# Lakonik/SSDNeRF

Measured on AMD Instinct MI355X. Metric: rays/s (rendered-views/s = rays/s / 16384), SRN Cars 128x128 novel-view render of cached triplanes, higher is better.
Workload: dtype f32

## Files before the change

include/ssdnerf_hip.h:

```cpp
#ifndef SSDNERF_HIP_H
#define SSDNERF_HIP_H

#include <stddef.h>
#include <stdint.h>

#ifdef __cplusplus
extern "C" {
#endif

#define SSDNERF_OK 0
#define SSDNERF_E_INVALID (-1)
#define SSDNERF_E_LAUNCH (-2)
#define SSDNERF_E_WORKSPACE (-3)

#define SSDNERF_DTYPE_F32 0
#define SSDNERF_DTYPE_F16 1

const char* ssdnerf_last_error(void);
int ssdnerf_abi_version(void);


int ssdnerf_near_far_from_aabb(const float* rays_o, const float* rays_d, const float* aabb, uint32_t N, float min_near,
                               float* nears, float* fars, void* stream);

// ... 68 lines not shown
                              const uint8_t* bitfield, uint32_t grid_size, const float* rays_o, const float* rays_d,
                              uint32_t N, float bound, float min_near, float dt_gamma, uint32_t max_steps, float T_thresh,
                              float bg_color, float sigmoid_saturation, float* image, float* depth, float* weights_sum,
                              int32_t* sample_counts, int32_t* overflow_flag, void* stream);

int ssdnerf_render_rays_fused_batch(const void* planes, int planes_dtype, uint32_t Hp, uint32_t Wp, const float* mlp_params,
                                    const uint8_t* bitfield, uint32_t grid_size, const float* rays_o, const float* rays_d,
                                    uint32_t S, uint32_t N, float bound, float min_near, float dt_gamma, const float* dt_gammas,
                                    uint32_t max_steps, float T_thresh, float bg_color, float sigmoid_saturation, float* image,
                                    float* depth, float* weights_sum, int32_t* sample_counts, int32_t* overflow_flag,
                                    void* stream);

size_t ssdnerf_render_queue_workspace(uint32_t S, uint32_t N, uint32_t grid_size);
int ssdnerf_render_first_hit(const uint8_t* bitfield, uint32_t grid_size, const float* rays_o, const float* rays_d, uint32_t S,
                             uint32_t N, float bound, float min_near, float dt_gamma, const float* dt_gammas, uint32_t max_steps,
                             float bg_color, float* image, float* depth, float* weights_sum, int32_t* sample_counts,
                             void* workspace, size_t workspace_bytes, void* stream);
int ssdnerf_render_shade_queue(const void* planes, int planes_dtype, uint32_t Hp, uint32_t Wp, const float* mlp_params,
                               uint32_t grid_size, const float* rays_o, const float* rays_d, uint32_t S, uint32_t N, float bound,
                               float min_near, float dt_gamma, const float* dt_gammas, uint32_t max_steps, float T_thresh,
                               float bg_color, float sigmoid_saturation, float* image, float* depth, float* weights_sum,
                               int32_t* sample_counts, int32_t* overflow_flag, void* workspace, size_t workspace_bytes,
                               void* stream);

#define SSDNERF_SHADE_FULL_DIR_PRODUCTS 0x100
int ssdnerf_render_shade_queue_mfma(const void* planes, int planes_dtype, uint32_t Hp, uint32_t Wp, const float* mlp_params,
                                    uint32_t grid_size, const float* rays_o, const float* rays_d, uint32_t S, uint32_t N,
                                    float bound, float min_near, float dt_gamma, const float* dt_gammas, uint32_t max_steps,
                                    float T_thresh, float bg_color, float sigmoid_saturation, float* image, float* depth,
                                    float* weights_sum, int32_t* sample_counts, int32_t* overflow_flag, void* workspace,
                                    size_t workspace_bytes, void* stream);

#define SSDNERF_FIRST_HIT_SMALL_BLOCKS 0x10000u
int ssdnerf_render_first_hit_cams(const uint8_t* bitfield, uint32_t grid_size, const float* c2w, const float* intrinsics, uint32_t S,
                                  uint32_t V, uint32_t h, uint32_t w, float bound, float min_near, float dt_gamma,
                                  const float* dt_gammas, uint32_t max_steps, float bg_color, float* image, float* depth,
                                  float* weights_sum, int32_t* sample_counts, uint8_t* image_u8, void* workspace, size_t workspace_bytes,
                                  void* stream);
int ssdnerf_render_shade_queue_mfma_cams(const void* planes, int planes_dtype, uint32_t Hp, uint32_t Wp, const float* mlp_params,
                                         uint32_t grid_size, const float* c2w, const float* intrinsics, uint32_t S, uint32_t V,
                                         uint32_t h, uint32_t w, float bound, float min_near, float dt_gamma, const float* dt_gammas,
                                         uint32_t max_steps, float T_thresh, float bg_color, float sigmoid_saturation, float* image,
                                         float* depth, float* weights_sum, int32_t* sample_counts, int32_t* overflow_flag,
                                         uint8_t* image_u8, void* workspace, size_t workspace_bytes, void* stream);

int ssdnerf_density_grid_update(const void* planes, int planes_dtype, uint32_t Hp, uint32_t Wp, const float* mlp_params,
                                uint32_t S, uint32_t grid_size, float bound, const float* jitter, float decay,
                                void* density_grid, int grid_dtype, float* mean_out, void* stream);

int ssdnerf_packbits_dev_thresh(const void* grid, int grid_dtype, uint32_t N, const float* mean, float density_thresh,
                                uint8_t* bitfield, void* stream);


int ssdnerf_ddim_step_v(const float* x_t, const float* v, uint64_t n, float sqrt_ab, float sqrt_1mab, float sqrt_ab_prev,
                        float dir_coef, float clip_lo, float clip_hi, float* x0_out, float* xprev_out, void* stream);

int ssdnerf_dpmpp_step_v(const float* x_t, const float* v, const float* x0_prev, uint64_t n, float sqrt_ab, float sqrt_1mab, float c,
                         float d, float e, float clip_lo, float clip_hi, float* x0_out, float* xnext_out, void* stream);
uint32_t ssdnerf_dpmpp_block_cap(void);

int ssdnerf_philox_normal_fill(float* out, uint64_t n, uint64_t seed, uint32_t draw, void* stream);

int ssdnerf_sde_step_v(const float* x_t, const float* v, const float* x0_prev, uint64_t n, int form, float sqrt_ab, float sqrt_1mab, float c,
                       float d, float e, float nz, float clip_lo, float clip_hi, uint64_t seed, uint32_t draw, float* x0_out, float* xnext_out,
                       void* stream);
uint32_t ssdnerf_sde_block_cap(void);

int ssdnerf_prior_q_sample(const float* x0, const float* a, const float* b, uint32_t B, uint64_t n_per, uint64_t seed, uint32_t draw,
                           float* x_t_out, void* stream);
int ssdnerf_prior_loss_v(const void* pred, int pred_dtype, const float* x0, const float* a, const float* b, uint32_t B, uint64_t n_per,
                         uint64_t seed, uint32_t draw, float* partials, float* msd_out, float* x0sq_out, void* stream);
int ssdnerf_prior_loss_v_backward(const void* pred, int pred_dtype, const float* x0, const float* a, const float* b, const float* k, uint32_t B,
                                  uint64_t n_per, uint64_t seed, uint32_t draw, void* grad_pred_out, float* grad_x0_out, void* stream);
uint32_t ssdnerf_prior_block_cap(void);
uint32_t ssdnerf_prior_blocks_per_sample(uint64_t n_per);
uint64_t ssdnerf_prior_loss_partials(uint32_t B, uint64_t n_per);

int ssdnerf_cam_rays(const float* c2w, const float* intrinsics, uint32_t n_views, uint32_t h, uint32_t w, float* rays_o,
                     float* rays_d, void* stream);

int ssdnerf_quantize_u8(const float* x, uint64_t n, uint8_t* y, void* stream);

int ssdnerf_image_metrics(const float* a, const float* b, uint32_t n, uint32_t h, uint32_t w, float* mse, float* ssim, void* stream);

int ssdnerf_tv_loss_forward(const float* x, uint32_t n, uint32_t h, uint32_t w, float power, float* slice_mean, void* stream);
int ssdnerf_tv_loss_backward(const float* x, const float* g, uint32_t n, uint32_t h, uint32_t w, float power, float* dx_out, void* stream);

#define SSDNERF_ADAM_MAX_TENSORS 32
typedef struct ssdnerf_adam_tensor {
    float* param;
    const float* grad;
    float* exp_avg;
    float* exp_avg_sq;
    uint64_t numel;
    float step_size, bc2_sqrt, weight_decay;
    uint32_t reserved;
} ssdnerf_adam_tensor;
uint32_t ssdnerf_adam_max_tensors(void);
int ssdnerf_adam_step_multi(const ssdnerf_adam_tensor* tensors, uint32_t T, double beta1, double beta2, double eps, void* stream);

#define SSDNERF_EMA_MAX_ROWS (1u << 20)
typedef struct ssdnerf_ema_row {
    const float* src;
    float* dst;
    uint64_t numel;
    uint32_t trainable;
    uint32_t first_block;
} ssdnerf_ema_row;
uint32_t ssdnerf_ema_chunk(void);
int ssdnerf_ema_plan_build(ssdnerf_ema_row* rows, uint32_t T, uint32_t* blocks_out);
int ssdnerf_ema_update_multi(const ssdnerf_ema_row* plan, uint32_t T, uint32_t blocks, float momentum, float momentum_nontrainable, void* stream);

int ssdnerf_gather_views_u8(const uint8_t* store, uint64_t image_bytes, uint64_t num_images, const int32_t* index, uint64_t count, float* out,
                            void* stream);

int ssdnerf_sample_rays_u8(const uint8_t* store, uint64_t num_images, uint32_t h, uint32_t w, const int32_t* view_image, const float* c2w,
                           const float* intr, uint32_t S, uint32_t V, const int64_t* inds, uint32_t R, float* rays_o, float* rays_d, float* target,
                           void* stream);

int ssdnerf_perm_indices(int64_t* out, uint32_t S, uint64_t P, uint64_t start, uint32_t R, uint64_t seed, uint32_t draw, void* stream);
int ssdnerf_sample_rays_perm_u8(const uint8_t* store, uint64_t num_images, uint32_t h, uint32_t w, const int32_t* view_image, const float* c2w,
                                const float* intr, uint32_t S, uint32_t V, uint64_t seed, uint32_t draw, uint64_t start, uint32_t R, float* rays_o,
                                float* rays_d, float* target, void* stream);

#define SSDNERF_CACHE_MAX_SCENES 32
typedef struct ssdnerf_cache_store {
    void* code;
    void* exp_avg;
    void* exp_avg_sq;
    void* density_grid;
    void* density_bitfield;
    uint64_t slots, numel, grid_bytes, bits_bytes;
    int32_t code_dtype, moment_dtype;
} ssdnerf_cache_store;
typedef struct ssdnerf_cache_row {
    uint32_t slot;
    uint32_t row;
    uint32_t has_state;
    uint32_t reserved;
} ssdnerf_cache_row;
uint32_t ssdnerf_cache_max_scenes(void);
int ssdnerf_cache_load_multi(const ssdnerf_cache_store* store, const ssdnerf_cache_row* rows, uint32_t S, float* leaves, float* m, float* v,
                             void* grid, void* bits, void* stream);
int ssdnerf_cache_store_multi(const ssdnerf_cache_store* store, const ssdnerf_cache_row* rows, uint32_t S, const float* leaves, const float* m,
                              const float* v, const void* grid, const void* bits, void* stream);

size_t ssdnerf_group_norm_workspace(uint32_t B, uint32_t G);
int ssdnerf_group_norm_nhwc(const void* x, const void* x2, uint32_t C1, int dtype, uint32_t B, uint32_t HW, uint32_t C, uint32_t G, const float* pre_bias,
                            const float* gamma, const float* beta, const float* scale_shift, uint32_t scale_shift_stride,
                            float eps, int act, void* workspace, int workspace_state, void* y, void* stream);
int ssdnerf_group_norm_nhwc_runs(const void* x, const void* x2, uint32_t C1, int dtype, uint32_t B, uint32_t HW, uint32_t C, uint32_t G, const float* gamma,
                                 const float* beta, const float* scale_shift, uint32_t scale_shift_stride, float eps, int act, const void* runs1,
                                 const void* runs2, void* y, void* stream);

size_t ssdnerf_group_norm_backward_workspace(uint32_t B, uint32_t G);

int ssdnerf_group_norm_nhwc_backward_cat(const void* x, const void* x2, uint32_t C1, const void* dy, int dtype, uint32_t B, uint32_t HW, uint32_t C, uint32_t G,
                                         const float* gamma, const float* beta, const float* scale_shift, uint32_t scale_shift_stride, float eps, int act,
                                         const void* fwd_sums, const void* fwd_sums2, void* bwd_workspace, int bwd_workspace_is_zero, void* dx, void* dx2,
                                         void* stream);
int ssdnerf_group_norm_nhwc_backward(const void* x, const void* dy, int dtype, uint32_t B, uint32_t HW, uint32_t C, uint32_t G,
                                     const float* gamma, const float* beta, const float* scale_shift, uint32_t scale_shift_stride,
                                     float eps, int act, const void* fwd_sums, void* bwd_workspace, int bwd_workspace_is_zero,
                                     void* dx, void* stream);

int ssdnerf_bias_residual_nhwc(const void* x, int dtype, uint32_t B, uint32_t HW, uint32_t C, const float* bias,
                               const void* residual, void* y, void* gn_sums, uint32_t gn_groups, void* stream);

int ssdnerf_conv2d_nhwc_bf16_supported(uint32_t Cin, uint32_t Cout, uint32_t ksize, uint32_t stride, uint32_t upsample);
int ssdnerf_conv2d_nhwc_bf16_plan(uint32_t M, uint32_t Cin, uint32_t Cout, uint32_t ksize, int tile_hint, int may_split,
                                  int splits_hint);
int ssdnerf_conv2d_nhwc_bf16(const void* x, const void* x2, uint32_t Cin1, const void* w, const float* bias,
                             const void* residual, void* y, uint32_t B, uint32_t H, uint32_t W, uint32_t Cin,
                             uint32_t Cout, uint32_t ksize, uint32_t stride,
                             uint32_t upsample, void* gn_sums, uint32_t gn_groups, int tile_hint, void* splitk_ws,
                             size_t splitk_ws_bytes, int splits_hint, void* stream);

int ssdnerf_conv2d_nhwc_f32x2_plan(uint32_t M, uint32_t Cin, uint32_t Cout, uint32_t ksize, int tile_hint, int splits_hint);
int ssdnerf_conv2d_nhwc_f32x2(const void* x, const void* x2, uint32_t Cin1, const void* w_hi, const void* w_lo, const float* bias,
                              const void* residual, void* y, uint32_t B, uint32_t H, uint32_t W, uint32_t Cin, uint32_t Cout,
                              uint32_t ksize, uint32_t stride, uint32_t upsample, void* gn_sums, uint32_t gn_groups, int tile_hint,
                              int splits_hint, int y_is_zero, void* splitk_ws, size_t splitk_ws_bytes, void* stream);

int ssdnerf_conv2d_nhwc_f32x2_presplit_supported(uint32_t B, uint32_t H, uint32_t W, uint32_t Cin, uint32_t Cout, uint32_t ksize, int with_gn_sums);
int ssdnerf_split_f32_nhwc(const void* x, void* y, uint64_t pixels, uint32_t C, uint64_t x_stride, void* stream);
int ssdnerf_conv2d_nhwc_f32x2_presplit(const void* x_split, const void* w_hi, const void* w_lo, const float* bias, const void* residual, void* y, uint32_t B,
                                       uint32_t H, uint32_t W, uint32_t Cin, uint32_t Cout, uint32_t ksize, void* gn_sums, uint32_t gn_groups,
                                       int tile_hint, int splits_hint, void* splitk_ws, size_t splitk_ws_bytes, void* stream);

int ssdnerf_attention_qkv_bf16(const void* qkv, void* out, uint32_t B, uint32_t T, uint32_t heads, uint32_t ch, void* stream);
int ssdnerf_attention_qkv_f32(const void* qkv, void* out, uint32_t B, uint32_t T, uint32_t heads, uint32_t ch, void* stream);
int ssdnerf_attention_qkv_f32_lse(const void* qkv, void* out, void* lse2, uint32_t B, uint32_t T, uint32_t heads, uint32_t ch, void* stream);
int ssdnerf_attention_qkv_f32_backward(const void* qkv, const void* out, const void* dout, const void* lse2, void* dqkv, void* workspace, uint32_t B,
                                       uint32_t T, uint32_t heads, uint32_t ch, void* stream);

int ssdnerf_marching_cubes_count(const float* volume, uint32_t nx, uint32_t ny, uint32_t nz, float iso, const uint8_t* tri_count,
                                 int32_t* cell_tris, int32_t* point_verts, uint8_t* point_mask, void* stream);
int ssdnerf_marching_cubes_emit(const float* volume, uint32_t nx, uint32_t ny, uint32_t nz, float iso, const uint8_t* tri_count,
                                const int8_t* tri_edges, const int32_t* tri_offsets, const int32_t* vert_offsets, const uint8_t* point_mask,
                                float* vertices, int32_t* triangles, void* stream);
int ssdnerf_mesh_vertex_attributes(const void* planes, int planes_dtype, uint32_t Hp, uint32_t Wp, const float* mlp_params, const float* verts_idx,
                                   uint32_t V, const float* b_min, const float* scale, float sigmoid_saturation, float* xyz, float* sigma,
                                   float* grad_sigma, float* normals, float* colors, uint8_t* colors_u8, void* stream);

int ssdnerf_lpips_input(const float* pred, const float* target, uint32_t n, uint32_t h, uint32_t w, float* out, void* stream);
int ssdnerf_relu_pool_nhwc(const float* x, uint32_t N, uint32_t H, uint32_t W, uint32_t C, int pool, int split_out, void* y, void* stream);
size_t ssdnerf_lpips_layer_workspace(uint32_t n);
int ssdnerf_lpips_layer(const float* x, uint32_t n, uint32_t H, uint32_t W, uint32_t C, const float* lin_w, float* acc, void* y_pool, int split_out,
                        void* workspace, void* stream);

int ssdnerf_feature_moments_accumulate(const float* x, uint32_t n, uint32_t D, double* sum, double* outer, void* stream);
size_t ssdnerf_kid_subset_sums_workspace(uint32_t num_subsets, uint32_t m);
int ssdnerf_kid_subset_sums(const float* fake, const float* real, const int64_t* idx_fake, const int64_t* idx_real, uint32_t num_subsets, uint32_t m,
                            uint32_t D, double* out, void* workspace, size_t workspace_bytes, void* stream);

int ssdnerf_png_filter_rows(const void* pred, int pred_is_u8, const void* target, int target_is_u8, uint32_t n, uint32_t h, uint32_t w, uint8_t* out,
                            void* stream);
int ssdnerf_code_plane_rgb(const float* code, const uint8_t* table, uint32_t S, uint32_t C, uint32_t h, uint32_t w, float vmin, float vmax, int flip_z,
                           uint8_t* out, void* stream);

#ifdef __cplusplus
}
#endif
#endif
```

ssdnerf_amd/_cabi.py:

```python
from __future__ import annotations

import ctypes
import os
from typing import Optional

import torch

_LIB_PATH = os.environ.get("SSDNERF_HIP_LIB") or os.path.join(os.path.dirname(os.path.abspath(__file__)), "lib", "libssdnerf_hip.so")
_lib: Optional[ctypes.CDLL] = None

ABI_VERSION = 3
F32, F16 = 0, 1
BF16 = 2

EXPORTS = [
    "ssdnerf_last_error", "ssdnerf_abi_version", "ssdnerf_near_far_from_aabb", "ssdnerf_sph_from_ray", "ssdnerf_morton3D",
    "ssdnerf_morton3D_invert", "ssdnerf_packbits", "ssdnerf_march_rays_train_workspace", "ssdnerf_march_rays_train",
    "ssdnerf_march_rays_train_batch_workspace", "ssdnerf_march_rays_train_batch_count", "ssdnerf_march_rays_train_batch_write",
    "ssdnerf_composite_rays_train_forward", "ssdnerf_composite_rays_train_backward", "ssdnerf_march_rays", "ssdnerf_composite_rays",
    "ssdnerf_sh_encode_forward", "ssdnerf_sh_encode_backward", "ssdnerf_triplane_pack", "ssdnerf_point_decode", "ssdnerf_point_decode_backward_workspace",
    "ssdnerf_point_decode_backward", "ssdnerf_point_decode_backward_layout",
    "ssdnerf_render_rays_fused", "ssdnerf_render_rays_fused_batch", "ssdnerf_render_queue_workspace", "ssdnerf_render_first_hit",
    "ssdnerf_render_shade_queue", "ssdnerf_render_shade_queue_mfma", "ssdnerf_render_first_hit_cams", "ssdnerf_render_shade_queue_mfma_cams", "ssdnerf_density_grid_update", "ssdnerf_packbits_dev_thresh", "ssdnerf_ddim_step_v",
    "ssdnerf_group_norm_workspace", "ssdnerf_group_norm_backward_workspace", "ssdnerf_group_norm_nhwc", "ssdnerf_group_norm_nhwc_runs", "ssdnerf_group_norm_nhwc_backward", "ssdnerf_group_norm_nhwc_backward_cat", "ssdnerf_bias_residual_nhwc",
    "ssdnerf_conv2d_nhwc_bf16_supported", "ssdnerf_conv2d_nhwc_bf16_plan", "ssdnerf_conv2d_nhwc_bf16", "ssdnerf_conv2d_nhwc_f32x2", "ssdnerf_conv2d_nhwc_f32x2_plan", "ssdnerf_attention_qkv_bf16", "ssdnerf_attention_qkv_f32", "ssdnerf_attention_qkv_f32_lse", "ssdnerf_attention_qkv_f32_backward", "ssdnerf_cam_rays", "ssdnerf_quantize_u8",
    "ssdnerf_marching_cubes_count", "ssdnerf_marching_cubes_emit", "ssdnerf_conv2d_nhwc_f32x2_presplit_supported", "ssdnerf_conv2d_nhwc_f32x2_presplit", "ssdnerf_split_f32_nhwc",
    "ssdnerf_image_metrics", "ssdnerf_tv_loss_forward", "ssdnerf_tv_loss_backward", "ssdnerf_mesh_vertex_attributes",
    "ssdnerf_lpips_input", "ssdnerf_relu_pool_nhwc", "ssdnerf_lpips_layer_workspace", "ssdnerf_lpips_layer",
    "ssdnerf_feature_moments_accumulate", "ssdnerf_kid_subset_sums_workspace", "ssdnerf_kid_subset_sums",
    "ssdnerf_adam_max_tensors", "ssdnerf_adam_step_multi",
    "ssdnerf_gather_views_u8", "ssdnerf_sample_rays_u8", "ssdnerf_perm_indices", "ssdnerf_sample_rays_perm_u8",
    "ssdnerf_ema_chunk", "ssdnerf_ema_plan_build", "ssdnerf_ema_update_multi",
    "ssdnerf_cache_max_scenes", "ssdnerf_cache_load_multi", "ssdnerf_cache_store_multi",
    "ssdnerf_dpmpp_step_v", "ssdnerf_dpmpp_block_cap",
    "ssdnerf_png_filter_rows", "ssdnerf_code_plane_rgb",
    "ssdnerf_philox_normal_fill", "ssdnerf_sde_step_v", "ssdnerf_sde_block_cap",
    "ssdnerf_prior_q_sample", "ssdnerf_prior_loss_v", "ssdnerf_prior_loss_v_backward", "ssdnerf_prior_block_cap", "ssdnerf_prior_blocks_per_sample",
    "ssdnerf_prior_loss_partials",
]


class AdamTensor(ctypes.Structure):
    _fields_ = [("param", ctypes.c_void_p), ("grad", ctypes.c_void_p), ("exp_avg", ctypes.c_void_p), ("exp_avg_sq", ctypes.c_void_p),
                ("numel", ctypes.c_uint64), ("step_size", ctypes.c_float), ("bc2_sqrt", ctypes.c_float), ("weight_decay", ctypes.c_float),
                ("reserved", ctypes.c_uint32)]


class EmaRow(ctypes.Structure):
    _fields_ = [("src", ctypes.c_void_p), ("dst", ctypes.c_void_p), ("numel", ctypes.c_uint64), ("trainable", ctypes.c_uint32),
                ("first_block", ctypes.c_uint32)]


class CacheStore(ctypes.Structure):
    _fields_ = [("code", ctypes.c_void_p), ("exp_avg", ctypes.c_void_p), ("exp_avg_sq", ctypes.c_void_p), ("density_grid", ctypes.c_void_p),
                ("density_bitfield", ctypes.c_void_p), ("slots", ctypes.c_uint64), ("numel", ctypes.c_uint64), ("grid_bytes", ctypes.c_uint64),
                ("bits_bytes", ctypes.c_uint64), ("code_dtype", ctypes.c_int32), ("moment_dtype", ctypes.c_int32)]


class CacheRow(ctypes.Structure):
    _fields_ = [("slot", ctypes.c_uint32), ("row", ctypes.c_uint32), ("has_state", ctypes.c_uint32), ("reserved", ctypes.c_uint32)]


def lib_path() -> str:
    return _LIB_PATH


def lib() -> ctypes.CDLL:
    global _lib
    if _lib is None:
        if not os.path.exists(_LIB_PATH):
            raise RuntimeError(
                f"libssdnerf_hip.so not found at {_LIB_PATH}: build it with `python -m ssdnerf_amd.build` "
                "(there is no CPU fallback for the product path)")
        l = ctypes.CDLL(_LIB_PATH)
        l.ssdnerf_last_error.restype = ctypes.c_char_p
        l.ssdnerf_abi_version.restype = ctypes.c_int
        l.ssdnerf_march_rays_train_workspace.restype = ctypes.c_size_t
        l.ssdnerf_march_rays_train_workspace.argtypes = [ctypes.c_uint32]
        l.ssdnerf_render_queue_workspace.restype = ctypes.c_size_t
        l.ssdnerf_render_queue_workspace.argtypes = [ctypes.c_uint32, ctypes.c_uint32, ctypes.c_uint32]
        l.ssdnerf_march_rays_train_batch_workspace.restype = ctypes.c_size_t
        l.ssdnerf_march_rays_train_batch_workspace.argtypes = [ctypes.c_uint32, ctypes.c_uint32]
        l.ssdnerf_point_decode_backward_workspace.restype = ctypes.c_size_t
        l.ssdnerf_point_decode_backward_workspace.argtypes = [ctypes.c_uint32] * 4
        l.ssdnerf_point_decode_backward_layout.restype = None
        l.ssdnerf_point_decode_backward_layout.argtypes = [ctypes.c_uint32] * 4 + [ctypes.POINTER(ctypes.c_uint64)]
        l.ssdnerf_group_norm_workspace.restype = ctypes.c_size_t
        l.ssdnerf_group_norm_workspace.argtypes = [ctypes.c_uint32, ctypes.c_uint32]
        l.ssdnerf_group_norm_backward_workspace.restype = ctypes.c_size_t
        l.ssdnerf_group_norm_backward_workspace.argtypes = [ctypes.c_uint32, ctypes.c_uint32]
        l.ssdnerf_image_metrics.argtypes = [ctypes.c_void_p, ctypes.c_void_p, ctypes.c_uint32, ctypes.c_uint32, ctypes.c_uint32, ctypes.c_void_p,
                                             ctypes.c_void_p, ctypes.c_void_p]
        l.ssdnerf_tv_loss_forward.argtypes = [ctypes.c_void_p, ctypes.c_uint32, ctypes.c_uint32, ctypes.c_uint32, ctypes.c_float, ctypes.c_void_p,
                                              ctypes.c_void_p]
        l.ssdnerf_tv_loss_backward.argtypes = [ctypes.c_void_p, ctypes.c_void_p, ctypes.c_uint32, ctypes.c_uint32, ctypes.c_uint32, ctypes.c_float,
                                               ctypes.c_void_p, ctypes.c_void_p]
        l.ssdnerf_mesh_vertex_attributes.argtypes = [ctypes.c_void_p, ctypes.c_int, ctypes.c_uint32, ctypes.c_uint32, ctypes.c_void_p, ctypes.c_void_p,
                                                     ctypes.c_uint32, ctypes.POINTER(ctypes.c_float), ctypes.POINTER(ctypes.c_float), ctypes.c_float] + [ctypes.c_void_p] * 7
        l.ssdnerf_lpips_input.argtypes = [ctypes.c_void_p, ctypes.c_void_p, ctypes.c_uint32, ctypes.c_uint32, ctypes.c_uint32, ctypes.c_void_p, ctypes.c_void_p]
        l.ssdnerf_relu_pool_nhwc.argtypes = [ctypes.c_void_p] + [ctypes.c_uint32] * 4 + [ctypes.c_int, ctypes.c_int, ctypes.c_void_p, ctypes.c_void_p]
        l.ssdnerf_lpips_layer_workspace.restype = ctypes.c_size_t
        l.ssdnerf_lpips_layer_workspace.argtypes = [ctypes.c_uint32]
        l.ssdnerf_lpips_layer.argtypes = [ctypes.c_void_p] + [ctypes.c_uint32] * 4 + [ctypes.c_void_p, ctypes.c_void_p, ctypes.c_void_p, ctypes.c_int, ctypes.c_void_p,
                                          ctypes.c_void_p]
        l.ssdnerf_feature_moments_accumulate.argtypes = [ctypes.c_void_p, ctypes.c_uint32, ctypes.c_uint32, ctypes.c_void_p, ctypes.c_void_p, ctypes.c_void_p]
        l.ssdnerf_kid_subset_sums_workspace.restype = ctypes.c_size_t
        l.ssdnerf_kid_subset_sums_workspace.argtypes = [ctypes.c_uint32, ctypes.c_uint32]
        l.ssdnerf_kid_subset_sums.argtypes = [ctypes.c_void_p] * 4 + [ctypes.c_uint32] * 3 + [ctypes.c_void_p, ctypes.c_void_p, ctypes.c_size_t, ctypes.c_void_p]
        l.ssdnerf_adam_max_tensors.restype = ctypes.c_uint32
        l.ssdnerf_adam_max_tensors.argtypes = []
        l.ssdnerf_adam_step_multi.argtypes = [ctypes.POINTER(AdamTensor), ctypes.c_uint32, ctypes.c_double, ctypes.c_double, ctypes.c_double, ctypes.c_void_p]
        l.ssdnerf_gather_views_u8.argtypes = [ctypes.c_void_p, ctypes.c_uint64, ctypes.c_uint64, ctypes.c_void_p, ctypes.c_uint64, ctypes.c_void_p, ctypes.c_void_p]
        l.ssdnerf_sample_rays_u8.argtypes = [ctypes.c_void_p, ctypes.c_uint64, ctypes.c_uint32, ctypes.c_uint32] + [ctypes.c_void_p] * 3 + \
                                            [ctypes.c_uint32, ctypes.c_uint32, ctypes.c_void_p, ctypes.c_uint32] + [ctypes.c_void_p] * 4
        l.ssdnerf_perm_indices.argtypes = [ctypes.c_void_p, ctypes.c_uint32, ctypes.c_uint64, ctypes.c_uint64, ctypes.c_uint32, ctypes.c_uint64,
                                           ctypes.c_uint32, ctypes.c_void_p]
        l.ssdnerf_sample_rays_perm_u8.argtypes = [ctypes.c_void_p, ctypes.c_uint64, ctypes.c_uint32, ctypes.c_uint32] + [ctypes.c_void_p] * 3 + \
                                                 [ctypes.c_uint32, ctypes.c_uint32, ctypes.c_uint64, ctypes.c_uint32, ctypes.c_uint64, ctypes.c_uint32] + \
                                                 [ctypes.c_void_p] * 4
        l.ssdnerf_ema_chunk.restype = ctypes.c_uint32
        l.ssdnerf_ema_chunk.argtypes = []
        l.ssdnerf_ema_plan_build.argtypes = [ctypes.POINTER(EmaRow), ctypes.c_uint32, ctypes.POINTER(ctypes.c_uint32)]
        l.ssdnerf_ema_update_multi.argtypes = [ctypes.c_void_p, ctypes.c_uint32, ctypes.c_uint32, ctypes.c_float, ctypes.c_float, ctypes.c_void_p]
        l.ssdnerf_cache_max_scenes.restype = ctypes.c_uint32
        l.ssdnerf_cache_max_scenes.argtypes = []
        for fn in (l.ssdnerf_cache_load_multi, l.ssdnerf_cache_store_multi):
            fn.argtypes = [ctypes.POINTER(CacheStore), ctypes.POINTER(CacheRow), ctypes.c_uint32] + [ctypes.c_void_p] * 6
        l.ssdnerf_dpmpp_block_cap.restype = ctypes.c_uint32
        l.ssdnerf_dpmpp_block_cap.argtypes = []
        l.ssdnerf_dpmpp_step_v.argtypes = [ctypes.c_void_p] * 3 + [ctypes.c_uint64] + [ctypes.c_float] * 7 + [ctypes.c_void_p] * 3
        l.ssdnerf_sde_block_cap.restype = ctypes.c_uint32
        l.ssdnerf_sde_block_cap.argtypes = []
        l.ssdnerf_philox_normal_fill.argtypes = [ctypes.c_void_p, ctypes.c_uint64, ctypes.c_uint64, ctypes.c_uint32, ctypes.c_void_p]
        l.ssdnerf_sde_step_v.argtypes = [ctypes.c_void_p] * 3 + [ctypes.c_uint64, ctypes.c_int] + [ctypes.c_float] * 8 + \
                                        [ctypes.c_uint64, ctypes.c_uint32] + [ctypes.c_void_p] * 3
        l.ssdnerf_prior_block_cap.restype = l.ssdnerf_prior_blocks_per_sample.restype = ctypes.c_uint32
        l.ssdnerf_prior_block_cap.argtypes = []
        l.ssdnerf_prior_blocks_per_sample.argtypes = [ctypes.c_uint64]
        l.ssdnerf_prior_loss_partials.restype = ctypes.c_uint64
        l.ssdnerf_prior_loss_partials.argtypes = [ctypes.c_uint32, ctypes.c_uint64]
        l.ssdnerf_prior_q_sample.argtypes = [ctypes.c_void_p] * 3 + [ctypes.c_uint32, ctypes.c_uint64, ctypes.c_uint64, ctypes.c_uint32] + [ctypes.c_void_p] * 2
        l.ssdnerf_prior_loss_v.argtypes = [ctypes.c_void_p, ctypes.c_int] + [ctypes.c_void_p] * 3 + \
                                          [ctypes.c_uint32, ctypes.c_uint64, ctypes.c_uint64, ctypes.c_uint32] + [ctypes.c_void_p] * 4
        l.ssdnerf_prior_loss_v_backward.argtypes = [ctypes.c_void_p, ctypes.c_int] + [ctypes.c_void_p] * 4 + \
                                                   [ctypes.c_uint32, ctypes.c_uint64, ctypes.c_uint64, ctypes.c_uint32] + [ctypes.c_void_p] * 3
        l.ssdnerf_png_filter_rows.argtypes =[ctypes.c_void_p, ctypes.c_int, ctypes.c_void_p, ctypes.c_int] + [ctypes.c_uint32] * 3 + [ctypes.c_void_p] * 2
        l.ssdnerf_code_plane_rgb.argtypes = [ctypes.c_void_p] * 2 + [ctypes.c_uint32] * 4 + [ctypes.c_float] * 2 + [ctypes.c_int] + [ctypes.c_void_p] * 2
        if l.ssdnerf_abi_version() != ABI_VERSION:
            raise RuntimeError(f"libssdnerf_hip.so ABI {l.ssdnerf_abi_version()} != expected {ABI_VERSION}: rebuild")
        _lib = l
    return _lib


_SYNC_CHECK = os.environ.get("SSDNERF_SYNC_CHECK", "0") == "1"


def check(status: int, what: str) -> None:
    if status != 0:
        raise RuntimeError(f"{what} failed ({status}): {lib().ssdnerf_last_error().decode()}")
    if _SYNC_CHECK and not torch.cuda.is_current_stream_capturing():
        import sys
        print(f"[ssdnerf sync-check] {what}", file=sys.stderr, flush=True)
        torch.cuda.synchronize()


def ptr(t: Optional[torch.Tensor]) -> ctypes.c_void_p:
    return ctypes.c_void_p(0 if t is None else t.data_ptr())


def stream() -> ctypes.c_void_p:
    return ctypes.c_void_p(torch.cuda.current_stream().cuda_stream)


def u32(v) -> ctypes.c_uint32:
    return ctypes.c_uint32(int(v))


def f32(v) -> ctypes.c_float:
    return ctypes.c_float(float(v))


def dtype_code(t: torch.Tensor) -> int:
    if t.dtype == torch.float32:
        return F32
    if t.dtype == torch.float16:
        return F16
    raise RuntimeError(f"unsupported dtype {t.dtype} (fp32 / fp16 only)")


def require_cuda(*tensors: torch.Tensor) -> None:
    for t in tensors:
# ... 3 lines not shown
```

ssdnerf_amd/csrc/conv_igemm.hip:

```cpp
#include "common.h"
#include <type_traits>

namespace {

typedef __attribute__((ext_vector_type(8))) __bf16 bf16x8;
typedef __attribute__((ext_vector_type(16))) float f32x16;

__device__ __attribute__((aligned(16))) const uint32_t g_conv_zero_page[4] = {0, 0, 0, 0};

struct ConvArgs {
    const unsigned char* x;
    const unsigned char* x2;
    uint32_t Cin1;
    const unsigned char* w;
    const float* bias;
    const unsigned char* res;
    unsigned char* y;
    double* gn_sums;
    float* splitk_ws;
    uint32_t splits;
    uint32_t B, H, W, Cin, Cout;
    uint32_t Ho, Wo, M;
    uint32_t ksize, stride, pad, upsample;
    uint32_t G;
    uint32_t m_tiles, n_tiles;
};

constexpr int CV_BK = 64;
constexpr int CV_ROWB = CV_BK * 2;

SSD_DEV void cv_glds16(const void* gptr, unsigned char* lds_wave_base) {
    __builtin_amdgcn_global_load_lds((const __attribute__((address_space(1))) void*)gptr, (__attribute__((address_space(3))) void*)lds_wave_base, 16, 0, 0);
}

SSD_DEV uint32_t cv_pack_bf16(float lo, float hi) {
    typedef float f2 __attribute__((ext_vector_type(2)));
    typedef __bf16 b2 __attribute__((ext_vector_type(2)));
    const b2 r = __builtin_convertvector(f2{lo, hi}, b2);
    return *reinterpret_cast<const uint32_t*>(&r);
}

template <int CTRL, int RM, int BM, bool BC> SSD_DEV double cv_dpp_f64(double v) {
    const unsigned long long u = (unsigned long long)__double_as_longlong(v);
    const uint32_t lo = (uint32_t)__builtin_amdgcn_update_dpp(0, (int)(uint32_t)u, CTRL, RM, BM, BC);
    const uint32_t hi = (uint32_t)__builtin_amdgcn_update_dpp(0, (int)(uint32_t)(u >> 32), CTRL, RM, BM, BC);
    return __longlong_as_double((long long)(((unsigned long long)hi << 32) | lo));
}
SSD_DEV double cv_half_wave_sum(double v) {
    v += cv_dpp_f64<0xB1, 0xf, 0xf, true>(v);
    v += cv_dpp_f64<0x4E, 0xf, 0xf, true>(v);
    v += cv_dpp_f64<0x141, 0xf, 0xf, true>(v);
    v += cv_dpp_f64<0x140, 0xf, 0xf, true>(v);
    v += cv_dpp_f64<0x142, 0xa, 0xf, false>(v);
    return v;
}

template <int TM, int TN, bool F32 = false>
SSD_DEV void cv_epilogue_direct(const ConvArgs& a, f32x16 (&acc)[TN][TM], unsigned char* lds, uint32_t m0, uint32_t n0, uint32_t wm, uint32_t wn) {
    constexpr int BN = 128;
    const uint32_t tid = threadIdx.x, lane = tid & 63, half = lane >> 5;
    using S = double;
    S* red = reinterpret_cast<S*>(lds);
    if (a.gn_sums) {
        if (tid < BN / 4 * 2) red[tid] = S(0);
        __syncthreads();
    }
#pragma unroll
    for (int j = 0; j < TN; ++j) {
        const uint32_t cb = n0 + wn * 32 * TN + j * 32;
        float4 bv[4];
#pragma unroll
        for (int q = 0; q < 4; ++q) bv[q] = a.bias ? *reinterpret_cast<const float4*>(a.bias + cb + 8 * q + 4 * half) : make_float4(0.f, 0.f, 0.f, 0.f);
        S gs[4] = {S(0), S(0), S(0), S(0)}, gq[4] = {S(0), S(0), S(0), S(0)};
#pragma unroll
        for (int i = 0; i < TM; ++i) {
            const uint32_t m = m0 + wm * 32 * TM + i * 32 + (lane & 31);
            const bool ok = m < a.M;
            const size_t row = (size_t)(ok ? m : 0) * a.Cout;
            uint2 pk[4];
#pragma unroll
            for (int q = 0; q < 4; ++q) {
                float f[4] = {acc[j][i][4 * q] + bv[q].x, acc[j][i][4 * q + 1] + bv[q].y, acc[j][i][4 * q + 2] + bv[q].z, acc[j][i][4 * q + 3] + bv[q].w};
                if (F32) {
                    const size_t o = row + cb + 8 * q + 4 * half;
                    if (a.res) {
                        const float4 rv = *reinterpret_cast<const float4*>(reinterpret_cast<const float*>(a.res) + o);
                        f[0] += rv.x; f[1] += rv.y; f[2] += rv.z; f[3] += rv.w;
                    }
                    if (ok) *reinterpret_cast<float4*>(reinterpret_cast<float*>(a.y) + o) = make_float4(f[0], f[1], f[2], f[3]);
                    if (a.gn_sums && ok) {
#pragma unroll
                        for (int k = 0; k < 4; ++k) { const double v = f[k]; gs[q] += v; gq[q] = __builtin_fma(v, v, gq[q]); }
                    }
                    continue;
                }
                if (a.res) {
                    const uint2 rv = *reinterpret_cast<const uint2*>(a.res + (row + cb + 8 * q + 4 * half) * 2);
                    f[0] += __uint_as_float(rv.x << 16); f[1] += __uint_as_float(rv.x & 0xffff0000u);
                    f[2] += __uint_as_float(rv.y << 16); f[3] += __uint_as_float(rv.y & 0xffff0000u);
                }
                pk[q] = make_uint2(cv_pack_bf16(f[0], f[1]), cv_pack_bf16(f[2], f[3]));
                if (a.gn_sums && ok) {
                    const double r[4] = {__uint_as_float(pk[q].x << 16), __uint_as_float(pk[q].x & 0xffff0000u), __uint_as_float(pk[q].y << 16),
                                         __uint_as_float(pk[q].y & 0xffff0000u)};
#pragma unroll
                    for (int k = 0; k < 4; ++k) { gs[q] += r[k]; gq[q] = __builtin_fma(r[k], r[k], gq[q]); }
                }
            }
#pragma unroll
            for (int qp = 0; qp < (F32 ? 0 : 2); ++qp) {
                auto sx = __builtin_amdgcn_permlane32_swap(pk[2 * qp].x, pk[2 * qp + 1].x, false, false);
                auto sy = __builtin_amdgcn_permlane32_swap(pk[2 * qp].y, pk[2 * qp + 1].y, false, false);
                if (ok) *reinterpret_cast<uint4*>(a.y + (row + cb + 16 * qp + 8 * half) * 2) = make_uint4(sx[0], sy[0], sx[1], sy[1]);
            }
        }
        if (a.gn_sums) {
#pragma unroll
            for (int q = 0; q < 4; ++q) {
                const S s1 = cv_half_wave_sum(gs[q]), s2 = cv_half_wave_sum(gq[q]);
                if ((lane & 31) == 31) {
                    const uint32_t run = (cb - n0 + 8 * q + 4 * half) / 4;
                    atomicAdd(&red[run * 2], s1);
                    atomicAdd(&red[run * 2 + 1], s2);
                }
            }
        }
    }
    if (a.gn_sums) {
        __syncthreads();
        const uint32_t cpg = a.Cout / a.G, hpg = cpg / 4, g0 = n0 / cpg, ng = (n0 + BN - 1) / cpg - g0 + 1;
        if (tid < ng && m0 < a.M) {
            const uint32_t lo = max((g0 + tid) * hpg, n0 / 4) - n0 / 4, hi = min((g0 + tid + 1) * hpg, (n0 + BN) / 4) - n0 / 4;
            S ss = S(0), qq = S(0);
            for (uint32_t i = lo; i < hi; ++i) { ss += red[i * 2]; qq += red[i * 2 + 1]; }
            double* dst = a.gn_sums + ((size_t)(m0 / (a.Ho * a.Wo)) * a.G + g0 + tid) * 2;
            atomicAdd(dst, (double)ss);
            atomicAdd(dst + 1, (double)qq);
        }
    }
}

typedef __attribute__((address_space(3))) void* cv_lds_ptr;
SSD_DEV __amdgpu_buffer_rsrc_t cv_rsrc(const void* base, uint64_t bytes) {
    return __builtin_amdgcn_make_buffer_rsrc(const_cast<void*>(base), 0, (uint32_t)bytes, 0x00020000);
}
SSD_DEV void cv_dma16(__amdgpu_buffer_rsrc_t r, unsigned char* dst, uint32_t voff, uint32_t soff) {
    __builtin_amdgcn_raw_ptr_buffer_load_lds(r, (cv_lds_ptr)dst, 16, voff, soff, 0, 0);
}
static constexpr uint32_t CV_OOB = 0x80000000u;


template <int N> SSD_DEV void cv_wait_tiles_and_barrier() {
    asm volatile("s_waitcnt vmcnt(%0) lgkmcnt(0)\n\ts_barrier" ::"n"(N) : "memory");
}

template <int TM, int TN, int WM, int WN, bool PT = false>
SSD_DEV void cv_epilogue_bf16(const ConvArgs& a, f32x16 (&acc)[TM][TN], unsigned char* lds, uint32_t m0, uint32_t n0) {
    constexpr int NT = 64 * WM * WN, BM = 32 * TM * WM, BN = 32 * TN * WN;
    constexpr int EP_ROWS = BM < 128 ? BM : 128, EPI = EP_ROWS * BN * 4;
    const uint32_t tid = threadIdx.x, lane = tid & 63, wave = tid >> 6, wm = wave / WN, wn = wave % WN;
    float* tile_f = reinterpret_cast<float*>(lds);
    constexpr int CPR = BN / 8;
    double* red = reinterpret_cast<double*>(lds + EPI);
    if (a.gn_sums && tid < CPR * 4) red[tid] = 0.0;
    const uint32_t cc = tid % CPR, co = n0 + cc * 8;
    const bool c_ok = !PT || co < a.Cout;
    float bias_v[8];
#pragma unroll
    for (int k = 0; k < 8; ++k) bias_v[k] = (a.bias && c_ok) ? a.bias[co + k] : 0.f;
    double gs[2] = {0.0, 0.0}, gq[2] = {0.0, 0.0};
#pragma unroll
    for (int pass = 0; pass < BM / EP_ROWS; ++pass) {
        if (pass) __syncthreads();
        if ((wm * 32 * TM) / EP_ROWS == (uint32_t)pass) {
#pragma unroll
            for (int i = 0; i < TM; ++i)
#pragma unroll
                for (int j = 0; j < TN; ++j)
#pragma unroll
                    for (int e = 0; e < 16; ++e) {
                        const uint32_t row = (wm * 32 * TM) % EP_ROWS + i * 32 + (e & 3) + 8 * (e >> 2) + 4 * (lane >> 5);
                        const uint32_t col = wn * 32 * TN + j * 32 + (lane & 31);
                        tile_f[row * BN + col] = acc[i][j][e];
                    }
        }
        __syncthreads();
#pragma unroll 2
        for (uint32_t row = tid / CPR; row < (uint32_t)EP_ROWS; row += NT / CPR) {
            const uint32_t m = m0 + pass * EP_ROWS + row;
            if (m >= a.M || !c_ok) break;
            const float4 v0 = *reinterpret_cast<const float4*>(tile_f + row * BN + cc * 8);
            const float4 v1 = *reinterpret_cast<const float4*>(tile_f + row * BN + cc * 8 + 4);
            float f[8] = {v0.x, v0.y, v0.z, v0.w, v1.x, v1.y, v1.z, v1.w};
#pragma unroll
            for (int k = 0; k < 8; ++k) f[k] += bias_v[k];
            const size_t o = ((size_t)m * a.Cout + co) * 2;
            if (a.res) {
                const uint4 rv = *reinterpret_cast<const uint4*>(a.res + o);
                const uint32_t rw[4] = {rv.x, rv.y, rv.z, rv.w};
#pragma unroll
                for (int k = 0; k < 4; ++k) { f[2 * k] += __uint_as_float(rw[k] << 16); f[2 * k + 1] += __uint_as_float(rw[k] & 0xffff0000u); }
            }
            uint32_t pk[4];
#pragma unroll
            for (int k = 0; k < 4; ++k) pk[k] = cv_pack_bf16(f[2 * k], f[2 * k + 1]);
            *reinterpret_cast<uint4*>(a.y + o) = make_uint4(pk[0], pk[1], pk[2], pk[3]);
            if (a.gn_sums) {
#pragma unroll
                for (int k = 0; k < 4; ++k) {
                    const double lo = __uint_as_float(pk[k] << 16), hi = __uint_as_float(pk[k] & 0xffff0000u);
                    gs[k >> 1] += lo + hi;
                    gq[k >> 1] = __builtin_fma(lo, lo, gq[k >> 1]);
                    gq[k >> 1] = __builtin_fma(hi, hi, gq[k >> 1]);
                }
            }
        }
    }
    if (a.gn_sums) {
#pragma unroll
        for (int h = 0; h < 2; ++h) { atomicAdd(&red[(cc * 2 + h) * 2], gs[h]); atomicAdd(&red[(cc * 2 + h) * 2 + 1], gq[h]); }
        __syncthreads();
        const uint32_t n1 = PT ? min(n0 + BN, a.Cout) : n0 + BN;
        const uint32_t cpg = a.Cout / a.G, hpg = cpg / 4, g0 = n0 / cpg, ng = (n1 - 1) / cpg - g0 + 1;
        if (tid < ng && m0 < a.M) {
            const uint32_t lo = max((g0 + tid) * hpg, n0 / 4) - n0 / 4, hi = min((g0 + tid + 1) * hpg, n1 / 4) - n0 / 4;
            double ss = 0.0, qq = 0.0;
            for (uint32_t i = lo; i < hi; ++i) { ss += red[i * 2]; qq += red[i * 2 + 1]; }
            double* dst = a.gn_sums + ((size_t)(m0 / (a.Ho * a.Wo)) * a.G + g0 + tid) * 2;
            atomicAdd(dst, ss);
            atomicAdd(dst + 1, qq);
        }
    }
}

template <int TM, int TN, bool PT = false> SSD_DEV void cv_epilogue_f32(const ConvArgs& a, f32x16 (&acc)[TM][TN], unsigned char* lds, uint32_t m0, uint32_t n0);

template <int TM, int TN, int WM, int WN, int NS, bool PT, bool PS = false>
__global__ __launch_bounds__(64 * WM * WN) void k_conv_igemm_bf16(const ConvArgs a) {
    static_assert(!PS || (WM == 2 && WN == 2 && !PT), "the pre-split form shares cv_epilogue_f32's 2 x 2 wave grid and takes whole tiles only");
    constexpr int KCH = PS ? 32 : CV_BK;
    constexpr int XB = PS ? 4 : 2;
    constexpr int NW = WM * WN, NT = 64 * NW;
    constexpr int BM = 32 * TM * WM, BN = 32 * TN * WN;
    constexpr int A_INST = BM / 8 / NW, B_INST = BN / 8 / NW;
    constexpr int STAGE = (BM + BN) * CV_ROWB;
    constexpr int EP_ROWS = BM < 128 ? BM : 128;
    constexpr int EPI = EP_ROWS * BN * 4;
    constexpr int LPT = A_INST + B_INST;
    constexpr int LDS_BYTES = ((NS * STAGE > EPI) ? NS * STAGE : EPI) + 512;
    static_assert((BM / 8) % NW == 0 && (BN / 8) % NW == 0 && EP_ROWS % (32 * TM) == 0, "tile / wave grid mismatch");
    __shared__ __attribute__((aligned(1024))) unsigned char lds[LDS_BYTES];

    const uint32_t tid = threadIdx.x, lane = tid & 63, wave = __builtin_amdgcn_readfirstlane(tid >> 6);
    const uint32_t wm = wave / WN, wn = wave % WN;

    const uint32_t n_blocks = a.m_tiles * a.n_tiles * a.splits;
    uint32_t tile, split;
    {
        const uint32_t xcd = blockIdx.x & 7, idx = blockIdx.x >> 3, q = n_blocks >> 3, r = n_blocks & 7;
        const uint32_t lin = (xcd < r ? xcd * (q + 1) : r * (q + 1) + (xcd - r) * q) + idx;
        tile = lin / a.splits; split = lin % a.splits;
    }
    const uint32_t m0 = (tile / a.n_tiles) * BM, n0 = (tile % a.n_tiles) * BN;

    const uint32_t taps = a.ksize * a.ksize;
    const uint32_t Hv = a.upsample ? a.H * 2 : a.H, Wv = a.upsample ? a.W * 2 : a.W;
    int32_t a_y0[A_INST], a_x0[A_INST];
    uint32_t a_img[A_INST], a_sc[A_INST];
    bool a_ok[A_INST];
#pragma unroll
    for (int i = 0; i < A_INST; ++i) {
        const uint32_t r = (wave * A_INST + i) * 8 + (lane >> 3);
        const uint32_t m = m0 + r;
        a_ok[i] = m < a.M;
        const uint32_t mm = a_ok[i] ? m : 0;
        const uint32_t b = mm / (a.Ho * a.Wo), rem = mm % (a.Ho * a.Wo);
        a_y0[i] = (int32_t)((rem / a.Wo) * a.stride) - (int32_t)a.pad;
        a_x0[i] = (int32_t)((rem % a.Wo) * a.stride) - (int32_t)a.pad;
        a_img[i] = b * a.H * a.W;
        a_sc[i] = (lane & 7) ^ ((r >> 1) & 7);
    }
    uint32_t b_off[B_INST], b_sc[B_INST];
#pragma unroll
    for (int i = 0; i < B_INST; ++i) {
        const uint32_t r = (wave * B_INST + i) * 8 + (lane >> 3);
        b_sc[i] = (lane & 7) ^ ((r >> 1) & 7);
        if (PS) b_off[i] = ((n0 + r) * taps * a.Cin) * 2 + (b_sc[i] & 3) * 16 + (b_sc[i] >> 2) * (a.Cout * taps * a.Cin * 2);
        else b_off[i] = (!PT || n0 + r < a.Cout) ? ((n0 + r) * taps * a.Cin) * 2 + b_sc[i] * 16 : CV_OOB;
    }

    const __amdgpu_buffer_rsrc_t rs_x = cv_rsrc(a.x, (uint64_t)a.B * a.H * a.W * a.Cin1 * XB);
    const __amdgpu_buffer_rsrc_t rs_x2 = cv_rsrc(a.x2 ? a.x2 : a.x, a.x2 ? (uint64_t)a.B * a.H * a.W * (a.Cin - a.Cin1) * 2 : 0);
    const __amdgpu_buffer_rsrc_t rs_w = cv_rsrc(a.w, (uint64_t)a.Cout * taps * a.Cin * 2 * (PS ? 2 : 1));
    uint32_t a_voff[A_INST], a_voff2[A_INST];
    const uint32_t Cin2 = a.Cin - a.Cin1;
    auto set_tap = [&](uint32_t tap) {
        const int32_t kh = (int32_t)(tap / a.ksize), kw = (int32_t)(tap % a.ksize);
#pragma unroll
        for (int i = 0; i < A_INST; ++i) {
            const int32_t yv = a_y0[i] + kh, xv = a_x0[i] + kw;
            const bool ok = a_ok[i] && yv >= 0 && xv >= 0 && yv < (int32_t)Hv && xv < (int32_t)Wv;
            const uint32_t yi = a.upsample ? (uint32_t)yv >> 1 : (uint32_t)yv, xi = a.upsample ? (uint32_t)xv >> 1 : (uint32_t)xv;
            const uint32_t pix = a_img[i] + yi * a.W + xi;
            a_voff[i] = ok ? pix * a.Cin1 * XB + a_sc[i] * 16 : CV_OOB;
            a_voff2[i] = ok ? pix * Cin2 * 2 + a_sc[i] * 16 : CV_OOB;
        }
    };

    const uint32_t kc1 = (a.Cin1 + KCH - 1) / KCH, kc = kc1 + (Cin2 + CV_BK - 1) / CV_BK;
    auto tile_channels = [&](uint32_t ci) {
        if (!PT) return (uint32_t)CV_BK;
        const uint32_t left = ci >= kc1 ? Cin2 - (ci - kc1) * CV_BK : a.Cin1 - ci * CV_BK;
        return left < (uint32_t)CV_BK ? left : (uint32_t)CV_BK;
    };
    auto issue = [&](uint32_t tap, uint32_t ci, uint32_t buf) {
        unsigned char* sa = lds + buf * STAGE;
        unsigned char* sb = sa + BM * CV_ROWB;
        const bool second = ci >= kc1;
        const uint32_t cb = (second ? ci - kc1 : ci) * KCH, coff = cb * XB, nchunk = tile_channels(ci) >> 3;
#pragma unroll
        for (int i = 0; i < A_INST; ++i) {
            unsigned char* dst = sa + (wave * A_INST + i) * 1024;
            if (second) cv_dma16(rs_x2, dst, (!PT || a_sc[i] < nchunk) ? a_voff2[i] : CV_OOB, coff);
            else cv_dma16(rs_x, dst, (!PT || a_sc[i] < nchunk) ? a_voff[i] : CV_OOB, coff);
        }
#pragma unroll
        for (int i = 0; i < B_INST; ++i)
            cv_dma16(rs_w, sb + (wave * B_INST + i) * 1024, (!PT || b_sc[i] < nchunk) ? b_off[i] : CV_OOB, (tap * a.Cin + (second ? a.Cin1 : 0u) + cb) * 2);
    };

    const uint32_t rd_row = lane & 31;
    const uint32_t rd_c0 = ((lane >> 5) ^ ((lane >> 1) & 7)) * 16;
    const uint32_t a_rd = (wm * 32 * TM + rd_row) * CV_ROWB + rd_c0;
    const uint32_t b_rd = BM * CV_ROWB + (wn * 32 * TN + rd_row) * CV_ROWB + rd_c0;

    f32x16 acc[TM][TN];
#pragma unroll
    for (int i = 0; i < TM; ++i)
#pragma unroll
        for (int j = 0; j < TN; ++j)
#pragma unroll
            for (int e = 0; e < 16; ++e) acc[i][j][e] = 0.f;

    const uint32_t KT_all = taps * kc;
    const uint32_t kt_begin = (uint32_t)((uint64_t)split * KT_all / a.splits), KT = (uint32_t)((uint64_t)(split + 1) * KT_all / a.splits) - kt_begin;
    uint32_t tap = kt_begin / kc, ci = kt_begin % kc, issued = 0;
    uint32_t ci_mul = ci;
    set_tap(tap);
    auto issue_next = [&]() {
        if (issued) { if (++ci == kc) { ci = 0; ++tap; set_tap(tap); } }
        issue(tap, ci, issued % NS);
        ++issued;
    };
#pragma unroll
    for (int p = 0; p < NS - 1; ++p)
        if (issued < KT) issue_next();
    for (uint32_t kt = 0; kt < KT; ++kt) {
        const uint32_t in_flight = issued - (kt + 1);
        if (NS >= 4 && in_flight >= 2) cv_wait_tiles_and_barrier<2 * LPT>();
        else if (NS >= 3 && in_flight == 1) cv_wait_tiles_and_barrier<1 * LPT>();
        else cv_wait_tiles_and_barrier<0>();
        if (issued < KT) issue_next();
        const unsigned char* st = lds + (kt % NS) * STAGE;
        const uint32_t ksteps = (tile_channels(ci_mul) + 15) >> 4;
        if (PT && ++ci_mul == kc) ci_mul = 0;
        if (!PT || ksteps == 4) {
            bf16x8 fa[4][TM], fb[4][TN];
#pragma unroll
            for (int s = 0; s < 4; ++s) {
#pragma unroll
                for (int i = 0; i < TM; ++i) fa[s][i] = *reinterpret_cast<const bf16x8*>(st + ((a_rd + i * 32 * CV_ROWB) ^ (s * 32)));
#pragma unroll
                for (int j = 0; j < TN; ++j) fb[s][j] = *reinterpret_cast<const bf16x8*>(st + ((b_rd + j * 32 * CV_ROWB) ^ (s * 32)));
            }
            __builtin_amdgcn_sched_barrier(0);
            if (PS) {
#pragma unroll
                for (int s = 0; s < 2; ++s)
#pragma unroll
                    for (int i = 0; i < TM; ++i)
#pragma unroll
                        for (int j = 0; j < TN; ++j) {
                            acc[i][j] = __builtin_amdgcn_mfma_f32_32x32x16_bf16(fa[2 + s][i], fb[s][j], acc[i][j], 0, 0, 0);
                            acc[i][j] = __builtin_amdgcn_mfma_f32_32x32x16_bf16(fa[s][i], fb[2 + s][j], acc[i][j], 0, 0, 0);
                            acc[i][j] = __builtin_amdgcn_mfma_f32_32x32x16_bf16(fa[s][i], fb[s][j], acc[i][j], 0, 0, 0);
                        }
            } else {
#pragma unroll
            for (int s = 0; s < 4; ++s)
#pragma unroll
                for (int i = 0; i < TM; ++i)
#pragma unroll
                    for (int j = 0; j < TN; ++j) acc[i][j] = __builtin_amdgcn_mfma_f32_32x32x16_bf16(fa[s][i], fb[s][j], acc[i][j], 0, 0, 0);
            }
        } else {
            for (uint32_t s = 0; s < ksteps; ++s) {
                bf16x8 fa[TM], fb[TN];
#pragma unroll
                for (int i = 0; i < TM; ++i) fa[i] = *reinterpret_cast<const bf16x8*>(st + ((a_rd + i * 32 * CV_ROWB) ^ (s * 32)));
#pragma unroll
                for (int j = 0; j < TN; ++j) fb[j] = *reinterpret_cast<const bf16x8*>(st + ((b_rd + j * 32 * CV_ROWB) ^ (s * 32)));
#pragma unroll
                for (int i = 0; i < TM; ++i)
#pragma unroll
                    for (int j = 0; j < TN; ++j) acc[i][j] = __builtin_amdgcn_mfma_f32_32x32x16_bf16(fa[i], fb[j], acc[i][j], 0, 0, 0);
            }
        }
    }
    __syncthreads();

    if (a.splits > 1) {
#pragma unroll
        for (int i = 0; i < TM; ++i)
#pragma unroll
            for (int j = 0; j < TN; ++j)
#pragma unroll
                for (int e = 0; e < 16; ++e) {
                    const uint32_t m = m0 + wm * 32 * TM + i * 32 + (e & 3) + 8 * (e >> 2) + 4 * (lane >> 5);
                    const uint32_t col = n0 + wn * 32 * TN + j * 32 + (lane & 31);
                    if (m < a.M && (!PT || col < a.Cout)) unsafeAtomicAdd(a.splitk_ws + (size_t)m * a.Cout + col, acc[i][j][e]);
                }
        return;
    }

    if constexpr (PS) cv_epilogue_f32<TM, TN, false>(a, acc, lds, m0, n0);
    else cv_epilogue_bf16<TM, TN, WM, WN, PT>(a, acc, lds, m0, n0);
}

template <int TM, int TN, bool PT>
SSD_DEV void cv_epilogue_f32(const ConvArgs& a, f32x16 (&acc)[TM][TN], unsigned char* lds, uint32_t m0, uint32_t n0) {
    constexpr int BM = 64 * TM, BN = 64 * TN, EPI = BM * BN * 4;
    const uint32_t tid = threadIdx.x, lane = tid & 63, wave = tid >> 6, wm = wave >> 1, wn = wave & 1;
    float* tile_f = reinterpret_cast<float*>(lds);
#pragma unroll
    for (int i = 0; i < TM; ++i)
#pragma unroll
        for (int j = 0; j < TN; ++j)
#pragma unroll
            for (int e = 0; e < 16; ++e)
                tile_f[(wm * 32 * TM + i * 32 + (e & 3) + 8 * (e >> 2) + 4 * (lane >> 5)) * BN + wn * 32 * TN + j * 32 + (lane & 31)] = acc[i][j][e];
    constexpr int CPR = BN / 8;
    double* red = reinterpret_cast<double*>(lds + EPI);
    if (a.gn_sums && tid < CPR * 4) red[tid] = 0.0;
    __syncthreads();
    const uint32_t cc = tid % CPR, co = n0 + cc * 8;
    const bool c_ok = !PT || co < a.Cout;
    float bias_v[8];
#pragma unroll
    for (int k = 0; k < 8; ++k) bias_v[k] = (a.bias && c_ok) ? a.bias[co + k] : 0.f;
    double gs[2] = {0.0, 0.0}, gq[2] = {0.0, 0.0};
    float* yo = reinterpret_cast<float*>(a.y);
    const float* ro = reinterpret_cast<const float*>(a.res);
#pragma unroll 2
    for (uint32_t row = tid / CPR; row < (uint32_t)BM; row += 256 / CPR) {
        const uint32_t m = m0 + row;
        if (m >= a.M || !c_ok) break;
        const float4 v0 = *reinterpret_cast<const float4*>(tile_f + row * BN + cc * 8), v1 = *reinterpret_cast<const float4*>(tile_f + row * BN + cc * 8 + 4);
        float f[8] = {v0.x, v0.y, v0.z, v0.w, v1.x, v1.y, v1.z, v1.w};
#pragma unroll
        for (int k = 0; k < 8; ++k) f[k] += bias_v[k];
        const size_t o = (size_t)m * a.Cout + co;
        if (ro) {
            const float4 r0 = *reinterpret_cast<const float4*>(ro + o), r1 = *reinterpret_cast<const float4*>(ro + o + 4);
            f[0] += r0.x; f[1] += r0.y; f[2] += r0.z; f[3] += r0.w; f[4] += r1.x; f[5] += r1.y; f[6] += r1.z; f[7] += r1.w;
        }
        *reinterpret_cast<float4*>(yo + o) = make_float4(f[0], f[1], f[2], f[3]);
        *reinterpret_cast<float4*>(yo + o + 4) = make_float4(f[4], f[5], f[6], f[7]);
        if (a.gn_sums) {
#pragma unroll
            for (int k = 0; k < 8; ++k) { const double v = f[k]; gs[k >> 2] += v; gq[k >> 2] = __builtin_fma(v, v, gq[k >> 2]); }
        }
    }
    if (a.gn_sums) {
#pragma unroll
        for (int h = 0; h < 2; ++h) { atomicAdd(&red[(cc * 2 + h) * 2], gs[h]); atomicAdd(&red[(cc * 2 + h) * 2 + 1], gq[h]); }
        __syncthreads();
        const uint32_t n1 = PT ? min(n0 + BN, a.Cout) : n0 + BN;
        const uint32_t cpg = a.Cout / a.G, hpg = cpg / 4, g0 = n0 / cpg, ng = (n1 - 1) / cpg - g0 + 1;
        if (tid < ng && m0 < a.M) {
            const uint32_t lo = max((g0 + tid) * hpg, n0 / 4) - n0 / 4, hi = min((g0 + tid + 1) * hpg, n1 / 4) - n0 / 4;
            double ss = 0.0, qq = 0.0;
            for (uint32_t i = lo; i < hi; ++i) { ss += red[i * 2]; qq += red[i * 2 + 1]; }
            double* dst = a.gn_sums + ((size_t)(m0 / (a.Ho * a.Wo)) * a.G + g0 + tid) * 2;
            atomicAdd(dst, ss);
            atomicAdd(dst + 1, qq);
        }
    }
}

__global__ __launch_bounds__(256) void k_conv3x3_bf16_rows(const ConvArgs a) {
    constexpr int TM = 2, TN = 2, BM = 128, BN = 128;
    constexpr int A_INST = BM / 32, B_INST = BN / 32;
    constexpr int A_ROWS = BM + 4 + 1, A_BUF = A_ROWS * CV_ROWB, B_BUF = BN * CV_ROWB;
    constexpr int EPI = BM * BN * 4;
    constexpr int LDS_BYTES = ((2 * A_BUF + 2 * B_BUF > EPI) ? 2 * A_BUF + 2 * B_BUF : EPI) + 512;
    __shared__ __attribute__((aligned(1024))) unsigned char lds[LDS_BYTES];
    const uint32_t tid = threadIdx.x, lane = tid & 63, wave = tid >> 6, wm = wave >> 1, wn = wave & 1;
    unsigned char* const abuf = lds;
    unsigned char* const bbuf = lds + 2 * A_BUF;

    const uint32_t n_blocks = a.m_tiles * a.n_tiles;
    uint32_t tile;
    {
        const uint32_t xcd = blockIdx.x & 7, idx = blockIdx.x >> 3, q = n_blocks >> 3, r = n_blocks & 7;
// ... 812 lines not shown
                if (P == 1) { advance_l(); if (l_kt < KT && l_ci == 0) set_tap(l_tap); }
            }
        }
        __builtin_amdgcn_sched_barrier(0);
        if (F32 && PS) {
            if (P == 0) pp_wait_vm_lgkm_barrier(issued);
            else pp_wait_lgkm_barrier();
        } else if (F32) {
            asm volatile("s_waitcnt lgkmcnt(0)" ::: "memory");
#pragma unroll
            for (int i = 0; i < TM; ++i) {
                const float v[8] = {xa[F32 ? i : 0][0].x, xa[F32 ? i : 0][0].y, xa[F32 ? i : 0][0].z, xa[F32 ? i : 0][0].w,
                                    xa[F32 ? i : 0][1].x, xa[F32 ? i : 0][1].y, xa[F32 ? i : 0][1].z, xa[F32 ? i : 0][1].w};
                uint32_t hw[4], lw[4];
#pragma unroll
                for (int k = 0; k < 4; ++k) {
                    const float r0 = v[2 * k] - __uint_as_float(__float_as_uint(v[2 * k]) & 0xffff0000u);
                    const float r1 = v[2 * k + 1] - __uint_as_float(__float_as_uint(v[2 * k + 1]) & 0xffff0000u);
                    hw[k] = __builtin_amdgcn_perm(__float_as_uint(v[2 * k + 1]), __float_as_uint(v[2 * k]), 0x07060302u);
                    lw[k] = __builtin_amdgcn_perm(__float_as_uint(r1), __float_as_uint(r0), 0x07060302u);
                }
                const uint4 uh = make_uint4(hw[0], hw[1], hw[2], hw[3]), ul = make_uint4(lw[0], lw[1], lw[2], lw[3]);
                fa[P][0][i] = *reinterpret_cast<const bf16x8*>(&uh);
                fa[P][1][i] = *reinterpret_cast<const bf16x8*>(&ul);
            }
            __builtin_amdgcn_sched_barrier(0);
            if (P == 0) pp_wait_vm_barrier(issued);
            else pp_barrier();
        } else if (P == 0) pp_wait_vm_lgkm_barrier(issued);
        else pp_wait_lgkm_barrier();
        __builtin_amdgcn_sched_barrier(0);
        __builtin_amdgcn_s_setprio(1);
        if (has_next) {
            if (P == 0) load_frags(P1{}, kwc, sa_n, sb_n);
            else load_frags(P0{}, kwnc, sa_n, sb_n);
        }
        __builtin_amdgcn_sched_barrier(0);
        if (F32) {
#pragma unroll
            for (int i = 0; i < TM; ++i)
#pragma unroll
                for (int j = 0; j < TN; ++j) {
                    acc[j][i] = __builtin_amdgcn_mfma_f32_32x32x16_bf16(fb[P][1][j], fa[P][0][i], acc[j][i], 0, 0, 0);
                    acc[j][i] = __builtin_amdgcn_mfma_f32_32x32x16_bf16(fb[P][0][j], fa[P][1][i], acc[j][i], 0, 0, 0);
                    acc[j][i] = __builtin_amdgcn_mfma_f32_32x32x16_bf16(fb[P][0][j], fa[P][0][i], acc[j][i], 0, 0, 0);
                }
        } else {
#pragma unroll
            for (int s = 0; s < 2; ++s)
#pragma unroll
                for (int i = 0; i < TM; ++i)
#pragma unroll
                    for (int j = 0; j < TN; ++j) acc[j][i] = __builtin_amdgcn_mfma_f32_32x32x16_bf16(fb[P][s][j], fa[P][s][i], acc[j][i], 0, 0, 0);
        }
        __builtin_amdgcn_s_setprio(0);
        __builtin_amdgcn_sched_barrier(0);
        pp_barrier();
        __builtin_amdgcn_sched_barrier(0);
    };
    if (ROWS) {
        const uint32_t G = 3 * kc;
        for (uint32_t g = 0, t = 0; g < G; ++g, t += 3) {
            const unsigned char* sa = abuf + (g & 1) * A_BUF;
            const unsigned char* sb0 = bbuf + (t % NB) * B_BUF;
            const unsigned char* sb1 = bbuf + ((t + 1) % NB) * B_BUF;
            const unsigned char* sb2 = bbuf + ((t + 2) % NB) * B_BUF;
            phase(P0{}, K0{}, K0{}, sa, sb0, true);
            phase(P1{}, K0{}, K1{}, sa, sb1, true);
            phase(P0{}, K1{}, K1{}, sa, sb1, true);
            phase(P1{}, K1{}, K2{}, sa, sb2, true);
            phase(P0{}, K2{}, K2{}, sa, sb2, true);
            phase(P1{}, K2{}, K0{}, abuf + ((g + 1) & 1) * A_BUF, bbuf + ((t + 3) % NB) * B_BUF, g + 1 < G);
        }
    } else {
        for (uint32_t t = 0; t < KT; ++t) {
            const unsigned char* sa = abuf + (t % NA) * A_BUF;
            const unsigned char* sb = bbuf + (t % NB) * B_BUF;
            phase(P0{}, K0{}, K0{}, sa, sb, true);
            phase(P1{}, K0{}, K0{}, abuf + ((t + 1) % NA) * A_BUF, bbuf + ((t + 1) % NB) * B_BUF, t + 1 < KT);
        }
    }
    if (group == 0) pp_barrier();
    __syncthreads();
#ifdef CV_PP_TIMING
    if (tid == 0) stamps[2] = __builtin_amdgcn_s_memtime();
#endif
    cv_epilogue_direct<TM, TN, F32>(a, acc, lds + RING, m0, n0, wm, wn);
#ifdef CV_PP_TIMING
    asm volatile("s_waitcnt vmcnt(0)" ::: "memory");
    if (tid == 0) stamps[3] = __builtin_amdgcn_s_memtime();
#endif
    if (a.gn_sums) __syncthreads();
  }
}

#ifndef CV_NS_SMALL
#define CV_NS_SMALL 4
#endif
template <int TM, int TN, int WM, int WN, int NS>
int cv_launch(ConvArgs& a, hipStream_t st) {
    constexpr int BM = 32 * TM * WM, BN = 32 * TN * WN;
    a.m_tiles = (a.M + BM - 1) / BM;
    a.n_tiles = (a.Cout + BN - 1) / BN;
    const bool partial = a.Cin1 % CV_BK != 0 || (a.Cin - a.Cin1) % CV_BK != 0 || a.Cout % BN != 0;
    if (partial) hipLaunchKernelGGL((k_conv_igemm_bf16<TM, TN, WM, WN, NS, true>), dim3(a.m_tiles * a.n_tiles * a.splits), dim3(64 * WM * WN), 0, st, a);
    else hipLaunchKernelGGL((k_conv_igemm_bf16<TM, TN, WM, WN, NS, false>), dim3(a.m_tiles * a.n_tiles * a.splits), dim3(64 * WM * WN), 0, st, a);
    return 0;
}

uint32_t cv_cu_count() {
    static const uint32_t n = [] {
        int dev = 0, n_cu = 0;
        hipDeviceProp_t prop;
        if (hipGetDevice(&dev) == hipSuccess && hipGetDeviceProperties(&prop, dev) == hipSuccess) n_cu = prop.multiProcessorCount;
        if (n_cu < 8) n_cu = 256;
        return (uint32_t)(n_cu & ~7);
    }();
    return n;
}

template <bool ROWS, bool F32 = false, bool PS = false>
void cv_launch_pp(ConvArgs& a, hipStream_t st) {
    a.m_tiles = (a.M + 255) / 256;
    a.n_tiles = a.Cout / 128;
    const uint32_t tiles = a.m_tiles * a.n_tiles, n_cu = cv_cu_count();
    hipLaunchKernelGGL((k_conv_pp_bf16<ROWS, F32, PS>), dim3(tiles < n_cu ? tiles : n_cu), dim3(512), 0, st, a);
}

void cv_launch_finish(const ConvArgs& a, bool f32_out, float* ws, hipStream_t st) {
    const uint32_t HWo = a.Ho * a.Wo, cpr = a.Cout / 8, rstep = 256 / cpr ? 256 / cpr : 1;
    uint32_t rows = HWo;
    while (rows > rstep && rows % 2 == 0 && (uint64_t)a.B * (HWo / rows) < 1024) rows /= 2;
    const dim3 grid((HWo + rows - 1) / rows, a.B);
    if (f32_out) hipLaunchKernelGGL(k_conv_f32_finish, grid, dim3(256), 0, st, (float*)a.y, ws, a.bias, (const float*)a.res, HWo, cpr, rows, a.gn_sums, a.G);
    else hipLaunchKernelGGL(k_conv_splitk_finish, grid, dim3(256), 0, st, ws, a.bias, a.res, a.y, HWo, cpr, rows, a.gn_sums, a.G);
}

ConvArgs cv_args(const void* x, const void* x2, uint32_t Cin1, const void* w, const float* bias, const void* residual, void* y, uint32_t B, uint32_t H,
                 uint32_t W, uint32_t Cin, uint32_t Cout, uint32_t ksize, uint32_t stride, uint32_t upsample, void* gn_sums, uint32_t gn_groups,
                 void* splitk_ws, size_t splitk_ws_bytes) {
    ConvArgs a;
    a.x = (const unsigned char*)x; a.x2 = (const unsigned char*)x2; a.Cin1 = x2 ? Cin1 : Cin;
    a.w = (const unsigned char*)w; a.bias = bias; a.res = (const unsigned char*)residual; a.y = (unsigned char*)y;
    a.gn_sums = (double*)gn_sums; a.G = gn_groups ? gn_groups : 1;
    a.B = B; a.H = H; a.W = W; a.Cin = Cin; a.Cout = Cout;
    a.ksize = ksize; a.stride = stride; a.pad = ksize / 2; a.upsample = upsample;
    const uint32_t Hv = upsample ? 2 * H : H, Wv = upsample ? 2 * W : W;
    a.Ho = (Hv + 2 * a.pad - ksize) / stride + 1;
    a.Wo = (Wv + 2 * a.pad - ksize) / stride + 1;
    a.M = B * a.Ho * a.Wo;
    a.splitk_ws = (splitk_ws && splitk_ws_bytes >= (size_t)a.M * Cout * 4) ? (float*)splitk_ws : nullptr;
    a.splits = 1;
    a.m_tiles = a.n_tiles = 0;
    return a;
}

int cv_check_layer(const char* fn, const void* x2, uint32_t Cin1, uint32_t Cin, uint32_t Cout, uint32_t ksize, uint32_t stride, uint32_t upsample) {
    SSD_REQUIRE(ssdnerf_conv2d_nhwc_bf16_supported(Cin, Cout, ksize, stride, upsample),
                "%s: needs Cin %% 8 == 0, Cout %% 8 == 0, ksize 1|3, stride 1|2 (no stride with upsample)", fn);
    SSD_REQUIRE(!x2 || (Cin1 <= Cin && Cin1 % 8 == 0), "%s: the first input's channel count must be a multiple of 8 and <= Cin", fn);
    SSD_REQUIRE((uint64_t)Cout * ksize * ksize * Cin * 2 < (1ull << 31), "%s: weight tensor too large", fn);
    return SSDNERF_OK;
}

int cv_check_gn(const char* fn, const void* gn_sums, uint32_t gn_groups, uint32_t Cout) {
    SSD_REQUIRE(!gn_sums || (gn_groups > 0 && Cout % gn_groups == 0 && (Cout / gn_groups) % 4 == 0), "%s: fused GroupNorm statistics need groups of a multiple of 4 channels", fn);
    return SSDNERF_OK;
}

}

static void cv_plan(uint32_t M, uint32_t Cin, uint32_t Cout, uint32_t ksize, int tile_hint, bool may_split, int splits_hint, int* choice_out, uint32_t* splits_out) {
    int choice = tile_hint;
    if (choice < 1 || choice > 4) {
        const uint64_t t128 = (uint64_t)((M + 127) / 128) * (Cout / 128);
        const uint64_t t64 = (uint64_t)((M + 63) / 64) * (Cout / 128);
        choice = (Cout % 128 != 0) ? 3 : (t128 >= 384) ? 1 : (t64 >= 512) ? 2 : 3;
    }
    const uint32_t bm = choice == 4 ? 256 : choice == 1 ? 128 : 64, bn = choice == 3 ? 64 : 128;
    const uint32_t tiles = ((M + bm - 1) / bm) * ((Cout + bn - 1) / bn);
    const uint32_t KT = ksize * ksize * ((Cin + 63) / 64);
    uint32_t splits = 1;
    if (may_split) {
        if (splits_hint > 0) splits = (uint32_t)splits_hint;
        else if (tiles < 384 && (uint64_t)M * Cout <= (1u << 20)) {
            splits = (384 + tiles / 2) / tiles;
            if (splits > KT / 12) splits = KT / 12;
            if (splits == 2 && KT < 64) splits = 1;
            if (splits < 1) splits = 1;
        }
        if (splits > 16) splits = 16;
        if (splits > KT / 2) splits = KT / 2 ? KT / 2 : 1;
    }
    *choice_out = choice; *splits_out = splits;
}

extern "C" int ssdnerf_conv2d_nhwc_bf16_plan(uint32_t M, uint32_t Cin, uint32_t Cout, uint32_t ksize, int tile_hint, int may_split, int splits_hint) {
    int choice; uint32_t splits;
    cv_plan(M, Cin, Cout, ksize, tile_hint, may_split != 0, splits_hint, &choice, &splits);
    return choice | (int)(splits << 8);
}

extern "C" int ssdnerf_conv2d_nhwc_f32x2_plan(uint32_t M, uint32_t Cin, uint32_t Cout, uint32_t ksize, int tile_hint, int splits_hint) {
    int choice = tile_hint;
    if (choice != 1 && choice != 3) choice = (Cout % 128 == 0 && (uint64_t)((M + 127) / 128) * (Cout / 128) >= 384) ? 1 : 3;
    const uint32_t bm = choice == 1 ? 128 : 64, tiles = ((M + bm - 1) / bm) * ((Cout + bm - 1) / bm), KT = ksize * ksize * ((Cin + 31) / 32);
    uint32_t splits = 1;
    if (splits_hint > 0) splits = (uint32_t)splits_hint;
    else if (tiles < 512 && (uint64_t)M * Cout <= (1u << 21) && Cout <= 1024) splits = (1024 + tiles - 1) / tiles;
    if (splits > 16) splits = 16;
    if (splits > KT / 2) splits = KT / 2 ? KT / 2 : 1;
    return choice | (int)(splits << 8);
}

extern "C" int ssdnerf_conv2d_nhwc_f32x2(const void* x, const void* x2, uint32_t Cin1, const void* w_hi, const void* w_lo, const float* bias, const void* residual,
                                         void* y, uint32_t B, uint32_t H, uint32_t W, uint32_t Cin, uint32_t Cout, uint32_t ksize, uint32_t stride, uint32_t upsample,
                                         void* gn_sums, uint32_t gn_groups, int tile_hint, int splits_hint, int y_is_zero, void* splitk_ws, size_t splitk_ws_bytes,
                                         void* stream) {
    if (B == 0 || H == 0 || W == 0) return SSDNERF_OK;
    SSD_REQUIRE(x && w_hi && w_lo && y, "conv2d_nhwc_f32x2: null pointer");
    if (const int e = cv_check_layer("conv2d_nhwc_f32x2", x2, Cin1, Cin, Cout, ksize, stride, upsample)) return e;
    if (const int e = cv_check_gn("conv2d_nhwc_f32x2", gn_sums, gn_groups, Cout)) return e;
    ConvArgs a = cv_args(x, x2, Cin1, w_hi, bias, residual, y, B, H, W, Cin, Cout, ksize, stride, upsample, gn_sums, gn_groups, splitk_ws, splitk_ws_bytes);
    SSD_REQUIRE((uint64_t)B * a.Ho * a.Wo < (1ull << 31), "conv2d_nhwc_f32x2: tensor too large");
    const int plan = ssdnerf_conv2d_nhwc_f32x2_plan(a.M, Cin, Cout, ksize, tile_hint, splits_hint);
    const int choice = plan & 0xff;
    const uint32_t splits = (uint32_t)plan >> 8, bm = choice == 1 ? 128 : 64;
    if (choice == 1) SSD_REQUIRE(Cout % 128 == 0, "conv2d_nhwc_f32x2: 128-wide tiles need Cout %% 128 == 0");
    SSD_REQUIRE(!gn_sums || splits > 1 || (a.Ho * a.Wo) % bm == 0, "conv2d_nhwc_f32x2: fused GroupNorm statistics need Ho*Wo to be a multiple of the M tile");
    hipStream_t st = (hipStream_t)stream;
    const bool pp_ok = Cin % 32 == 0 && a.Cin1 % 32 == 0 && Cout % 128 == 0 && (const unsigned char*)w_lo == (const unsigned char*)w_hi + (size_t)Cout * ksize * ksize * Cin * 2
                       && (uint64_t)B * H * W * Cin * 4 < (1ull << 31) && (!gn_sums || (a.Ho * a.Wo) % 256 == 0);
    if (tile_hint == 0 && pp_ok && splits == 1 && ksize == 3 && stride == 1 && a.M >= 32768 && !upsample && (W == 128 || W == 64) && (H * W) % 256 == 0)
        tile_hint = 6;
    if (tile_hint == 5 || tile_hint == 6) {
        SSD_REQUIRE(pp_ok, "conv2d_nhwc_f32x2: the 256 x 128 kernel needs Cin %% 32 == 0, Cout %% 128 == 0 and w_lo directly behind w_hi");
        const bool pp_rows = tile_hint == 6 && ksize == 3 && stride == 1 && !upsample && (W == 128 || W == 64 || W == 32) && (H * W) % 256 == 0;
        if (pp_rows) cv_launch_pp<true, true>(a, st); else cv_launch_pp<false, true>(a, st);
        SSD_CHECK_LAUNCH("conv2d_nhwc_f32x2");
        return SSDNERF_OK;
    }
    a.splits = splits;
    if (splits > 1 && !a.splitk_ws && !y_is_zero && hipMemsetAsync(y, 0, (size_t)a.M * Cout * 4, st) != hipSuccess)
        return ssdnerf_fail(SSDNERF_E_LAUNCH, "conv2d_nhwc_f32x2: memset failed");
    a.m_tiles = (a.M + bm - 1) / bm; a.n_tiles = (Cout + bm - 1) / bm;
    const bool rows = Cin % 64 == 0 && a.Cin1 % 64 == 0 && choice == 1 && splits == 1 && ksize == 3 && stride == 1 && !upsample && (W == 128 || W == 64 || W == 32) && (H * W) % 128 == 0;
    if (rows) hipLaunchKernelGGL(k_conv3x3_f32x2_rows, dim3(a.m_tiles * a.n_tiles), dim3(256), 0, st, a, (const unsigned char*)w_lo);
    else {
        const bool partial = a.Cin1 % 32 != 0 || (Cin - a.Cin1) % 32 != 0 || Cout % bm != 0;
        const dim3 grid(a.m_tiles * a.n_tiles * splits);
        if (choice == 1 && partial) hipLaunchKernelGGL((k_conv_igemm_f32x2<2, 2, true>), grid, dim3(256), 0, st, a, (const unsigned char*)w_lo);
        else if (choice == 1) hipLaunchKernelGGL((k_conv_igemm_f32x2<2, 2, false>), grid, dim3(256), 0, st, a, (const unsigned char*)w_lo);
        else if (partial) hipLaunchKernelGGL((k_conv_igemm_f32x2<1, 1, true>), grid, dim3(256), 0, st, a, (const unsigned char*)w_lo);
        else hipLaunchKernelGGL((k_conv_igemm_f32x2<1, 1, false>), grid, dim3(256), 0, st, a, (const unsigned char*)w_lo);
    }
    if (splits > 1) cv_launch_finish(a, true, a.splitk_ws, st);
    SSD_CHECK_LAUNCH("conv2d_nhwc_f32x2");
    return SSDNERF_OK;
}

static int cv_ps_plan(uint32_t M, uint32_t Cin, uint32_t Cout, uint32_t ksize, int tile_hint, int splits_hint) {
    int choice = tile_hint;
    if (choice < 1 || choice > 3) choice = (Cout % 128 == 0 && (uint64_t)((M + 127) / 128) * (Cout / 128) >= 384) ? 1 : 3;
    const uint32_t bm = choice == 1 ? 128 : 64, bn = choice == 3 ? 64 : 128, tiles = ((M + bm - 1) / bm) * ((Cout + bn - 1) / bn), KT = ksize * ksize * (Cin / 32);
    uint32_t splits = 1;
    if (splits_hint > 0) splits = (uint32_t)splits_hint;
    else if (tiles < 384 && KT >= 64 && (uint64_t)M * Cout <= (1u << 21) && Cout <= 1024) {
        splits = (512 + tiles / 2) / tiles;
        if (splits > 8) splits = 8;
        while (splits > 1 && KT / splits < 16) --splits;
    }
    if (splits > 16) splits = 16;
    if (splits > KT / 2) splits = KT / 2 ? KT / 2 : 1;
    return choice | (int)(splits << 8);
}

extern "C" int ssdnerf_conv2d_nhwc_f32x2_presplit_supported(uint32_t B, uint32_t H, uint32_t W, uint32_t Cin, uint32_t Cout, uint32_t ksize, int with_gn_sums) {
    const uint64_t M = (uint64_t)B * H * W;
    if (B == 0 || H == 0 || W == 0 || (ksize != 1 && ksize != 3) || Cin % 32 != 0 || M >= (1ull << 31) || M * Cin * 4 >= (1ull << 31)
        || (uint64_t)Cout * ksize * ksize * Cin * 4 >= (1ull << 31)) return 0;
    if (ksize == 3 && Cout % 128 == 0 && (W == 128 || W == 64) && (H * W) % 256 == 0 && M >= 32768) return 1;
    if (Cout % 64 != 0 || M * Cout * 4 >= (1ull << 31)) return 0;
    const int plan = cv_ps_plan((uint32_t)M, Cin, Cout, ksize, 0, 0);
    const uint32_t bm = (plan & 0xff) == 1 ? 128 : 64, splits = (uint32_t)plan >> 8;
    if (with_gn_sums && splits == 1 && (H * W) % bm != 0) return 0;
    return 2;
}

extern "C" int ssdnerf_conv2d_nhwc_f32x2_presplit(const void* x_split, const void* w_hi, const void* w_lo, const float* bias, const void* residual, void* y, uint32_t B,
                                                  uint32_t H, uint32_t W, uint32_t Cin, uint32_t Cout, uint32_t ksize, void* gn_sums, uint32_t gn_groups,
                                                  int tile_hint, int splits_hint, void* splitk_ws, size_t splitk_ws_bytes, void* stream) {
    if (B == 0 || H == 0 || W == 0) return SSDNERF_OK;
    SSD_REQUIRE(x_split && w_hi && w_lo && y, "conv2d_nhwc_f32x2_presplit: null pointer");
    int kind = ssdnerf_conv2d_nhwc_f32x2_presplit_supported(B, H, W, Cin, Cout, ksize, gn_sums != nullptr);
    if (tile_hint >= 1 && tile_hint <= 3 && ssdnerf_conv2d_nhwc_f32x2_presplit_supported(B, H, W, Cin, tile_hint == 3 ? 64 : 128, ksize, 0) && Cout % (tile_hint == 3 ? 64 : 128) == 0)
        kind = 2;
    SSD_REQUIRE(kind != 0, "conv2d_nhwc_f32x2_presplit: layer not taken by a pre-split kernel (ask ssdnerf_conv2d_nhwc_f32x2_presplit_supported first)");
    SSD_REQUIRE((const unsigned char*)w_lo == (const unsigned char*)w_hi + (size_t)Cout * ksize * ksize * Cin * 2, "conv2d_nhwc_f32x2_presplit: w_lo must lie directly behind w_hi");
    if (const int e = cv_check_gn("conv2d_nhwc_f32x2_presplit", gn_sums, gn_groups, Cout)) return e;
    hipStream_t st = (hipStream_t)stream;
    ConvArgs a = cv_args(x_split, nullptr, Cin, w_hi, bias, residual, y, B, H, W, Cin, Cout, ksize, 1, 0, gn_sums, gn_groups, splitk_ws, splitk_ws_bytes);
    if (kind == 1) {
        cv_launch_pp<true, true, true>(a, st);
        SSD_CHECK_LAUNCH("conv2d_nhwc_f32x2_presplit");
        return SSDNERF_OK;
    }
    const int plan = cv_ps_plan(a.M, Cin, Cout, ksize, tile_hint, splits_hint);
    const int choice = plan & 0xff;
    const uint32_t bm = choice == 1 ? 128 : 64, bn = choice == 3 ? 64 : 128;
    a.splits = (uint32_t)plan >> 8;
    SSD_REQUIRE(!gn_sums || a.splits > 1 || (H * W) % bm == 0, "conv2d_nhwc_f32x2_presplit: fused GroupNorm statistics need H*W to be a multiple of the M tile");
    a.m_tiles = (a.M + bm - 1) / bm; a.n_tiles = Cout / bn;
    float* const ws = a.splitk_ws;
    if (a.splits > 1 && !ws) {
        if (hipMemsetAsync(y, 0, (size_t)a.M * Cout * 4, st) != hipSuccess) return ssdnerf_fail(SSDNERF_E_LAUNCH, "conv2d_nhwc_f32x2_presplit: memset failed");
        a.splitk_ws = (float*)y;
    }
    const dim3 grid(a.m_tiles * a.n_tiles * a.splits);
    if (choice == 1) hipLaunchKernelGGL((k_conv_igemm_bf16<2, 2, 2, 2, 2, false, true>), grid, dim3(256), 0, st, a);
    else if (choice == 2) hipLaunchKernelGGL((k_conv_igemm_bf16<1, 2, 2, 2, 3, false, true>), grid, dim3(256), 0, st, a);
    else hipLaunchKernelGGL((k_conv_igemm_bf16<1, 1, 2, 2, CV_NS_SMALL, false, true>), grid, dim3(256), 0, st, a);
    if (a.splits > 1) cv_launch_finish(a, true, ws, st);
    SSD_CHECK_LAUNCH("conv2d_nhwc_f32x2_presplit");
    return SSDNERF_OK;
}

extern "C" int ssdnerf_conv2d_nhwc_bf16_supported(uint32_t Cin, uint32_t Cout, uint32_t ksize, uint32_t stride, uint32_t upsample) {
    return Cin > 0 && Cout > 0 && (Cin % 8 == 0) && (Cout % 8 == 0) && (ksize == 1 || ksize == 3) && (stride == 1 || stride == 2) && !(upsample && stride != 1);
}

extern "C" int ssdnerf_conv2d_nhwc_bf16(const void* x, const void* x2, uint32_t Cin1, const void* w, const float* bias, const void* residual, void* y, uint32_t B,
                                        uint32_t H, uint32_t W, uint32_t Cin, uint32_t Cout, uint32_t ksize, uint32_t stride, uint32_t upsample, void* gn_sums, uint32_t gn_groups,
                                        int tile_hint, void* splitk_ws, size_t splitk_ws_bytes, int splits_hint, void* stream) {
    if (B == 0 || H == 0 || W == 0) return SSDNERF_OK;
    SSD_REQUIRE(x && w && y, "conv2d_nhwc_bf16: null pointer");
    if (const int e = cv_check_layer("conv2d_nhwc_bf16", x2, Cin1, Cin, Cout, ksize, stride, upsample)) return e;
    if (const int e = cv_check_gn("conv2d_nhwc_bf16", gn_sums, gn_groups, Cout)) return e;
    ConvArgs a = cv_args(x, x2, Cin1, w, bias, residual, y, B, H, W, Cin, Cout, ksize, stride, upsample, gn_sums, gn_groups, splitk_ws, splitk_ws_bytes);
    SSD_REQUIRE((uint64_t)B * a.Ho * a.Wo < (1ull << 31) && (uint64_t)B * H * W * Cin * 2 < (1ull << 31), "conv2d_nhwc_bf16: tensor too large (32-bit buffer offsets)");
    const bool c64 = Cin % 64 == 0 && a.Cin1 % 64 == 0;
    hipStream_t st = (hipStream_t)stream;
    if (tile_hint == 0 && c64 && Cout % 128 == 0 && ksize == 3 && stride == 1 && a.M >= 32768 && (!gn_sums || (a.Ho * a.Wo) % 256 == 0)
        && ((!upsample && (W == 128 || W == 64) && (H * W) % 256 == 0) || (upsample && a.M >= 131072)))
        tile_hint = 6;
    if (tile_hint == 5 || tile_hint == 6) {
        SSD_REQUIRE(c64 && Cout % 128 == 0, "conv2d_nhwc_bf16: the 256 x 128 kernel needs Cin %% 64 == 0 and Cout %% 128 == 0");
        SSD_REQUIRE(!gn_sums || (a.Ho * a.Wo) % 256 == 0, "conv2d_nhwc_bf16: fused GroupNorm statistics need Ho*Wo to be a multiple of the M tile");
#ifdef CV_PP_TIMING
        a.splitk_ws = (float*)splitk_ws;
#endif
        const bool pp_rows = tile_hint == 6 && ksize == 3 && stride == 1 && !upsample && (W == 128 || W == 64 || W == 32) && (H * W) % 256 == 0;
        if (pp_rows) cv_launch_pp<true>(a, st); else cv_launch_pp<false>(a, st);
        SSD_CHECK_LAUNCH("conv2d_nhwc_bf16");
        return SSDNERF_OK;
    }
    int choice; uint32_t splits;
    cv_plan(a.M, Cin, Cout, ksize, tile_hint, a.splitk_ws && Cout <= 1024, splits_hint, &choice, &splits);
    if (choice != 3) SSD_REQUIRE(Cout % 128 == 0, "conv2d_nhwc_bf16: 128-wide tiles need Cout %% 128 == 0");
    SSD_REQUIRE(!gn_sums || splits > 1 || (a.Ho * a.Wo) % (choice == 4 ? 256 : choice == 1 ? 128 : 64) == 0, "conv2d_nhwc_bf16: fused GroupNorm statistics need Ho*Wo to be a multiple of the M tile");
    a.splits = splits;
    const bool rows = c64 && choice == 1 && splits == 1 && ksize == 3 && stride == 1 && !upsample && (W == 128 || W == 64 || W == 32) && (H * W) % 128 == 0;
    if (rows) {
        a.m_tiles = (a.M + 127) / 128; a.n_tiles = Cout / 128;
        hipLaunchKernelGGL(k_conv3x3_bf16_rows, dim3(a.m_tiles * a.n_tiles), dim3(256), 0, st, a);
    } else if (choice == 4) cv_launch<2, 2, 4, 2, 3>(a, st); else if (choice == 1) cv_launch<2, 2, 2, 2, 2>(a, st); else if (choice == 2) cv_launch<1, 2, 2, 2, 3>(a, st); else cv_launch<1, 1, 2, 2, CV_NS_SMALL>(a, st);
    if (splits > 1) cv_launch_finish(a, false, a.splitk_ws, st);
    SSD_CHECK_LAUNCH("conv2d_nhwc_bf16");
    return SSDNERF_OK;
}
```

ssdnerf_amd/csrc/groupnorm.hip:

```cpp
#include "common.h"
#include "gn_bwd_math.h"

#include <hip/hip_fp16.h>

namespace {

enum { GN_F32 = 0, GN_F16 = 1, GN_BF16 = 2 };

template <int DT> struct GnVec;
template <> struct GnVec<GN_F32> {
    static constexpr int V = 4;
    __device__ static void load(const void* p, size_t idx, float* f) {
        const float4 v = reinterpret_cast<const float4*>(p)[idx];
        f[0] = v.x; f[1] = v.y; f[2] = v.z; f[3] = v.w;
    }
    __device__ static uint4 raw(const void* p, size_t idx) { return reinterpret_cast<const uint4*>(p)[idx]; }
    __device__ static void cvt(const uint4& v, float* f) { f[0] = __uint_as_float(v.x); f[1] = __uint_as_float(v.y); f[2] = __uint_as_float(v.z); f[3] = __uint_as_float(v.w); }
    __device__ static void store(void* p, size_t idx, const float* f) { reinterpret_cast<float4*>(p)[idx] = make_float4(f[0], f[1], f[2], f[3]); }
    __device__ static float round(float x) { return x; }
    __device__ static void store_split(void* p, size_t idx, const float* f) {
        uint32_t hi[4], lo[4];
#pragma unroll
        for (int i = 0; i < 4; ++i) {
            hi[i] = __float_as_uint(f[i]) & 0xffff0000u;
            lo[i] = __float_as_uint(f[i] - __uint_as_float(hi[i]));
        }
        unsigned char* base = reinterpret_cast<unsigned char*>(p) + (idx >> 3) * 128 + (idx & 7) * 8;
        *reinterpret_cast<uint2*>(base) = make_uint2(__builtin_amdgcn_perm(hi[1], hi[0], 0x07060302u), __builtin_amdgcn_perm(hi[3], hi[2], 0x07060302u));
        *reinterpret_cast<uint2*>(base + 64) = make_uint2(__builtin_amdgcn_perm(lo[1], lo[0], 0x07060302u), __builtin_amdgcn_perm(lo[3], lo[2], 0x07060302u));
    }
};
template <> struct GnVec<GN_BF16> {
    static constexpr int V = 8;
    __device__ static void load(const void* p, size_t idx, float* f) {
        const uint4 v = reinterpret_cast<const uint4*>(p)[idx];
        const uint32_t w[4] = {v.x, v.y, v.z, v.w};
#pragma unroll
        for (int i = 0; i < 4; ++i) {
            f[2 * i] = __uint_as_float(w[i] << 16);
            f[2 * i + 1] = __uint_as_float(w[i] & 0xffff0000u);
        }
    }
    __device__ static uint4 raw(const void* p, size_t idx) { return reinterpret_cast<const uint4*>(p)[idx]; }
    __device__ static void cvt(const uint4& v, float* f) {
        const uint32_t w[4] = {v.x, v.y, v.z, v.w};
#pragma unroll
        for (int i = 0; i < 4; ++i) {
            f[2 * i] = __uint_as_float(w[i] << 16);
            f[2 * i + 1] = __uint_as_float(w[i] & 0xffff0000u);
        }
    }
    typedef float f2 __attribute__((ext_vector_type(2)));
    typedef __bf16 b2 __attribute__((ext_vector_type(2)));
    __device__ static uint32_t pack2(float lo, float hi) {
        const b2 r = __builtin_convertvector(f2{lo, hi}, b2);
        return *reinterpret_cast<const uint32_t*>(&r);
    }
    __device__ static void store(void* p, size_t idx, const float* f) {
        reinterpret_cast<uint4*>(p)[idx] = make_uint4(pack2(f[0], f[1]), pack2(f[2], f[3]), pack2(f[4], f[5]), pack2(f[6], f[7]));
    }
    __device__ static float round(float x) { return __uint_as_float(pack2(x, 0.f) << 16); }
};
template <> struct GnVec<GN_F16> {
    static constexpr int V = 8;
    __device__ static void load(const void* p, size_t idx, float* f) {
        union { uint4 u; _Float16 h[8]; } v;
        v.u = reinterpret_cast<const uint4*>(p)[idx];
#pragma unroll
        for (int i = 0; i < 8; ++i) f[i] = (float)v.h[i];
    }
    __device__ static uint4 raw(const void* p, size_t idx) { return reinterpret_cast<const uint4*>(p)[idx]; }
    __device__ static void cvt(const uint4& r, float* f) {
        union { uint4 u; _Float16 h[8]; } v;
        v.u = r;
#pragma unroll
        for (int i = 0; i < 8; ++i) f[i] = (float)v.h[i];
    }
    __device__ static void store(void* p, size_t idx, const float* f) {
        union { uint4 u; _Float16 h[8]; } v;
#pragma unroll
        for (int i = 0; i < 8; ++i) v.h[i] = (_Float16)f[i];
        reinterpret_cast<uint4*>(p)[idx] = v.u;
    }
    __device__ static float round(float x) { return (float)(_Float16)x; }
};

constexpr int GN_TPB = 256;
constexpr int GN_MAX_C = 2048;

template <int V>
__device__ __forceinline__ void gn_fold_to_groups(double* part, const double (&v)[V], bool active, uint32_t lane_row, uint32_t cv, uint32_t rif, uint32_t C,
                                                  uint32_t G, double* __restrict__ dst) {
    if (active) {
#pragma unroll
        for (int i = 0; i < V; ++i) part[lane_row * C + cv * V + i] = v[i];
    }
    __syncthreads();
    for (uint32_t c = threadIdx.x; c < C; c += GN_TPB) {
        double t = 0.0;
        for (uint32_t r = 0; r < rif; ++r) t += part[r * C + c];
        part[c] = t;
    }
    __syncthreads();
    const uint32_t cpg = C / G;
    for (uint32_t g = threadIdx.x; g < G; g += GN_TPB) {
        double t = 0.0;
        for (uint32_t i = 0; i < cpg; ++i) t += part[g * cpg + i];
        atomicAdd(&dst[(size_t)g * 2], t);
    }
    __syncthreads();
}

template <int DT>
__global__ __launch_bounds__(GN_TPB) void k_gn_stats(const void* __restrict__ x, const void* __restrict__ x2, uint32_t C1, const float* __restrict__ pre_bias,
                                                      uint32_t HW, uint32_t C, uint32_t G, uint32_t rows_per_block, double* __restrict__ sums) {
    constexpr int V = GnVec<DT>::V;
    __shared__ double part[GN_TPB * V];
    const uint32_t tpr = C / V, rif = GN_TPB / tpr;
    const uint32_t lane_row = threadIdx.x / tpr, cv = threadIdx.x % tpr;
    const uint32_t b = blockIdx.y, row0 = blockIdx.x * rows_per_block;
    const uint32_t tpr1 = C1 / V;
    const bool second = cv >= tpr1;
    const void* src = second ? x2 : x;
    const uint32_t stpr = second ? tpr - tpr1 : tpr1, scv = second ? cv - tpr1 : cv;
    double s[V], q[V];
#pragma unroll
    for (int i = 0; i < V; ++i) { s[i] = 0.0; q[i] = 0.0; }
    if (lane_row < rif) {
        const size_t base = ((size_t)b * HW + row0) * stpr + scv;
        for (uint32_t r = lane_row; r < rows_per_block; r += rif) {
            float f[V];
            GnVec<DT>::load(src, base + (size_t)r * stpr, f);
#pragma unroll
            for (int i = 0; i < V; ++i) { const double v = f[i]; s[i] += v; q[i] = __builtin_fma(v, v, q[i]); }
        }
        if (pre_bias) {
            const double n = (double)((rows_per_block - lane_row + rif - 1) / rif);
#pragma unroll
            for (int i = 0; i < V; ++i) { const double pb = pre_bias[cv * V + i]; q[i] += pb * (2.0 * s[i] + n * pb); s[i] += n * pb; }
        }
    }
    gn_fold_to_groups<V>(part, s, lane_row < rif, lane_row, cv, rif, C, G, sums + (size_t)b * G * 2);
    gn_fold_to_groups<V>(part, q, lane_row < rif, lane_row, cv, rif, C, G, sums + (size_t)b * G * 2 + 1);
}

template <int DT, bool RUNS = false>
__global__ __launch_bounds__(GN_TPB) void k_gn_apply(const void* __restrict__ x, const void* __restrict__ x2, uint32_t C1, const float* __restrict__ pre_bias,
                                                      uint32_t HW, uint32_t C, uint32_t G, uint32_t rows_per_block, const double* __restrict__ sums, const float* __restrict__ gamma,
                                                      const float* __restrict__ beta, const float* __restrict__ scale_shift, uint32_t ss_stride, float eps,
                                                      int act, void* __restrict__ y, const double* __restrict__ sums2 = nullptr) {
    constexpr int V = GnVec<DT>::V;
    __shared__ float fa[GN_MAX_C], fb[GN_MAX_C];
    const uint32_t tpr = C / V, rif = GN_TPB / tpr;
    const uint32_t lane_row = threadIdx.x / tpr, cv = threadIdx.x % tpr;
    const uint32_t b = blockIdx.y, row0 = blockIdx.x * rows_per_block;
    const uint32_t cpg = C / G;
    const double inv_n = 1.0 / ((double)HW * (double)cpg);
    __shared__ double grp[RUNS ? 2 * GN_TPB : 2];
    if (RUNS) {
        const uint32_t R1 = C1 / 4, R2 = C / 4 - R1, rpg = cpg / 4;
        for (uint32_t g = threadIdx.x; g < G; g += GN_TPB) {
            double gs = 0.0, gq = 0.0;
            for (uint32_t r0 = g * rpg; r0 < (g + 1) * rpg; r0 += 8) {
                double2 v[8];
#pragma unroll
                for (uint32_t k = 0; k < 8; ++k) {
                    const uint32_t r = r0 + k;
                    const double* p = r < R1 ? sums + ((size_t)b * R1 + r) * 2 : sums2 + ((size_t)b * R2 + (r - R1)) * 2;
                    v[k] = r < (g + 1) * rpg ? *reinterpret_cast<const double2*>(p) : make_double2(0.0, 0.0);
                }
#pragma unroll
                for (uint32_t k = 0; k < 8; ++k) { gs += v[k].x; gq += v[k].y; }
            }
            grp[2 * g] = gs; grp[2 * g + 1] = gq;
        }
        __syncthreads();
    }
    for (uint32_t c = threadIdx.x; c < C; c += GN_TPB) {
        const uint32_t g = c / cpg;
        const double gs = RUNS ? grp[2 * g] : sums[((size_t)b * G + g) * 2 + 0], gq = RUNS ? grp[2 * g + 1] : sums[((size_t)b * G + g) * 2 + 1];
        const double mean = gs * inv_n;
        double var = gq * inv_n - mean * mean;
        var = var > 0.0 ? var : 0.0;
        const float rstd = (float)(1.0 / sqrt(var + (double)eps));
        float a = rstd * gamma[c];
        float o = __builtin_fmaf((pre_bias ? pre_bias[c] : 0.f) - (float)mean, a, beta[c]);
        if (scale_shift) {
            const float sc = 1.0f + scale_shift[(size_t)b * ss_stride + c], sh = scale_shift[(size_t)b * ss_stride + C + c];
            a *= sc;
            o = __builtin_fmaf(o, sc, sh);
        }
        fa[c] = a; fb[c] = o;
    }
    __syncthreads();
    if (lane_row >= rif) return;
    float a[V], o[V];
#pragma unroll
    for (int i = 0; i < V; ++i) { a[i] = fa[cv * V + i]; o[i] = fb[cv * V + i]; }
    const uint32_t tpr1 = C1 / V;
    const bool second = cv >= tpr1;
    const void* src = second ? x2 : x;
    const uint32_t stpr = second ? tpr - tpr1 : tpr1, scv = second ? cv - tpr1 : cv;
    const size_t sbase = ((size_t)b * HW + row0) * stpr + scv;
    const size_t base = ((size_t)b * HW + row0) * tpr + cv;
#ifndef GN_APPLY_UNROLL
#define GN_APPLY_UNROLL 2
#endif
    constexpr int UR = GN_APPLY_UNROLL;
    for (uint32_t r0 = lane_row; r0 < rows_per_block; r0 += rif * UR) {
        float f[UR][V];
#pragma unroll
        for (int k = 0; k < UR; ++k)
            if (r0 + k * rif < rows_per_block) GnVec<DT>::load(src, sbase + (size_t)(r0 + k * rif) * stpr, f[k]);
        typedef float f2 __attribute__((ext_vector_type(2)));
#pragma unroll
        for (int k = 0; k < UR; ++k) {
            if (r0 + k * rif >= rows_per_block) break;
#pragma unroll
            for (int i = 0; i < V; i += 2) {
                f2 v = __builtin_elementwise_fma(f2{f[k][i], f[k][i + 1]}, f2{a[i], a[i + 1]}, f2{o[i], o[i + 1]});
                if (act & 1) {
                    const f2 u = v * f2{-1.4426950408889634f, -1.4426950408889634f};
                    const f2 d = f2{__builtin_amdgcn_exp2f(u.x), __builtin_amdgcn_exp2f(u.y)} + f2{1.0f, 1.0f};
                    v = v * f2{__builtin_amdgcn_rcpf(d.x), __builtin_amdgcn_rcpf(d.y)};
                }
                f[k][i] = v.x; f[k][i + 1] = v.y;
            }
            if constexpr (DT == GN_F32) {
                if (act & 2) { GnVec<DT>::store_split(y, base + (size_t)(r0 + k * rif) * tpr, f[k]); continue; }
            }
            GnVec<DT>::store(y, base + (size_t)(r0 + k * rif) * tpr, f[k]);
        }
    }
}

template <int DT>
__global__ __launch_bounds__(GN_TPB) void k_bias_residual(const void* __restrict__ x, const float* __restrict__ bias, const void* __restrict__ residual,
                                                           uint32_t HW, uint32_t C, uint32_t rows_per_block, void* __restrict__ y, double* __restrict__ sums,
                                                           uint32_t G) {
    constexpr int V = GnVec<DT>::V;
    __shared__ double part[GN_TPB * V];
    const uint32_t tpr = C / V, rif = GN_TPB / tpr;
    const uint32_t lane_row = threadIdx.x / tpr, cv = threadIdx.x % tpr;
    const uint32_t b = blockIdx.y, row0 = blockIdx.x * rows_per_block;
    double s[V], q[V];
#pragma unroll
    for (int i = 0; i < V; ++i) { s[i] = 0.0; q[i] = 0.0; }
    if (lane_row < rif) {
        float bv[V];
#pragma unroll
        for (int i = 0; i < V; ++i) bv[i] = bias ? bias[cv * V + i] : 0.f;
        const size_t base = ((size_t)b * HW + row0) * tpr + cv;
        for (uint32_t r = lane_row; r < rows_per_block; r += rif) {
            float f[V], rr[V];
            GnVec<DT>::load(x, base + (size_t)r * tpr, f);
#pragma unroll
            for (int i = 0; i < V; ++i) f[i] += bv[i];
            if (residual) {
                GnVec<DT>::load(residual, base + (size_t)r * tpr, rr);
#pragma unroll
                for (int i = 0; i < V; ++i) f[i] += rr[i];
            }
            GnVec<DT>::store(y, base + (size_t)r * tpr, f);
            if (sums) {
#pragma unroll
                for (int i = 0; i < V; ++i) { const double v = GnVec<DT>::round(f[i]); s[i] += v; q[i] = __builtin_fma(v, v, q[i]); }
            }
        }
    }
    if (!sums) return;
    gn_fold_to_groups<V>(part, s, lane_row < rif, lane_row, cv, rif, C, G, sums + (size_t)b * G * 2);
    gn_fold_to_groups<V>(part, q, lane_row < rif, lane_row, cv, rif, C, G, sums + (size_t)b * G * 2 + 1);
}

__device__ __forceinline__ void gn_bwd_group_table(uint32_t b, uint32_t HW, uint32_t C, uint32_t G, const double* __restrict__ fsums, float eps, int act,
                                                   float* __restrict__ g_mean, float* __restrict__ g_rstd, const double* __restrict__ fsums2 = nullptr, uint32_t C1 = 0) {
    const uint32_t cpg = C / G;
    const double inv_n = 1.0 / ((double)HW * (double)cpg);
    for (uint32_t g = threadIdx.x; g < G; g += GN_TPB) {
        double gs, gq;
        if (act & 4) {
            gs = 0.0; gq = 0.0;
            const uint32_t rpg = cpg / 4, R1 = fsums2 ? C1 / 4 : C / 4, R2 = C / 4 - R1;
            for (uint32_t r = g * rpg; r < (g + 1) * rpg; ++r) {
                const double2 v = *reinterpret_cast<const double2*>(r < R1 ? fsums + ((size_t)b * R1 + r) * 2 : fsums2 + ((size_t)b * R2 + (r - R1)) * 2);
                gs += v.x; gq += v.y;
            }
        } else {
            gs = fsums[((size_t)b * G + g) * 2 + 0]; gq = fsums[((size_t)b * G + g) * 2 + 1];
        }
        const double mean = gs * inv_n;
        double var = gq * inv_n - mean * mean;
        var = var > 0.0 ? var : 0.0;
        g_mean[g] = (float)mean;
        g_rstd[g] = (float)(1.0 / sqrt(var + (double)eps));
    }
}

#ifndef GN_BWD_UNROLL
#define GN_BWD_UNROLL 4
#endif
#ifndef GN_BWD_REPLICAS
#define GN_BWD_REPLICAS 8
#endif
__device__ __forceinline__ void gn_bwd_channel_table(uint32_t b, uint32_t C, uint32_t G, const float* __restrict__ g_mean, const float* __restrict__ g_rstd,
                                                     const float* __restrict__ gamma, const float* __restrict__ beta, const float* __restrict__ scale_shift,
                                                     uint32_t ss_stride, float* __restrict__ tab) {
    const uint32_t cpg = C / G;
    for (uint32_t c = threadIdx.x; c < C; c += GN_TPB) {
        const uint32_t g = c / cpg;
        float A, O, K, M, R;
        ssdg_coeffs_from(g_mean[g], g_rstd[g], gamma[c], beta[c], scale_shift != nullptr,
                         scale_shift ? scale_shift[(size_t)b * ss_stride + c] : 0.f, scale_shift ? scale_shift[(size_t)b * ss_stride + C + c] : 0.f, &A, &O, &K, &M, &R);
        tab[c] = A; tab[C + c] = O; tab[2 * C + c] = K;
    }
}
template <int V>
__device__ __forceinline__ void gn_bwd_coeffs(uint32_t cv, uint32_t C, uint32_t G, const float* __restrict__ g_mean, const float* __restrict__ g_rstd,
                                              const float* __restrict__ tab, float* A, float* O, float* K, float* M, float* R) {
    const uint32_t cpg = C / G;
#pragma unroll
    for (int i = 0; i < V; i += 4) {
        const float4 a = *reinterpret_cast<const float4*>(tab + cv * V + i), o = *reinterpret_cast<const float4*>(tab + C + cv * V + i),
                     k = *reinterpret_cast<const float4*>(tab + 2 * C + cv * V + i);
        A[i] = a.x; A[i + 1] = a.y; A[i + 2] = a.z; A[i + 3] = a.w;
        O[i] = o.x; O[i + 1] = o.y; O[i + 2] = o.z; O[i + 3] = o.w;
        K[i] = k.x; K[i + 1] = k.y; K[i + 2] = k.z; K[i + 3] = k.w;
    }
#pragma unroll
    for (int i = 0; i < V; ++i) {
        const uint32_t g = (cv * V + i) / cpg;
        M[i] = g_mean[g]; R[i] = g_rstd[g];
    }
}

template <int DT>
__global__ __launch_bounds__(GN_TPB) void k_gn_bwd_stats(const void* __restrict__ x, const void* __restrict__ dy, uint32_t HW, uint32_t C, uint32_t G,
                                                          uint32_t rows_per_block, const double* __restrict__ fsums, const float* __restrict__ gamma,
                                                          const float* __restrict__ beta, const float* __restrict__ scale_shift, uint32_t ss_stride, float eps,
                                                          int act, double* __restrict__ bsums, const void* __restrict__ x2, uint32_t C1, const double* __restrict__ fsums2) {
    constexpr int V = GnVec<DT>::V;
    __shared__ float part_s[GN_TPB * V], part_q[GN_TPB * V];
    const uint32_t tpr = C / V, rif = GN_TPB / tpr;
    const uint32_t lane_row = threadIdx.x / tpr, cv = threadIdx.x % tpr;
    const uint32_t b = blockIdx.y, row0 = blockIdx.x * rows_per_block;
    constexpr int UR = GN_BWD_UNROLL;
    const size_t base = ((size_t)b * HW + row0) * tpr + cv;
    const uint32_t tpr1 = (x2 ? C1 : C) / V;
    const bool second = cv >= tpr1;
    const void* const xs = second ? x2 : x;
    const uint32_t stpr = second ? tpr - tpr1 : tpr1;
    const size_t sbase = ((size_t)b * HW + row0) * stpr + (second ? cv - tpr1 : cv);
    uint4 rx[UR], rd[UR];
    auto issue = [&](uint32_t r0) {
#pragma unroll
        for (int k = 0; k < UR; ++k)
            if (r0 + k * rif < rows_per_block) {
                rx[k] = GnVec<DT>::raw(xs, sbase + (size_t)(r0 + k * rif) * stpr);
                rd[k] = GnVec<DT>::raw(dy, base + (size_t)(r0 + k * rif) * tpr);
            }
    };
    if (lane_row < rif) issue(lane_row);
    extern __shared__ __attribute__((aligned(16))) float ctab[];
    float* const gtab = ctab + 3 * C;
    gn_bwd_group_table(b, HW, C, G, fsums, eps, act, gtab, gtab + G, fsums2, C1);
    __syncthreads();
    gn_bwd_channel_table(b, C, G, gtab, gtab + G, gamma, beta, scale_shift, ss_stride, ctab);
    __syncthreads();
    float A[V], O[V], K[V], M[V], R[V];
    if (lane_row < rif) gn_bwd_coeffs<V>(cv, C, G, gtab, gtab + G, ctab, A, O, K, M, R);
// ... 35 lines not shown
        double* rep = bsums + (size_t)(blockIdx.x % GN_BWD_REPLICAS) * gridDim.y * G * 2;
        atomicAdd(&rep[((size_t)b * G + g) * 2 + 0], ds);
        atomicAdd(&rep[((size_t)b * G + g) * 2 + 1], dq);
    }
}

template <int DT>
__global__ __launch_bounds__(GN_TPB) void k_gn_bwd_apply(const void* __restrict__ x, const void* __restrict__ dy, uint32_t HW, uint32_t C, uint32_t G,
                                                          uint32_t rows_per_block, const double* __restrict__ fsums, const double* __restrict__ bsums,
                                                          const float* __restrict__ gamma, const float* __restrict__ beta, const float* __restrict__ scale_shift,
                                                          uint32_t ss_stride, float eps, int act, void* __restrict__ dx, const void* __restrict__ x2, uint32_t C1,
                                                          const double* __restrict__ fsums2, void* __restrict__ dx2) {
    constexpr int V = GnVec<DT>::V;
    const uint32_t tpr = C / V, rif = GN_TPB / tpr;
    const uint32_t lane_row = threadIdx.x / tpr, cv = threadIdx.x % tpr;
    const uint32_t b = blockIdx.y, row0 = blockIdx.x * rows_per_block;
    extern __shared__ __attribute__((aligned(16))) float ctab[];
    float* const gtab = ctab + 3 * C;
    const uint32_t cpg = C / G;
    constexpr int UR = GN_BWD_UNROLL;
    const size_t base = ((size_t)b * HW + row0) * tpr + cv;
    const uint32_t tpr1 = (x2 ? C1 : C) / V;
    const bool second = cv >= tpr1;
    const void* const xs = second ? x2 : x;
    void* const dxs = second ? dx2 : dx;
    const uint32_t stpr = second ? tpr - tpr1 : tpr1;
    const size_t sbase = ((size_t)b * HW + row0) * stpr + (second ? cv - tpr1 : cv);
    uint4 rx[UR], rd[UR];
    auto issue = [&](uint32_t r0) {
#pragma unroll
        for (int k = 0; k < UR; ++k)
            if (r0 + k * rif < rows_per_block) {
                rx[k] = GnVec<DT>::raw(xs, sbase + (size_t)(r0 + k * rif) * stpr);
                rd[k] = GnVec<DT>::raw(dy, base + (size_t)(r0 + k * rif) * tpr);
            }
    };
    if (lane_row < rif) issue(lane_row);
    gn_bwd_group_table(b, HW, C, G, fsums, eps, act, gtab, gtab + G, fsums2, C1);
    {
        const double inv_n = 1.0 / ((double)HW * (double)cpg);
        for (uint32_t g = threadIdx.x; g < G; g += GN_TPB) {
            double s0 = 0.0, s1 = 0.0;
#pragma unroll
            for (uint32_t r = 0; r < GN_BWD_REPLICAS; ++r) {
                const double2 v = *reinterpret_cast<const double2*>(bsums + ((size_t)r * gridDim.y * G + (size_t)b * G + g) * 2);
                s0 += v.x; s1 += v.y;
            }
            gtab[2 * G + g] = (float)(s0 * inv_n);
            gtab[3 * G + g] = (float)(s1 * inv_n);
        }
    }
    __syncthreads();
    gn_bwd_channel_table(b, C, G, gtab, gtab + G, gamma, beta, scale_shift, ss_stride, ctab);
    __syncthreads();
    if (lane_row >= rif) return;
    float A[V], O[V], K[V], M[V], R[V], m1[V], m2[V];
    gn_bwd_coeffs<V>(cv, C, G, gtab, gtab + G, ctab, A, O, K, M, R);
#pragma unroll
    for (int i = 0; i < V; ++i) {
        const uint32_t g = (cv * V + i) / cpg;
        m1[i] = gtab[2 * G + g];
        m2[i] = gtab[3 * G + g];
    }
    for (uint32_t r0 = lane_row; r0 < rows_per_block; r0 += rif * UR) {
        if (r0 != lane_row) issue(r0);
#pragma unroll
        for (int k = 0; k < UR; ++k) {
            if (r0 + k * rif >= rows_per_block) break;
            float f[V], d[V];
            GnVec<DT>::cvt(rx[k], f);
            GnVec<DT>::cvt(rd[k], d);
#pragma unroll
            for (int i = 0; i < V; ++i) {
                float p, xh;
                ssdg_elem(f[i], d[i], A[i], O[i], K[i], M[i], R[i], act & 1, &p, &xh);
                f[i] = ssdg_dx(p, xh, R[i], m1[i], m2[i]);
            }
            if constexpr (DT == GN_F32) {
                if (act & 2) { GnVec<DT>::store_split(dx, base + (size_t)(r0 + k * rif) * tpr, f); continue; }
            }
            GnVec<DT>::store(dxs, sbase + (size_t)(r0 + k * rif) * stpr, f);
        }
    }
}

__global__ __launch_bounds__(256) void k_split_f32(const float* __restrict__ x, void* __restrict__ y, size_t n_vec, uint32_t vpp, size_t x_stride) {
    for (size_t i = (size_t)blockIdx.x * 256 + threadIdx.x; i < n_vec; i += (size_t)gridDim.x * 256) {
        const size_t pix = i / vpp;
        const float4 v = *reinterpret_cast<const float4*>(x + pix * x_stride + (i - pix * vpp) * 4);
        const float f[4] = {v.x, v.y, v.z, v.w};
        GnVec<GN_F32>::store_split(y, i, f);
    }
}

#ifndef GN_FWD_STATS_BLOCKS
#define GN_FWD_STATS_BLOCKS 1024
#define GN_FWD_STATS_ROWS 64
#endif
#ifndef GN_FWD_APPLY_BLOCKS
#define GN_FWD_APPLY_BLOCKS 2048
#define GN_FWD_APPLY_ROWS 16
#endif
#ifndef GN_BWD_STATS_BLOCKS
#define GN_BWD_STATS_BLOCKS 1024
#endif
#ifndef GN_BWD_MIN_TRIPS
#define GN_BWD_MIN_TRIPS 1
#endif
#ifndef GN_BWD_APPLY_BLOCKS
#define GN_BWD_APPLY_BLOCKS 1024
#endif
uint32_t gn_rows_per_block(uint32_t B, uint32_t HW, uint32_t min_blocks, uint32_t min_rows) {
    uint32_t rows = HW;
    while (rows > min_rows && (rows % 2 == 0) && (uint64_t)B * (HW / rows) < min_blocks) rows /= 2;
    return rows;
}

}

extern "C" size_t ssdnerf_group_norm_workspace(uint32_t B, uint32_t G) { return (size_t)B * G * 2 * sizeof(double); }
extern "C" size_t ssdnerf_group_norm_backward_workspace(uint32_t B, uint32_t G) { return (size_t)GN_BWD_REPLICAS * B * G * 2 * sizeof(double); }

extern "C" int ssdnerf_group_norm_nhwc(const void* x, const void* x2, uint32_t C1, int dtype, uint32_t B, uint32_t HW, uint32_t C, uint32_t G, const float* pre_bias, const float* gamma,
                                       const float* beta, const float* scale_shift, uint32_t scale_shift_stride, float eps, int act, void* workspace,
                                       int workspace_state, void* y, void* stream) {
    if (B == 0 || HW == 0 || C == 0) return SSDNERF_OK;
    SSD_REQUIRE(x && y && gamma && beta && workspace, "group_norm_nhwc: null pointer");
    SSD_REQUIRE(dtype == GN_F32 || dtype == GN_F16 || dtype == GN_BF16, "group_norm_nhwc: dtype must be 0 (f32), 1 (f16) or 2 (bf16)");
    const uint32_t V = dtype == GN_F32 ? 4 : 8;
    SSD_REQUIRE(G > 0 && C % G == 0, "group_norm_nhwc: channels must be divisible by groups");
    SSD_REQUIRE(!scale_shift || scale_shift_stride >= 2 * C, "group_norm_nhwc: scale_shift_stride must be >= 2*C");
    SSD_REQUIRE(C % V == 0 && C / V <= GN_TPB && C <= GN_MAX_C, "group_norm_nhwc: channel count must be a multiple of the 16-byte vector and <= 1024 (f32) / 2048 (16-bit)");
    if (!x2) C1 = C;
    SSD_REQUIRE(C1 <= C && C1 % V == 0 && (x2 || C1 == C), "group_norm_nhwc: the first tensor's channel count must be a multiple of the 16-byte vector and <= C");
    SSD_REQUIRE(!(act & 2) || (dtype == GN_F32 && C % 32 == 0), "group_norm_nhwc: the pre-split output (act & 2) needs fp32 and C % 32 == 0");
    hipStream_t st = (hipStream_t)stream;
    const uint32_t rows_s = gn_rows_per_block(B, HW, GN_FWD_STATS_BLOCKS, GN_FWD_STATS_ROWS), rows_a = gn_rows_per_block(B, HW, GN_FWD_APPLY_BLOCKS, GN_FWD_APPLY_ROWS);
    const dim3 grid_s(HW / rows_s, B), grid_a(HW / rows_a, B), block(GN_TPB);
    SSD_REQUIRE(workspace_state >= 0 && workspace_state <= 2 && !(workspace_state == 2 && pre_bias), "group_norm_nhwc: bad workspace_state");
    const bool stats_ready = workspace_state == 2;
    if (workspace_state == 0 && hipMemsetAsync(workspace, 0, ssdnerf_group_norm_workspace(B, G), st) != hipSuccess)
        return ssdnerf_fail(SSDNERF_E_LAUNCH, "group_norm_nhwc: memset failed");
    double* sums = (double*)workspace;
#define SSD_GN_LAUNCH(DT)                                                                                                                    \
    if (!stats_ready) hipLaunchKernelGGL(k_gn_stats<DT>, grid_s, block, 0, st, x, x2, C1, pre_bias, HW, C, G, rows_s, sums);                                            \
    hipLaunchKernelGGL(k_gn_apply<DT>, grid_a, block, 0, st, x, x2, C1, pre_bias, HW, C, G, rows_a, (const double*)sums, gamma, beta, scale_shift,    \
                       scale_shift_stride, eps, act, y);
    if (dtype == GN_F32) { SSD_GN_LAUNCH(GN_F32) } else if (dtype == GN_F16) { SSD_GN_LAUNCH(GN_F16) } else { SSD_GN_LAUNCH(GN_BF16) }
#undef SSD_GN_LAUNCH
    SSD_CHECK_LAUNCH("group_norm_nhwc");
    return SSDNERF_OK;
}

extern "C" int ssdnerf_group_norm_nhwc_runs(const void* x, const void* x2, uint32_t C1, int dtype, uint32_t B, uint32_t HW, uint32_t C, uint32_t G, const float* gamma,
                                            const float* beta, const float* scale_shift, uint32_t scale_shift_stride, float eps, int act, const void* runs1,
                                            const void* runs2, void* y, void* stream) {
    if (B == 0 || HW == 0 || C == 0) return SSDNERF_OK;
    SSD_REQUIRE(x && y && gamma && beta && runs1 && (!x2 || runs2), "group_norm_nhwc_runs: null pointer");
    SSD_REQUIRE(dtype == GN_F32 || dtype == GN_F16 || dtype == GN_BF16, "group_norm_nhwc_runs: dtype must be 0 (f32), 1 (f16) or 2 (bf16)");
    const uint32_t V = dtype == GN_F32 ? 4 : 8;
    SSD_REQUIRE(G > 0 && G <= GN_TPB && C % G == 0 && (C / G) % 4 == 0, "group_norm_nhwc_runs: groups must be multiples of 4 channels (and at most 256 groups)");
    SSD_REQUIRE(!scale_shift || scale_shift_stride >= 2 * C, "group_norm_nhwc_runs: scale_shift_stride must be >= 2*C");
    SSD_REQUIRE(C % V == 0 && C / V <= GN_TPB && C <= GN_MAX_C, "group_norm_nhwc_runs: channel count must be a multiple of the 16-byte vector and <= 1024 (f32) / 2048 (16-bit)");
    if (!x2) C1 = C;
    SSD_REQUIRE(C1 <= C && C1 % V == 0 && (x2 || C1 == C), "group_norm_nhwc_runs: the first tensor's channel count must be a multiple of the 16-byte vector and <= C");
    SSD_REQUIRE(!(act & 2) || (dtype == GN_F32 && C % 32 == 0), "group_norm_nhwc_runs: the pre-split output (act & 2) needs fp32 and C % 32 == 0");
    hipStream_t st = (hipStream_t)stream;
    const uint32_t rows_a = gn_rows_per_block(B, HW, GN_FWD_APPLY_BLOCKS, GN_FWD_APPLY_ROWS);
    const dim3 grid_a(HW / rows_a, B), block(GN_TPB);
#define SSD_GN_LAUNCH(DT)                                                                                                                    \
    hipLaunchKernelGGL((k_gn_apply<DT, true>), grid_a, block, 0, st, x, x2, C1, (const float*)nullptr, HW, C, G, rows_a, (const double*)runs1, gamma, beta, scale_shift,    \
                       scale_shift_stride, eps, act, y, (const double*)runs2);
    if (dtype == GN_F32) { SSD_GN_LAUNCH(GN_F32) } else if (dtype == GN_F16) { SSD_GN_LAUNCH(GN_F16) } else { SSD_GN_LAUNCH(GN_BF16) }
#undef SSD_GN_LAUNCH
    SSD_CHECK_LAUNCH("group_norm_nhwc_runs");
    return SSDNERF_OK;
}

extern "C" int ssdnerf_group_norm_nhwc_backward_cat(const void* x, const void* x2, uint32_t C1, const void* dy, int dtype, uint32_t B, uint32_t HW, uint32_t C, uint32_t G,
                                                    const float* gamma, const float* beta, const float* scale_shift, uint32_t scale_shift_stride, float eps, int act,
                                                    const void* fwd_sums, const void* fwd_sums2, void* bwd_workspace, int bwd_workspace_is_zero, void* dx, void* dx2,
                                                    void* stream) {
    if (B == 0 || HW == 0 || C == 0) return SSDNERF_OK;
    SSD_REQUIRE(x && dy && dx && gamma && beta && fwd_sums && bwd_workspace, "group_norm_nhwc_backward: null pointer");
    SSD_REQUIRE(dtype == GN_F32 || dtype == GN_F16 || dtype == GN_BF16, "group_norm_nhwc_backward: dtype must be 0 (f32), 1 (f16) or 2 (bf16)");
    const uint32_t V = dtype == GN_F32 ? 4 : 8;
    SSD_REQUIRE(G > 0 && C % G == 0, "group_norm_nhwc_backward: channels must be divisible by groups");
    SSD_REQUIRE(!scale_shift || scale_shift_stride >= 2 * C, "group_norm_nhwc_backward: scale_shift_stride must be >= 2*C");
    SSD_REQUIRE(C % V == 0 && C / V <= GN_TPB && C <= GN_MAX_C, "group_norm_nhwc_backward: channel count must be a multiple of the 16-byte vector and <= 1024 (f32) / 2048 (16-bit)");
    SSD_REQUIRE(!(act & 2) || (dtype == GN_F32 && C % 32 == 0), "group_norm_nhwc_backward: the pre-split dx (act & 2) needs fp32 and C % 32 == 0");
    SSD_REQUIRE(!(act & 4) || (C / G) % 4 == 0, "group_norm_nhwc_backward: run-level forward sums (act & 4) need groups of a multiple of 4 channels");
    if (x2) {
        SSD_REQUIRE(dx2 && C1 > 0 && C1 < C && C1 % V == 0, "group_norm_nhwc_backward_cat: needs dx2 and 0 < C1 < C, C1 a multiple of the 16-byte vector");
        SSD_REQUIRE(!(act & 2), "group_norm_nhwc_backward_cat: no pre-split dx for two sources");
        SSD_REQUIRE(!(act & 4) || (fwd_sums2 && C1 % 4 == 0), "group_norm_nhwc_backward_cat: run-level sums need fwd_sums2 and C1 % 4 == 0");
    } else {
        C1 = C; fwd_sums2 = nullptr; dx2 = nullptr;
    }
    hipStream_t st = (hipStream_t)stream;
    const uint32_t rif = GN_TPB / (C / V) ? GN_TPB / (C / V) : 1;
    const uint32_t rows_s = gn_rows_per_block(B, HW, GN_BWD_STATS_BLOCKS, rif * GN_BWD_MIN_TRIPS), rows_a = gn_rows_per_block(B, HW, GN_BWD_APPLY_BLOCKS, rif * GN_BWD_MIN_TRIPS);
    const dim3 grid_s(HW / rows_s, B), grid_a(HW / rows_a, B), block(GN_TPB);
    if (!bwd_workspace_is_zero && hipMemsetAsync(bwd_workspace, 0, ssdnerf_group_norm_backward_workspace(B, G), st) != hipSuccess)
        return ssdnerf_fail(SSDNERF_E_LAUNCH, "group_norm_nhwc_backward: memset failed");
#define SSD_GNB_LAUNCH(DT)                                                                                                                              \
    hipLaunchKernelGGL(k_gn_bwd_stats<DT>, grid_s, block, ((size_t)2 * G + 3 * C) * 4, st, x, dy, HW, C, G, rows_s, (const double*)fwd_sums, gamma, beta, scale_shift, scale_shift_stride, \
                       eps, act, (double*)bwd_workspace, x2, C1, (const double*)fwd_sums2);                                                            \
    hipLaunchKernelGGL(k_gn_bwd_apply<DT>, grid_a, block, ((size_t)4 * G + 3 * C) * 4, st, x, dy, HW, C, G, rows_a, (const double*)fwd_sums, (const double*)bwd_workspace, gamma, beta,   \
                       scale_shift, scale_shift_stride, eps, act, dx, x2, C1, (const double*)fwd_sums2, dx2);
    if (dtype == GN_F32) { SSD_GNB_LAUNCH(GN_F32) } else if (dtype == GN_F16) { SSD_GNB_LAUNCH(GN_F16) } else { SSD_GNB_LAUNCH(GN_BF16) }
#undef SSD_GNB_LAUNCH
    SSD_CHECK_LAUNCH("group_norm_nhwc_backward");
    return SSDNERF_OK;
}

extern "C" int ssdnerf_group_norm_nhwc_backward(const void* x, const void* dy, int dtype, uint32_t B, uint32_t HW, uint32_t C, uint32_t G, const float* gamma,
                                                const float* beta, const float* scale_shift, uint32_t scale_shift_stride, float eps, int act,
                                                const void* fwd_sums, void* bwd_workspace, int bwd_workspace_is_zero, void* dx, void* stream) {
    return ssdnerf_group_norm_nhwc_backward_cat(x, nullptr, C, dy, dtype, B, HW, C, G, gamma, beta, scale_shift, scale_shift_stride, eps, act, fwd_sums, nullptr, bwd_workspace,
                                                bwd_workspace_is_zero, dx, nullptr, stream);
}

extern "C" int ssdnerf_bias_residual_nhwc(const void* x, int dtype, uint32_t B, uint32_t HW, uint32_t C, const float* bias, const void* residual, void* y,
                                          void* gn_sums, uint32_t gn_groups, void* stream) {
    if (B == 0 || HW == 0 || C == 0) return SSDNERF_OK;
    SSD_REQUIRE(x && y, "bias_residual_nhwc: null pointer");
    SSD_REQUIRE(dtype == GN_F32 || dtype == GN_F16 || dtype == GN_BF16, "bias_residual_nhwc: dtype must be 0 (f32), 1 (f16) or 2 (bf16)");
    const uint32_t V = dtype == GN_F32 ? 4 : 8;
    SSD_REQUIRE(C % V == 0 && C / V <= GN_TPB && C <= GN_MAX_C, "bias_residual_nhwc: channel count must be a multiple of the 16-byte vector and <= 1024 (f32) / 2048 (16-bit)");
    SSD_REQUIRE(!gn_sums || (gn_groups > 0 && C % gn_groups == 0), "bias_residual_nhwc: channels must be divisible by groups");
    const uint32_t rows = gn_rows_per_block(B, HW, GN_FWD_APPLY_BLOCKS, GN_FWD_APPLY_ROWS);
    hipStream_t st = (hipStream_t)stream;
    const dim3 grid(HW / rows, B), block(GN_TPB);
#define SSD_BR_LAUNCH(DT) hipLaunchKernelGGL(k_bias_residual<DT>, grid, block, 0, st, x, bias, residual, HW, C, rows, y, (double*)gn_sums, gn_groups ? gn_groups : 1u);
    if (dtype == GN_F32) { SSD_BR_LAUNCH(GN_F32) } else if (dtype == GN_F16) { SSD_BR_LAUNCH(GN_F16) } else { SSD_BR_LAUNCH(GN_BF16) }
#undef SSD_BR_LAUNCH
    SSD_CHECK_LAUNCH("bias_residual_nhwc");
    return SSDNERF_OK;
}

extern "C" int ssdnerf_split_f32_nhwc(const void* x, void* y, uint64_t pixels, uint32_t C, uint64_t x_stride, void* stream) {
    if (pixels == 0 || C == 0) return SSDNERF_OK;
    SSD_REQUIRE(x && y && x != y, "split_f32_nhwc: null pointer / in place");
    SSD_REQUIRE(C % 32 == 0, "split_f32_nhwc: C %% 32 == 0");
    if (x_stride == 0) x_stride = C;
    SSD_REQUIRE(x_stride >= C && x_stride % 4 == 0 && ((uintptr_t)x & 15) == 0, "split_f32_nhwc: the source's pixel stride must be >= C and, like its base, a multiple of 16 bytes");
    const size_t n_vec = (size_t)pixels * (C / 4);
    const size_t blocks = (n_vec + 255) / 256;
    hipLaunchKernelGGL(k_split_f32, dim3((unsigned)(blocks < 8192 ? blocks : 8192)), dim3(256), 0, (hipStream_t)stream, (const float*)x, y, n_vec, C / 4, (size_t)x_stride);
    SSD_CHECK_LAUNCH("split_f32_nhwc");
    return SSDNERF_OK;
}
```

ssdnerf_amd/unet_fast.py:

```python
from __future__ import annotations

import ctypes
import math
import os
from typing import Dict, List, Optional, Tuple

import torch
import torch.nn.functional as F

from . import _cabi as C

_GN_DTYPE = {torch.float32: 0, torch.float16: 1, torch.bfloat16: 2}

_FALLBACK_LOG: Optional[list] = None


def _lib_call(what: str):
    if _FALLBACK_LOG is not None:
        _FALLBACK_LOG.append(what)


def group_norm_nhwc(x: torch.Tensor, groups: int, gamma: torch.Tensor, beta: torch.Tensor, scale_shift: Optional[torch.Tensor], eps: float,
                    act: bool, workspace: torch.Tensor, out: Optional[torch.Tensor] = None, pre_bias: Optional[torch.Tensor] = None,
                    workspace_is_zero: bool = False, stats_ready: bool = False, x2: Optional[torch.Tensor] = None,
                    runs: Optional[Tuple[torch.Tensor, Optional[torch.Tensor]]] = None, split_out: bool = False) -> torch.Tensor:
    act_bits = int(bool(act)) | (2 if split_out else 0)
    if x.dim() == 4:
        B, C1, H, W = x.shape
        HW = H * W
        if not x.is_contiguous(memory_format=torch.channels_last):
            raise RuntimeError("group_norm_nhwc: 4-D input must be channels_last")
        Cc = C1
        if x2 is not None:
            if x2.dim() != 4 or x2.shape[0] != B or x2.shape[2:] != x.shape[2:] or x2.dtype != x.dtype or not x2.is_contiguous(memory_format=torch.channels_last):
                raise RuntimeError("group_norm_nhwc: x2 must match x in batch, spatial size, dtype and layout")
            Cc = C1 + x2.shape[1]
    else:
        B, HW, Cc = x.shape
        C1 = Cc
        if x2 is not None or not x.is_contiguous():
            raise RuntimeError("group_norm_nhwc: 3-D input must be a single contiguous (B, T, C) tensor")
    if out is not None:
        y = out
    elif x2 is None:
        y = torch.empty_like(x)
    else:
        y = torch.empty((B, Cc, H, W), dtype=x.dtype, device=x.device, memory_format=torch.channels_last)
    ss_stride = 0
    if scale_shift is not None:
        assert scale_shift.dtype == torch.float32 and scale_shift.shape == (B, 2 * Cc) and scale_shift.stride(1) == 1
        ss_stride = scale_shift.stride(0)
    if runs is not None:
        assert pre_bias is None and (x2 is None) == (runs[1] is None)
        C.check(C.lib().ssdnerf_group_norm_nhwc_runs(C.ptr(x), C.ptr(x2), C.u32(C1), _GN_DTYPE[x.dtype], C.u32(B), C.u32(HW), C.u32(Cc), C.u32(groups), C.ptr(gamma),
                                                      C.ptr(beta), C.ptr(scale_shift), C.u32(ss_stride), C.f32(eps), act_bits, C.ptr(runs[0]), C.ptr(runs[1]),
                                                      C.ptr(y), C.stream()), "group_norm_nhwc_runs")
        return y
    C.check(C.lib().ssdnerf_group_norm_nhwc(C.ptr(x), C.ptr(x2), C.u32(C1), _GN_DTYPE[x.dtype], C.u32(B), C.u32(HW), C.u32(Cc), C.u32(groups), C.ptr(pre_bias), C.ptr(gamma),
                                             C.ptr(beta), C.ptr(scale_shift), C.u32(ss_stride), C.f32(eps), act_bits, C.ptr(workspace),
                                             2 if stats_ready else int(bool(workspace_is_zero)), C.ptr(y), C.stream()),
            "group_norm_nhwc")
    return y


def group_norm_backward_workspace_doubles(B: int, groups: int) -> int:
    return int(C.lib().ssdnerf_group_norm_backward_workspace(C.u32(B), C.u32(groups))) // 8


def group_norm_nhwc_backward(x: torch.Tensor, dy: torch.Tensor, groups: int, gamma: torch.Tensor, beta: torch.Tensor, scale_shift: Optional[torch.Tensor],
                             eps: float, act: bool, fwd_sums: torch.Tensor, workspace: Optional[torch.Tensor] = None, split_out: bool = False,
                             sums_are_runs: bool = False) -> torch.Tensor:
    if x.dim() != 4 or not x.is_contiguous(memory_format=torch.channels_last) or dy.shape != x.shape or dy.dtype != x.dtype \
            or not dy.is_contiguous(memory_format=torch.channels_last):
        raise RuntimeError("group_norm_nhwc_backward: x and dy must be channels_last 4-D tensors of the same shape and dtype")
    B, Cc, H, W = x.shape
    ss_stride = 0
    if scale_shift is not None:
        assert scale_shift.dtype == torch.float32 and scale_shift.shape == (B, 2 * Cc) and scale_shift.stride(1) == 1
        ss_stride = scale_shift.stride(0)
    dx = torch.empty_like(x)
    need = group_norm_backward_workspace_doubles(B, groups)
    ws = workspace if workspace is not None else torch.zeros(need, dtype=torch.float64, device=x.device)
    if ws.numel() < need or ws.dtype != torch.float64:
        raise RuntimeError(f"group_norm_nhwc_backward: the workspace must hold {need} zeroed doubles (group_norm_backward_workspace_doubles)")
    C.check(C.lib().ssdnerf_group_norm_nhwc_backward(C.ptr(x), C.ptr(dy), _GN_DTYPE[x.dtype], C.u32(B), C.u32(H * W), C.u32(Cc), C.u32(groups), C.ptr(gamma),
                                                      C.ptr(beta), C.ptr(scale_shift), C.u32(ss_stride), C.f32(eps), int(bool(act)) | (2 if split_out else 0) | (4 if sums_are_runs else 0), C.ptr(fwd_sums), C.ptr(ws), 1,
                                                      C.ptr(dx), C.stream()), "group_norm_nhwc_backward")
    return dx


def group_norm_nhwc_backward_cat(x: torch.Tensor, x2: torch.Tensor, dy: torch.Tensor, groups: int, gamma: torch.Tensor, beta: torch.Tensor,
                                 scale_shift: Optional[torch.Tensor], eps: float, act: bool, fwd_sums: torch.Tensor, fwd_sums2: Optional[torch.Tensor] = None,
                                 workspace: Optional[torch.Tensor] = None):
    ok = lambda t: t.dim() == 4 and t.is_contiguous(memory_format=torch.channels_last)
    if not (ok(x) and ok(x2) and ok(dy)) or x.dtype != x2.dtype or x.dtype != dy.dtype or x.shape[0] != x2.shape[0] or x.shape[2:] != x2.shape[2:] \
            or dy.shape != (x.size(0), x.size(1) + x2.size(1), x.size(2), x.size(3)):
        raise RuntimeError("group_norm_nhwc_backward_cat: x, x2 and dy must be channels_last 4-D tensors of one dtype, dy over the concatenated channels")
    B, C1, H, W = x.shape
    Cc = C1 + x2.size(1)
    ss_stride = 0
    if scale_shift is not None:
        assert scale_shift.dtype == torch.float32 and scale_shift.shape == (B, 2 * Cc) and scale_shift.stride(1) == 1
        ss_stride = scale_shift.stride(0)
    dx, dx2 = torch.empty_like(x), torch.empty_like(x2)
    need = group_norm_backward_workspace_doubles(B, groups)
    ws = workspace if workspace is not None else torch.zeros(need, dtype=torch.float64, device=x.device)
    if ws.numel() < need or ws.dtype != torch.float64:
        raise RuntimeError(f"group_norm_nhwc_backward_cat: the workspace must hold {need} zeroed doubles")
    C.check(C.lib().ssdnerf_group_norm_nhwc_backward_cat(C.ptr(x), C.ptr(x2), C.u32(C1), C.ptr(dy), _GN_DTYPE[x.dtype], C.u32(B), C.u32(H * W), C.u32(Cc), C.u32(groups),
                                                          C.ptr(gamma), C.ptr(beta), C.ptr(scale_shift), C.u32(ss_stride), C.f32(eps),
                                                          int(bool(act)) | (4 if fwd_sums2 is not None else 0), C.ptr(fwd_sums), C.ptr(fwd_sums2), C.ptr(ws), 1, C.ptr(dx), C.ptr(dx2),
                                                          C.stream()), "group_norm_nhwc_backward_cat")
    return dx, dx2


def bias_residual_nhwc(x: torch.Tensor, bias: Optional[torch.Tensor], residual: Optional[torch.Tensor], gn_sums: Optional[torch.Tensor] = None,
                       gn_groups: int = 0) -> torch.Tensor:
    if x.dim() == 4:
        B, Cc, H, W = x.shape
        HW = H * W
        ok = x.is_contiguous(memory_format=torch.channels_last) and (residual is None or residual.is_contiguous(memory_format=torch.channels_last))
    else:
        B, HW, Cc = x.shape
        ok = x.is_contiguous() and (residual is None or residual.is_contiguous())
    if not ok or (residual is not None and (residual.shape != x.shape or residual.dtype != x.dtype)):
        raise RuntimeError("bias_residual_nhwc: input (and residual) must be channel-last with matching shape and dtype")
    C.check(C.lib().ssdnerf_bias_residual_nhwc(C.ptr(x), _GN_DTYPE[x.dtype], C.u32(B), C.u32(HW), C.u32(Cc), C.ptr(bias), C.ptr(residual), C.ptr(x),
                                                C.ptr(gn_sums), C.u32(gn_groups), C.stream()), "bias_residual_nhwc")
    return x


def conv2d_nhwc_bf16(x: torch.Tensor, w: torch.Tensor, bias: Optional[torch.Tensor] = None, residual: Optional[torch.Tensor] = None, stride: int = 1,
                     upsample: bool = False, gn_sums: Optional[torch.Tensor] = None, gn_groups: int = 0, tile_hint: int = 0,
                     splitk_ws: Optional[torch.Tensor] = None, splits_hint: int = 0, x2: Optional[torch.Tensor] = None) -> torch.Tensor:
    if x.dtype != torch.bfloat16 or w.dtype != torch.bfloat16:
        raise RuntimeError("conv2d_nhwc_bf16: bf16 tensors only")
    if not x.is_contiguous(memory_format=torch.channels_last) or not w.is_contiguous(memory_format=torch.channels_last):
        raise RuntimeError("conv2d_nhwc_bf16: input and weight must be channels_last")
    B, Cin1, H, W = x.shape
    Cin = Cin1
    if x2 is not None:
        if x2.dtype != torch.bfloat16 or not x2.is_contiguous(memory_format=torch.channels_last) or x2.shape[0] != B or x2.shape[2:] != x.shape[2:]:
            raise RuntimeError("conv2d_nhwc_bf16: x2 must match x in batch, spatial size, dtype and layout")
        Cin = Cin1 + x2.shape[1]
    Cout, Cin_w, k, k2 = w.shape
    if Cin_w != Cin or k != k2:
        raise RuntimeError("conv2d_nhwc_bf16: weight shape does not match the input")
    Hv, Wv = (2 * H, 2 * W) if upsample else (H, W)
    pad = k // 2
    Ho, Wo = (Hv + 2 * pad - k) // stride + 1, (Wv + 2 * pad - k) // stride + 1
    y = torch.empty((B, Cout, Ho, Wo), dtype=torch.bfloat16, device=x.device, memory_format=torch.channels_last)
    if residual is not None and (residual.shape != y.shape or residual.dtype != y.dtype or not residual.is_contiguous(memory_format=torch.channels_last)):
        raise RuntimeError("conv2d_nhwc_bf16: residual must match the output's shape, dtype and layout")
    C.check(C.lib().ssdnerf_conv2d_nhwc_bf16(C.ptr(x), C.ptr(x2), C.u32(Cin1), C.ptr(w), C.ptr(bias), C.ptr(residual), C.ptr(y), C.u32(B), C.u32(H), C.u32(W), C.u32(Cin), C.u32(Cout),
                                              C.u32(k), C.u32(stride), C.u32(int(upsample)), C.ptr(gn_sums), C.u32(gn_groups), int(tile_hint), C.ptr(splitk_ws),
                                              ctypes.c_size_t(0 if splitk_ws is None else splitk_ws.numel() * splitk_ws.element_size()), int(splits_hint),
                                              C.stream()),
            "conv2d_nhwc_bf16")
    return y


def split_bf16x2(w: torch.Tensor):
    hi = w.to(torch.bfloat16)
    lo = (w - hi.float()).to(torch.bfloat16)
    return hi, lo


def split_bf16x2_adjacent(w: torch.Tensor):
    hi, lo = split_bf16x2(w)
    buf = torch.empty((2, w.shape[0], w.shape[2], w.shape[3], w.shape[1]), dtype=torch.bfloat16, device=w.device)
    buf[0].copy_(hi.permute(0, 2, 3, 1))
    buf[1].copy_(lo.permute(0, 2, 3, 1))
    return buf[0].permute(0, 3, 1, 2), buf[1].permute(0, 3, 1, 2)


def presplit_supported(x: torch.Tensor, cout: int, k: int, with_stats: bool = False) -> int:
    if not (x.is_cuda and x.dtype == torch.float32):
        return 0
    return int(C.lib().ssdnerf_conv2d_nhwc_f32x2_presplit_supported(
        C.u32(x.size(0)), C.u32(x.size(2)), C.u32(x.size(3)), C.u32(x.size(1)), C.u32(cout), C.u32(k), int(with_stats)))


def nhwc_pixel_stride(x: torch.Tensor) -> int:
    if x.dim() != 4:
        return 0
    B, Cc, H, W = x.shape
    sb, sc, sh, sw = x.stride()
    if sc != 1 or sw < Cc or sh != W * sw or (B > 1 and sb != H * W * sw):
        return 0
    return int(sw)


def split_f32_nhwc(x: torch.Tensor) -> torch.Tensor:
    stride = nhwc_pixel_stride(x)
    if x.dtype != torch.float32 or stride == 0 or x.size(1) % 32 != 0 or stride % 4 != 0 or x.data_ptr() % 16 != 0:
        raise RuntimeError("split_f32_nhwc: channel-last fp32 (B, C, H, W) with C % 32 == 0 (dense, or a 16-byte aligned channel slice)")
    y = torch.empty((x.size(0), x.size(1), x.size(2), x.size(3)), dtype=torch.float32, device=x.device, memory_format=torch.channels_last)
    C.check(C.lib().ssdnerf_split_f32_nhwc(C.ptr(x), C.ptr(y), ctypes.c_uint64(x.size(0) * x.size(2) * x.size(3)), C.u32(x.size(1)), ctypes.c_uint64(stride),
                                           C.stream()), "split_f32_nhwc")
    return y


def conv2d_nhwc_f32x2_presplit(x_split: torch.Tensor, w_hi: torch.Tensor, w_lo: torch.Tensor, bias: Optional[torch.Tensor] = None,
                               residual: Optional[torch.Tensor] = None, gn_sums: Optional[torch.Tensor] = None, gn_groups: int = 0,
                               splitk_ws: Optional[torch.Tensor] = None, tile_hint: int = 0, splits_hint: int = 0) -> torch.Tensor:
    B, Cin, H, W = x_split.shape
    Cout, k = w_hi.shape[0], w_hi.shape[2]
    if not x_split.is_contiguous(memory_format=torch.channels_last) or x_split.dtype != torch.float32 or tuple(w_hi.shape[1:]) != (Cin, k, k) or k not in (1, 3):
        raise RuntimeError("conv2d_nhwc_f32x2_presplit: (B, Cin, H, W) channels_last carrier tensor and a (Cout, Cin, k, k) weight pair, k 1 | 3")
    y = torch.empty((B, Cout, H, W), dtype=torch.float32, device=x_split.device, memory_format=torch.channels_last)
    if residual is not None and (residual.shape != y.shape or residual.dtype != y.dtype or not residual.is_contiguous(memory_format=torch.channels_last)):
        raise RuntimeError("conv2d_nhwc_f32x2_presplit: residual must match the output's shape, dtype and layout")
    C.check(C.lib().ssdnerf_conv2d_nhwc_f32x2_presplit(C.ptr(x_split), C.ptr(w_hi), C.ptr(w_lo), C.ptr(bias), C.ptr(residual), C.ptr(y), C.u32(B), C.u32(H), C.u32(W),
                                                        C.u32(Cin), C.u32(Cout), C.u32(k), C.ptr(gn_sums), C.u32(gn_groups), int(tile_hint), int(splits_hint), C.ptr(splitk_ws),
                                                        ctypes.c_size_t(0 if splitk_ws is None else splitk_ws.numel() * splitk_ws.element_size()), C.stream()),
            "conv2d_nhwc_f32x2_presplit")
    return y


def conv2d_nhwc_f32x2(x: torch.Tensor, w_hi: torch.Tensor, w_lo: torch.Tensor, bias: Optional[torch.Tensor] = None, residual: Optional[torch.Tensor] = None,
                      stride: int = 1, upsample: bool = False, gn_sums: Optional[torch.Tensor] = None, gn_groups: int = 0, tile_hint: int = 0,
                      x2: Optional[torch.Tensor] = None, splits_hint: int = 0, splitk_ws: Optional[torch.Tensor] = None) -> torch.Tensor:
    if x.dtype != torch.float32 or w_hi.dtype != torch.bfloat16 or w_lo.dtype != torch.bfloat16:
        raise RuntimeError("conv2d_nhwc_f32x2: fp32 input, bf16 weight pair")
    if not (x.is_contiguous(memory_format=torch.channels_last) and w_hi.is_contiguous(memory_format=torch.channels_last) and w_lo.is_contiguous(memory_format=torch.channels_last)):
        raise RuntimeError("conv2d_nhwc_f32x2: input and weights must be channels_last")
    B, Cin1, H, W = x.shape
    Cin = Cin1
    if x2 is not None:
        if x2.dtype != torch.float32 or not x2.is_contiguous(memory_format=torch.channels_last) or x2.shape[0] != B or x2.shape[2:] != x.shape[2:]:
            raise RuntimeError("conv2d_nhwc_f32x2: x2 must match x in batch, spatial size, dtype and layout")
        Cin = Cin1 + x2.shape[1]
    Cout, Cin_w, k, k2 = w_hi.shape
    if Cin_w != Cin or k != k2 or w_lo.shape != w_hi.shape:
        raise RuntimeError("conv2d_nhwc_f32x2: weight shape does not match the input")
    Hv, Wv = (2 * H, 2 * W) if upsample else (H, W)
    pad = k // 2
    Ho, Wo = (Hv + 2 * pad - k) // stride + 1, (Wv + 2 * pad - k) // stride + 1
    plan = C.lib().ssdnerf_conv2d_nhwc_f32x2_plan(C.u32(B * Ho * Wo), C.u32(Cin), C.u32(Cout), C.u32(k), int(tile_hint), int(splits_hint))
    ws_bytes = 0 if splitk_ws is None else splitk_ws.numel() * splitk_ws.element_size()
    split = (plan >> 8) > 1 and ws_bytes < B * Ho * Wo * Cout * 4
    y = torch.empty((B, Cout, Ho, Wo), dtype=torch.float32, device=x.device, memory_format=torch.channels_last)
    if split:
        y.zero_()
    if residual is not None and (residual.shape != y.shape or residual.dtype != y.dtype or not residual.is_contiguous(memory_format=torch.channels_last)):
        raise RuntimeError("conv2d_nhwc_f32x2: residual must match the output's shape, dtype and layout")
    C.check(C.lib().ssdnerf_conv2d_nhwc_f32x2(C.ptr(x), C.ptr(x2), C.u32(Cin1), C.ptr(w_hi), C.ptr(w_lo), C.ptr(bias), C.ptr(residual), C.ptr(y), C.u32(B), C.u32(H),
                                               C.u32(W), C.u32(Cin), C.u32(Cout), C.u32(k), C.u32(stride), C.u32(int(upsample)), C.ptr(gn_sums), C.u32(gn_groups),
                                               int(tile_hint), int(splits_hint), int(split), C.ptr(splitk_ws), ctypes.c_size_t(ws_bytes), C.stream()), "conv2d_nhwc_f32x2")
    return y


def attention_qkv_bf16(qkv: torch.Tensor, heads: int) -> torch.Tensor:
    B, T, C3 = qkv.shape
    Cc = C3 // 3
    if qkv.dtype != torch.bfloat16 or not qkv.is_contiguous():
        raise RuntimeError("attention_qkv_bf16: contiguous bf16 input only")
    out = torch.empty((B, T, Cc), dtype=torch.bfloat16, device=qkv.device)
    C.check(C.lib().ssdnerf_attention_qkv_bf16(C.ptr(qkv), C.ptr(out), C.u32(B), C.u32(T), C.u32(heads), C.u32(Cc // heads), C.stream()), "attention_qkv_bf16")
    return out


def attention_qkv_f32(qkv: torch.Tensor, heads: int) -> torch.Tensor:
    B, T, C3 = qkv.shape
    Cc = C3 // 3
    if qkv.dtype != torch.float32 or not qkv.is_contiguous():
        raise RuntimeError("attention_qkv_f32: contiguous fp32 input only")
    out = torch.empty((B, T, Cc), dtype=torch.float32, device=qkv.device)
    C.check(C.lib().ssdnerf_attention_qkv_f32(C.ptr(qkv), C.ptr(out), C.u32(B), C.u32(T), C.u32(heads), C.u32(Cc // heads), C.stream()), "attention_qkv_f32")
    return out


def attention_qkv_f32_with_lse(qkv: torch.Tensor, heads: int):
    B, T, C3 = qkv.shape
    Cc = C3 // 3
    if qkv.dtype != torch.float32 or not qkv.is_contiguous():
        raise RuntimeError("attention_qkv_f32_with_lse: contiguous fp32 input only")
    out = torch.empty((B, T, Cc), dtype=torch.float32, device=qkv.device)
    lse = torch.empty((B, heads, T), dtype=torch.float32, device=qkv.device)
    C.check(C.lib().ssdnerf_attention_qkv_f32_lse(C.ptr(qkv), C.ptr(out), C.ptr(lse), C.u32(B), C.u32(T), C.u32(heads), C.u32(Cc // heads), C.stream()),
            "attention_qkv_f32_lse")
    return out, lse


def attention_qkv_f32_backward(qkv: torch.Tensor, out: torch.Tensor, dout: torch.Tensor, lse: torch.Tensor, heads: int) -> torch.Tensor:
    B, T, C3 = qkv.shape
    Cc = C3 // 3
    if any(t.dtype != torch.float32 or not t.is_contiguous() for t in (qkv, out, dout, lse)) or out.shape != (B, T, Cc) or dout.shape != out.shape:
        raise RuntimeError("attention_qkv_f32_backward: contiguous fp32 tensors of matching shapes only")
    dqkv = torch.empty_like(qkv)
    ws = torch.empty(B * heads * T, dtype=torch.float32, device=qkv.device)
    C.check(C.lib().ssdnerf_attention_qkv_f32_backward(C.ptr(qkv), C.ptr(out), C.ptr(dout), C.ptr(lse), C.ptr(dqkv), C.ptr(ws), C.u32(B), C.u32(T), C.u32(heads),
                                                        C.u32(Cc // heads), C.stream()), "attention_qkv_f32_backward")
    return dqkv


def attention_supported(dtype, T: int, ch: int) -> bool:
    return dtype in (torch.bfloat16, torch.float32) and ch % 8 == 0 and 8 <= ch <= 128 and T >= 1


def attention_qkv(qkv: torch.Tensor, heads: int) -> torch.Tensor:
    return attention_qkv_bf16(qkv, heads) if qkv.dtype == torch.bfloat16 else attention_qkv_f32(qkv, heads)


CAPTURE_MODE = os.environ.get("SSDNERF_GRAPH_CAPTURE_MODE", "thread_local")


class _Conv:
    __slots__ = ("w", "w_lo", "bias", "stride", "padding", "fold", "own", "cin", "cout")
    SPLITK_BYTES = 16 << 20

    def __init__(self, conv, dtype, pad_in: bool = False, pad_out: bool = False):
        weight = conv.weight.detach()
        if weight.dim() == 3:
            weight = weight[..., None]
            stride, padding, dilation, k, groups = (1, 1), (0, 0), (1, 1), (1, 1), conv.groups
        else:
            stride, padding, dilation, k, groups = conv.stride, conv.padding, conv.dilation, conv.kernel_size, conv.groups
        assert groups == 1
        self.cout, self.cin = int(weight.shape[0]), int(weight.shape[1])
        bias = conv.bias.detach().float() if conv.bias is not None else None
        pin = (-self.cin) % 8 if pad_in else 0
        pout = (-self.cout) % 8 if pad_out else 0
        if pin or pout:
            weight = F.pad(weight, (0, 0, 0, 0, 0, pin, 0, pout))
            if bias is not None and pout:
                bias = F.pad(bias, (0, pout))
        self.w = weight.to(dtype).contiguous(memory_format=torch.channels_last)
        self.bias = bias.contiguous() if bias is not None else None
        self.stride, self.padding = tuple(stride), tuple(padding)
        self.fold = weight.shape[0] % 8 == 0
        self.own = bool(dtype in (torch.bfloat16, torch.float32) and self.w.is_cuda and k[0] == k[1] and stride[0] == stride[1]
                        and tuple(padding) == (k[0] // 2, k[0] // 2) and tuple(dilation) == (1, 1)
                        and C.lib().ssdnerf_conv2d_nhwc_bf16_supported(int(weight.shape[1]), int(weight.shape[0]), k[0], stride[0], 0))
        self.w_lo = None
        if self.own and dtype == torch.float32 and _Conv.F32X2:
            self.w_lo = split_bf16x2_adjacent(weight.float())
            self.w = self.w_lo[0]
        elif dtype == torch.float32:
            self.own = False
        if not self.own and (pin or pout):
            self.__init__(conv, dtype)

    splitk_ws_by_device: dict = {}
    F32X2 = os.environ.get("SSDNERF_UNET_F32X2", "1") != "0"

    def takes_presplit(self, x, with_stats=False) -> bool:
        return bool(self.w_lo is not None and self.own and _Conv.PRESPLIT and self.stride[0] == 1 and int(self.w.shape[1]) == int(x.size(1))
                    and presplit_supported(x, int(self.w.shape[0]), int(self.w.shape[2]), with_stats))

    PRESPLIT = os.environ.get("SSDNERF_UNET_PRESPLIT", "1") != "0"

    def igemm(self, x, bias=None, residual=None, upsample=False, gn_sums=None, gn_groups=0, x2=None, presplit=False):
        if presplit:
            return conv2d_nhwc_f32x2_presplit(x, self.w_lo[0], self.w_lo[1], bias, residual, gn_sums, gn_groups, splitk_ws=shared_splitk_ws(x.device))
        if self.w_lo is not None:
            return conv2d_nhwc_f32x2(x, self.w_lo[0], self.w_lo[1], bias, residual, self.stride[0], upsample, gn_sums, gn_groups, x2=x2,
                                     splitk_ws=shared_splitk_ws(x.device))
        return conv2d_nhwc_bf16(x, self.w, bias, residual, self.stride[0], upsample, gn_sums, gn_groups, splitk_ws=shared_splitk_ws(x.device), x2=x2)

    def _w_lib(self):
        return self.w if self.w_lo is None else (self.w_lo[0].float() + self.w_lo[1].float()).contiguous(memory_format=torch.channels_last)

    def mm(self, x):
        _lib_call(f"conv2d {tuple(self.w.shape)}")
        return F.conv2d(x, self._w_lib(), None, self.stride, self.padding)

    def __call__(self, x):
        if self.own:
            return self.igemm(x, self.bias)
        if self.bias is None:
            return self.mm(x)
        if not self.fold:
            _lib_call(f"conv2d {tuple(self.w.shape)}")
            return F.conv2d(x, self.w, self.bias.to(self.w.dtype), self.stride, self.padding)
        return bias_residual_nhwc(self.mm(x), self.bias, None)


class _like:
    __slots__ = ("_x", "_c")

    def __init__(self, x, channels):
        self._x, self._c = x, channels

    is_cuda = property(lambda self: self._x.is_cuda)
    dtype = property(lambda self: self._x.dtype)

    def size(self, i):
        return self._c if i == 1 else self._x.size(i)


def shared_splitk_ws(device) -> Optional[torch.Tensor]:
    dev = torch.device(device)
    if dev.type != "cuda":
        return None
    idx = dev.index if dev.index is not None else torch.cuda.current_device()
    ws = _Conv.splitk_ws_by_device.get(idx)
    if ws is None:
        ws = _Conv.splitk_ws_by_device[idx] = torch.zeros(_Conv.SPLITK_BYTES // 4, dtype=torch.float32, device=torch.device("cuda", idx))
    return ws


class _GN:
    __slots__ = ("groups", "gamma", "beta", "eps")

    def __init__(self, gn: torch.nn.GroupNorm):
        self.groups, self.eps = gn.num_groups, gn.eps
        self.gamma, self.beta = gn.weight.detach().float().contiguous(), gn.bias.detach().float().contiguous()


class FastUnet:

    capture_by_default = True

    def __init__(self, net, dtype: torch.dtype = torch.float32, use_graph: Optional[bool] = None):
        from .unet import DenoisingResBlockMod, MultiHeadAttentionMod, DenoisingDownsampleMod, DenoisingUpsampleMod
        if net.num_classes != 0 or net.concat_cond_channels != 0:
            raise RuntimeError("FastUnet: label / concat conditioning is not on the hot path (use the module forward)")
        self.net, self.dtype = net, dtype
        self.use_graph = self.capture_by_default if use_graph is None else use_graph
        self.device = next(net.parameters()).device
        self._types = (DenoisingResBlockMod, MultiHeadAttentionMod, DenoisingDownsampleMod, DenoisingUpsampleMod)
        self._graphs: Dict[Tuple[int, int, int], tuple] = {}
        self.fallback_log: Optional[list] = None
        self.library_fallbacks: Optional[int] = None
        self._pack()

    @staticmethod
    def param_version(net):
        return hash(tuple((p.data_ptr(), p._version, p.device.index, p.dtype) for p in net.parameters()))

    def invalidate(self):
        self.version = None
        self._retire_graphs()
        self.fallback_log = None

    def _retire_graphs(self):
        self._graphs.clear()

    def _pack(self):
        net, dt = self.net, self.dtype
        Res, Att, Down, Up = self._types
        self.version = self.param_version(net)
        te = net.time_embedding
        self.te = (te.dim, te.max_period, te.blocks[0].weight.detach().float(), te.blocks[0].bias.detach().float(),
                   te.blocks[2].weight.detach().float(), te.blocks[2].bias.detach().float())
        emb_w: List[torch.Tensor] = []
        emb_b: List[torch.Tensor] = []
        self._emb_off = 0
        self._n_gn = 1

        def res(m):
            assert m.norm_with_embedding.use_scale_shift, "FastUnet implements the scale-shift norm the hot-path configs use"
            assert len(m.conv_2) == 2, "dropout is inactive at inference and must not be configured > 0 here"
            lin = m.norm_with_embedding.embedding_layer[1]
            off = self._emb_off
            emb_w.append(lin.weight.detach().float()); emb_b.append(lin.bias.detach().float())
            self._emb_off += lin.out_features
            conv2, shortcut = _Conv(m.conv_2[-1], dt), _Conv(m.shortcut, dt) if m.learnable_shortcut else None
            out_bias = conv2.bias if shortcut is None or shortcut.bias is None else (conv2.bias + shortcut.bias)
            self._n_gn += 2
            return ("res", _GN(m.conv_1[0]), _Conv(m.conv_1[2], dt), _GN(m.norm_with_embedding.norm), (off, lin.out_features), conv2, shortcut, out_bias)

        def att(m):
            assert m.groups == 1
            self._n_gn += 1
            return ("att", _GN(m.norm), m.num_heads, _Conv(m.qkv, dt), _Conv(m.proj, dt))

        def seq(block):
            ops = []
            for layer in block:
                if isinstance(layer, Res):
                    ops.append(res(layer))
                elif isinstance(layer, Att):
                    ops.append(att(layer))
                elif isinstance(layer, Down):
                    assert isinstance(layer.downsample, torch.nn.Conv2d)
                    ops.append(("conv", _Conv(layer.downsample, dt)))
                elif isinstance(layer, Up):
                    ops.append(("up", _Conv(layer.conv, dt) if layer.with_conv else None))
                elif isinstance(layer, torch.nn.Conv2d):
                    ops.append(("conv", _Conv(layer, dt)))
                else:
                    raise RuntimeError(f"FastUnet: unsupported layer {type(layer).__name__}")
            return ops

        self.in_ops = [seq(b) for b in net.in_blocks]
        stem = net.in_blocks[0][0]
        if len(net.in_blocks[0]) == 1 and isinstance(stem, torch.nn.Conv2d):
            self.in_ops[0] = [("conv", _Conv(stem, dt, pad_in=True))]
        self.stem_cin = self.in_ops[0][0][1].w.shape[1] if self.in_ops[0][0][0] == "conv" and self.in_ops[0][0][1].own else None
        self.mid_ops = seq(net.mid_blocks)
        self.out_ops = [seq(b) for b in net.out_blocks]
        self.head = (_GN(net.out.gn), _Conv(net.out.conv, dt, pad_out=True))
        self.emb_w, self.emb_b = torch.cat(emb_w, 0).contiguous(), torch.cat(emb_b, 0).contiguous()
        if self.device.type == "cuda":
            shared_splitk_ws(self.device)
        self._ws, self._ws_by_batch = None, {}
        self._max_c = max(int(p.shape[0]) for p in net.parameters() if p.dim() == 4)

    def _stats_slice(self, batch, channels=256):
        n = batch * (channels // 4) * 2
        ws = self._ws[self._ws_next:self._ws_next + n]
        self._ws_next += n
        assert ws.numel() == n, "GroupNorm statistics arena exhausted"
        return ws

    def _gn(self, x, gn: _GN, ss, act, pre_bias=None, stats=None, x2=None, stats2=None, split=False):
        Cc = (x.size(1) if x.dim() == 4 else x.size(2)) + (x2.size(1) if x2 is not None else 0)
        if stats is not None and (x2 is None or stats2 is not None) and (Cc // gn.groups) % 4 == 0:
            return group_norm_nhwc(x, gn.groups, gn.gamma, gn.beta, ss, gn.eps, act, stats, x2=x2, runs=(stats, stats2), split_out=split)
        return group_norm_nhwc(x, gn.groups, gn.gamma, gn.beta, ss, gn.eps, act, self._stats_slice(x.size(0)), pre_bias=pre_bias, workspace_is_zero=True,
                               x2=x2, split_out=split)

    def _can_fuse_stats(self, conv: _Conv, x, upsample=False):
        if not conv.own:
            return False
        hw = x.size(2) * x.size(3) * (4 if upsample else 1) // (conv.stride[0] * conv.stride[1])
        cout, cin, k = conv.w.size(0), conv.w.size(1), conv.w.size(2)
        if cout % 4 != 0:
            return False
        if hw > 128 * 256:
            return False
        if conv.w_lo is not None:
            plan = C.lib().ssdnerf_conv2d_nhwc_f32x2_plan(C.u32(x.size(0) * hw), C.u32(cin), C.u32(cout), C.u32(k), 0, 0)
            if plan >> 8 != 1:
                return True
            return hw % (128 if (plan & 0xff) == 1 else 64) == 0
        plan = C.lib().ssdnerf_conv2d_nhwc_bf16_plan(C.u32(x.size(0) * hw), C.u32(cin), C.u32(cout), C.u32(k), 0, 1, 0)
        if plan >> 8 != 1:
            return True
        return hw % (256 if (plan & 0xff) == 4 else 128 if (plan & 0xff) == 1 else 64) == 0

    def _conv_stats(self, conv: _Conv, x, bias=None, residual=None, upsample=False, x2=None, presplit=False):
        st = self._stats_slice(x.size(0), conv.w.size(0)) if self._can_fuse_stats(conv, x, upsample) else None
        return conv.igemm(x, bias, residual, upsample=upsample, gn_sums=st, gn_groups=conv.w.size(0) // 4 if st is not None else 0, x2=x2, presplit=presplit), st

    def _res(self, x, stats, op, ss_all, x2=None, stats2=None):
        _, gn1, conv1, gn2, (off, n), conv2, shortcut, out_bias = op
        ss = ss_all[:, off:off + n]
        own = conv1.own and conv2.own and (shortcut is None or shortcut.own)
        if x2 is not None and not (own and shortcut is not None and x.size(1) % 8 == 0 and x2.size(1) % 8 == 0):
            x, x2, stats, stats2 = torch.cat([x, x2], dim=1).contiguous(memory_format=torch.channels_last), None, None, None
        if own:
            cin1 = x.size(1) + (x2.size(1) if x2 is not None else 0)
            ps1 = conv1.w_lo is not None and conv1.takes_presplit(_like(x, cin1), with_stats=True)
            g1 = self._gn(x, gn1, None, True, stats=stats, x2=x2, stats2=stats2, split=ps1)
            h, st1 = self._conv_stats(conv1, g1, conv1.bias, presplit=ps1)
            ps2 = conv2.w_lo is not None and conv2.takes_presplit(h, with_stats=True)
            g2 = self._gn(h, gn2, ss, True, stats=st1, split=ps2)
            skip = shortcut.igemm(x, x2=x2) if shortcut is not None else x
            return self._conv_stats(conv2, g2, out_bias, skip, presplit=ps2)
        g1 = self._gn(x, gn1, None, True, stats=stats, x2=x2, stats2=stats2)
        h = conv1.mm(g1)
        h = conv2.mm(self._gn(h, gn2, ss, True, pre_bias=conv1.bias))
        return bias_residual_nhwc(h, out_bias, shortcut.mm(x) if shortcut is not None else x), None

    def _att(self, x, stats, op):
        _, gn, heads, qkv_conv, proj_conv = op
        B, Cc, H, W = x.shape
        T, ch = H * W, Cc // heads
        xt = x.permute(0, 2, 3, 1).reshape(B, T, Cc)
        own = qkv_conv.own and proj_conv.own and attention_supported(self.dtype, T, ch)
        ps = own and qkv_conv.w_lo is not None and qkv_conv.takes_presplit(x)
        xn = self._gn(xt, gn, None, False, stats=stats, split=ps)
        if own:
            qkv = qkv_conv.igemm(xn.view(B, H, W, Cc).permute(0, 3, 1, 2), qkv_conv.bias, presplit=ps)
            a = attention_qkv(qkv.permute(0, 2, 3, 1).reshape(B, T, 3 * Cc), heads)
            return self._conv_stats(proj_conv, a.view(B, H, W, Cc).permute(0, 3, 1, 2), proj_conv.bias, x)
        _lib_call(f"attention block C={Cc} T={T} (linear, sdpa, linear)")
        wqkv, wproj = qkv_conv._w_lib()[:, :, 0, 0], proj_conv._w_lib()[:, :, 0, 0]
        qkv = F.linear(xn, wqkv.to(xn.dtype), qkv_conv.bias.to(xn.dtype))
        if qkv.is_cuda and attention_supported(self.dtype, T, ch):
            a = attention_qkv(qkv, heads)
        else:
            q, k, v = qkv.view(B, T, heads, 3, ch).permute(3, 0, 2, 1, 4)
            a = F.scaled_dot_product_attention(q, k, v, scale=1.0 / math.sqrt(ch)).permute(0, 2, 1, 3).reshape(B, T, Cc)
        h = bias_residual_nhwc(F.linear(a, wproj.to(a.dtype), proj_conv.bias.to(a.dtype)), None, xt)
        return h.view(B, H, W, Cc).permute(0, 3, 1, 2), None

    def _run(self, ops, h, ss_all, stats=None, x2=None, stats2=None):
        for op in ops:
            kind = op[0]
            if kind == "res":
                h, stats = self._res(h, stats, op, ss_all, x2=x2, stats2=stats2)
                x2 = stats2 = None
            elif kind == "att":
                h, stats = self._att(h, stats, op)
            elif kind == "conv":
                h, stats = self._conv_stats(op[1], h, op[1].bias) if op[1].own else (op[1](h), None)
            elif kind == "up":
                if op[1] is not None and op[1].own:
                    h, stats = self._conv_stats(op[1], h, op[1].bias, upsample=True)
                else:
                    _lib_call("interpolate (+ library convolution)")
                    h = F.interpolate(h, scale_factor=2, mode="nearest")
                    if op[1] is not None:
                        h = op[1](h)
                    stats = None
        return h, stats

    def _time_embedding(self, t):
        dim, max_period, w0, b0, w2, b2 = self.te
        half = dim // 2
        freqs = torch.exp(-math.log(max_period) * torch.arange(0, half, dtype=torch.float32, device=t.device) / half)
        args = t[:, None].float() * freqs[None]
        e = torch.cat([torch.cos(args), torch.sin(args)], dim=-1)
        if dim % 2:
            e = torch.cat([e, torch.zeros_like(e[:, :1])], dim=-1)
        return F.linear(F.silu(F.linear(e, w0, b0)), w2, b2)

    def _forward(self, x_t, t):
        net = self.net
        if net.use_rescale_timesteps:
            t = t.float() * (1000.0 / net.num_timesteps)
        self._ws.zero_()
        self._ws_next = 0
        emb = self._time_embedding(t)
        ss_all = F.linear(F.silu(emb), self.emb_w, self.emb_b)
        if self.stem_cin is not None and self.stem_cin != x_t.size(1):
            h = torch.zeros((x_t.size(0), self.stem_cin) + tuple(x_t.shape[2:]), dtype=self.dtype, device=x_t.device).contiguous(memory_format=torch.channels_last)
            h[:, :x_t.size(1)] = x_t
        else:
            h = x_t.to(self.dtype).contiguous(memory_format=torch.channels_last)
        hs, stats = [], None
        for ops in self.in_ops:
            h, stats = self._run(ops, h, ss_all, stats)
            hs.append((h, stats))
        h, stats = self._run(self.mid_ops, h, ss_all, stats)
        for ops in self.out_ops:
            assert ops[0][0] == "res"
            skip, skip_stats = hs.pop()
            h, stats = self._run(ops, h, ss_all, stats, x2=skip, stats2=skip_stats)
        gn, conv = self.head
        out = conv(self._gn(h, gn, None, True, stats=stats))
        return out[:, :net.out_channels].float().contiguous()

    def _ensure_ws(self, B):
        ws = self._ws_by_batch.get(B)
        n = (2 * self._n_gn + 16) * B * (max(256, self._max_c) // 4) * 2
        if ws is None or ws.numel() != n:
            ws = self._ws_by_batch[B] = torch.zeros(n, dtype=torch.float64, device=self.device)
        self._ws = ws

    def session(self, x_t: torch.Tensor, t: torch.Tensor) -> "UnetSession":
        if not self.use_graph:
            raise RuntimeError("FastUnet.session needs graph capture")
        if self.version is None or self.param_version(self.net) != self.version or tuple(x_t.shape) not in self._graphs:
            self(x_t, t)
        g, sx, st, sy = self._graphs[tuple(x_t.shape)]
        return UnetSession(self, g, sx, st, sy)

    @torch.no_grad()
    def __call__(self, x_t: torch.Tensor, t: torch.Tensor) -> torch.Tensor:
        if self.version is None or self.param_version(self.net) != self.version:
            self._pack()
            self._retire_graphs()
        self._ensure_ws(x_t.size(0))
        if self.fallback_log is None:
            global _FALLBACK_LOG
            _FALLBACK_LOG = []
            try:
                y = self._forward(x_t, t)
            finally:
                self.fallback_log, _FALLBACK_LOG = _FALLBACK_LOG, None
            self.library_fallbacks = len(self.fallback_log)
            if not self.use_graph:
                return y
        if not self.use_graph:
            return self._forward(x_t, t)
        key = tuple(x_t.shape)
        entry = self._graphs.get(key)
        if entry is None:
            sx, st = x_t.clone(), t.clone()
            side = torch.cuda.Stream()
            side.wait_stream(torch.cuda.current_stream())
            with torch.cuda.stream(side):
                for _ in range(2):
                    self._forward(sx, st)
            torch.cuda.current_stream().wait_stream(side)
            g = torch.cuda.CUDAGraph()
            with torch.cuda.graph(g, capture_error_mode=CAPTURE_MODE):
                sy = self._forward(sx, st)
            entry = self._graphs[key] = (g, sx, st, sy)
        g, sx, st, sy = entry
        sx.copy_(x_t); st.copy_(t)
        g.replay()
        return sy.clone()


class UnetSession:
    __slots__ = ("ex", "graph", "x", "t", "y", "version")

    def __init__(self, ex: FastUnet, graph, x, t, y):
        self.ex, self.graph, self.x, self.t, self.y, self.version = ex, graph, x, t, y, ex.version

    def run(self) -> torch.Tensor:
        if self.ex.version != self.version or self.ex.param_version(self.ex.net) != self.version:
            raise RuntimeError("UnetSession: the network's weights changed since this session was opened; open a new one")
        self.graph.replay()
        return self.y
```

Before: 6.678 billion.

## Fold 1x1 shortcut conv into second residual conv as extra K chunks

In ResBlocks that have a 1x1 projection shortcut, the first GroupNorm now also writes a pre-split hi/lo copy of the raw input. The second conv's implicit-GEMM kernel is extended to run extra K iterations over that input and the shortcut weights. This drops the separate shortcut conv launch and the residual tensor round trip through memory. The cost is a longer K loop per tile, an extra split-input buffer written by the GroupNorm pass, and a split-K workspace requirement when the plan splits K.

```diff
diff --git a/include/ssdnerf_hip.h b/include/ssdnerf_hip.h
--- a/include/ssdnerf_hip.h
+++ b/include/ssdnerf_hip.h
@@ -244,6 +244,9 @@
 int ssdnerf_group_norm_nhwc_runs(const void* x, const void* x2, uint32_t C1, int dtype, uint32_t B, uint32_t HW, uint32_t C, uint32_t G, const float* gamma,
                                  const float* beta, const float* scale_shift, uint32_t scale_shift_stride, float eps, int act, const void* runs1,
                                  const void* runs2, void* y, void* stream);
+int ssdnerf_group_norm_nhwc_runs_raw_split(const void* x, const void* x2, uint32_t C1, uint32_t B, uint32_t HW, uint32_t C, uint32_t G, const float* gamma,
+                                           const float* beta, const float* scale_shift, uint32_t scale_shift_stride, float eps, int act, const void* runs1,
+                                           const void* runs2, void* y, void* xs, void* stream);
 
 size_t ssdnerf_group_norm_backward_workspace(uint32_t B, uint32_t G);
 
@@ -279,6 +282,10 @@
 int ssdnerf_conv2d_nhwc_f32x2_presplit(const void* x_split, const void* w_hi, const void* w_lo, const float* bias, const void* residual, void* y, uint32_t B,
                                        uint32_t H, uint32_t W, uint32_t Cin, uint32_t Cout, uint32_t ksize, void* gn_sums, uint32_t gn_groups,
                                        int tile_hint, int splits_hint, void* splitk_ws, size_t splitk_ws_bytes, void* stream);
+int ssdnerf_conv2d_nhwc_f32x2_presplit_plan(uint32_t M, uint32_t Cin, uint32_t Cout, uint32_t ksize, uint32_t Csc, int tile_hint, int splits_hint);
+int ssdnerf_conv2d_nhwc_f32x2_presplit_sc(const void* x_split, const void* w_hi, const void* w_lo, const void* xs, const void* w_sc, uint32_t Csc, const float* bias,
+                                          void* y, uint32_t B, uint32_t H, uint32_t W, uint32_t Cin, uint32_t Cout, uint32_t ksize, void* gn_sums, uint32_t gn_groups,
+                                          int tile_hint, int splits_hint, void* splitk_ws, size_t splitk_ws_bytes, void* stream);
 
 int ssdnerf_attention_qkv_bf16(const void* qkv, void* out, uint32_t B, uint32_t T, uint32_t heads, uint32_t ch, void* stream);
 int ssdnerf_attention_qkv_f32(const void* qkv, void* out, uint32_t B, uint32_t T, uint32_t heads, uint32_t ch, void* stream);
diff --git a/ssdnerf_amd/_cabi.py b/ssdnerf_amd/_cabi.py
--- a/ssdnerf_amd/_cabi.py
+++ b/ssdnerf_amd/_cabi.py
@@ -37,6 +37,7 @@
     "ssdnerf_philox_normal_fill", "ssdnerf_sde_step_v", "ssdnerf_sde_block_cap",
     "ssdnerf_prior_q_sample", "ssdnerf_prior_loss_v", "ssdnerf_prior_loss_v_backward", "ssdnerf_prior_block_cap", "ssdnerf_prior_blocks_per_sample",
     "ssdnerf_prior_loss_partials",
+    "ssdnerf_group_norm_nhwc_runs_raw_split", "ssdnerf_conv2d_nhwc_f32x2_presplit_plan", "ssdnerf_conv2d_nhwc_f32x2_presplit_sc",
 ]
 
 
diff --git a/ssdnerf_amd/csrc/conv_igemm.hip b/ssdnerf_amd/csrc/conv_igemm.hip
--- a/ssdnerf_amd/csrc/conv_igemm.hip
+++ b/ssdnerf_amd/csrc/conv_igemm.hip
@@ -24,6 +24,9 @@
     uint32_t ksize, stride, pad, upsample;
     uint32_t G;
     uint32_t m_tiles, n_tiles;
+    const unsigned char* xs;
+    const unsigned char* w_sc;
+    uint32_t Csc;
 };
 
 constexpr int CV_BK = 64;
@@ -292,6 +295,9 @@
     const __amdgpu_buffer_rsrc_t rs_x = cv_rsrc(a.x, (uint64_t)a.B * a.H * a.W * a.Cin1 * XB);
     const __amdgpu_buffer_rsrc_t rs_x2 = cv_rsrc(a.x2 ? a.x2 : a.x, a.x2 ? (uint64_t)a.B * a.H * a.W * (a.Cin - a.Cin1) * 2 : 0);
     const __amdgpu_buffer_rsrc_t rs_w = cv_rsrc(a.w, (uint64_t)a.Cout * taps * a.Cin * 2 * (PS ? 2 : 1));
+    const uint32_t sc_kt = PS ? a.Csc / KCH : 0u;
+    const __amdgpu_buffer_rsrc_t rs_xs = cv_rsrc(sc_kt ? a.xs : a.x, sc_kt ? (uint64_t)a.M * a.Csc * XB : 0);
+    const __amdgpu_buffer_rsrc_t rs_wsc = cv_rsrc(sc_kt ? a.w_sc : a.w, sc_kt ? (uint64_t)a.Cout * a.Csc * 4 : 0);
     uint32_t a_voff[A_INST], a_voff2[A_INST];
     const uint32_t Cin2 = a.Cin - a.Cin1;
     auto set_tap = [&](uint32_t tap) {
@@ -329,6 +335,21 @@
             cv_dma16(rs_w, sb + (wave * B_INST + i) * 1024, (!PT || b_sc[i] < nchunk) ? b_off[i] : CV_OOB, (tap * a.Cin + (second ? a.Cin1 : 0u) + cb) * 2);
     };
 
+    auto issue_sc = [&](uint32_t ci, uint32_t buf) {
+        unsigned char* sa = lds + buf * STAGE;
+        unsigned char* sb = sa + BM * CV_ROWB;
+#pragma unroll
+        for (int i = 0; i < A_INST; ++i) {
+            const uint32_t m = m0 + (wave * A_INST + i) * 8 + (lane >> 3);
+            cv_dma16(rs_xs, sa + (wave * A_INST + i) * 1024, m < a.M ? m * a.Csc * XB + a_sc[i] * 16 : CV_OOB, ci * KCH * XB);
+        }
+#pragma unroll
+        for (int i = 0; i < B_INST; ++i) {
+            const uint32_t r = (wave * B_INST + i) * 8 + (lane >> 3);
+            cv_dma16(rs_wsc, sb + (wave * B_INST + i) * 1024, (n0 + r) * a.Csc * 2 + (b_sc[i] & 3) * 16 + (b_sc[i] >> 2) * (a.Cout * a.Csc * 2), ci * KCH * 2);
+        }
+    };
+
     const uint32_t rd_row = lane & 31;
     const uint32_t rd_c0 = ((lane >> 5) ^ ((lane >> 1) & 7)) * 16;
     const uint32_t a_rd = (wm * 32 * TM + rd_row) * CV_ROWB + rd_c0;
@@ -342,14 +363,16 @@
 #pragma unroll
             for (int e = 0; e < 16; ++e) acc[i][j][e] = 0.f;
 
-    const uint32_t KT_all = taps * kc;
+    const uint32_t KT_all = taps * kc + sc_kt;
     const uint32_t kt_begin = (uint32_t)((uint64_t)split * KT_all / a.splits), KT = (uint32_t)((uint64_t)(split + 1) * KT_all / a.splits) - kt_begin;
-    uint32_t tap = kt_begin / kc, ci = kt_begin % kc, issued = 0;
+    const bool begin_sc = PS && kt_begin >= taps * kc;
+    uint32_t tap = begin_sc ? taps : kt_begin / kc, ci = begin_sc ? kt_begin - taps * kc : kt_begin % kc, issued = 0;
     uint32_t ci_mul = ci;
-    set_tap(tap);
+    if (!begin_sc) set_tap(tap);
     auto issue_next = [&]() {
-        if (issued) { if (++ci == kc) { ci = 0; ++tap; set_tap(tap); } }
-        issue(tap, ci, issued % NS);
+        if (issued) { if (++ci == ((PS && tap >= taps) ? sc_kt : kc)) { ci = 0; ++tap; if (!PS || tap < taps) set_tap(tap); } }
+        if (PS && tap >= taps) issue_sc(ci, issued % NS);
+        else issue(tap, ci, issued % NS);
         ++issued;
     };
 #pragma unroll
@@ -1468,6 +1491,7 @@
     a.splitk_ws = (splitk_ws && splitk_ws_bytes >= (size_t)a.M * Cout * 4) ? (float*)splitk_ws : nullptr;
     a.splits = 1;
     a.m_tiles = a.n_tiles = 0;
+    a.xs = a.w_sc = nullptr; a.Csc = 0;
     return a;
 }
 
@@ -1575,10 +1599,10 @@
     return SSDNERF_OK;
 }
 
-static int cv_ps_plan(uint32_t M, uint32_t Cin, uint32_t Cout, uint32_t ksize, int tile_hint, int splits_hint) {
+static int cv_ps_plan(uint32_t M, uint32_t Cin, uint32_t Cout, uint32_t ksize, int tile_hint, int splits_hint, uint32_t Csc = 0) {
     int choice = tile_hint;
     if (choice < 1 || choice > 3) choice = (Cout % 128 == 0 && (uint64_t)((M + 127) / 128) * (Cout / 128) >= 384) ? 1 : 3;
-    const uint32_t bm = choice == 1 ? 128 : 64, bn = choice == 3 ? 64 : 128, tiles = ((M + bm - 1) / bm) * ((Cout + bn - 1) / bn), KT = ksize * ksize * (Cin / 32);
+    const uint32_t bm = choice == 1 ? 128 : 64, bn = choice == 3 ? 64 : 128, tiles = ((M + bm - 1) / bm) * ((Cout + bn - 1) / bn), KT = ksize * ksize * (Cin / 32) + Csc / 32;
     uint32_t splits = 1;
     if (splits_hint > 0) splits = (uint32_t)splits_hint;
     else if (tiles < 384 && KT >= 64 && (uint64_t)M * Cout <= (1u << 21) && Cout <= 1024) {
@@ -1603,33 +1627,62 @@
     return 2;
 }
 
+extern "C" int ssdnerf_conv2d_nhwc_f32x2_presplit_plan(uint32_t M, uint32_t Cin, uint32_t Cout, uint32_t ksize, uint32_t Csc, int tile_hint, int splits_hint) {
+    return cv_ps_plan(M, Cin, Cout, ksize, tile_hint, splits_hint, Csc);
+}
+
+static int cv_presplit(const char* fn, const void* x_split, const void* w_hi, const void* w_lo, const void* xs, const void* w_sc, uint32_t Csc, const float* bias,
+                       const void* residual, void* y, uint32_t B, uint32_t H, uint32_t W, uint32_t Cin, uint32_t Cout, uint32_t ksize, void* gn_sums, uint32_t gn_groups,
+                       int tile_hint, int splits_hint, void* splitk_ws, size_t splitk_ws_bytes, void* stream);
+
 extern "C" int ssdnerf_conv2d_nhwc_f32x2_presplit(const void* x_split, const void* w_hi, const void* w_lo, const float* bias, const void* residual, void* y, uint32_t B,
                                                   uint32_t H, uint32_t W, uint32_t Cin, uint32_t Cout, uint32_t ksize, void* gn_sums, uint32_t gn_groups,
                                                   int tile_hint, int splits_hint, void* splitk_ws, size_t splitk_ws_bytes, void* stream) {
     if (B == 0 || H == 0 || W == 0) return SSDNERF_OK;
     SSD_REQUIRE(x_split && w_hi && w_lo && y, "conv2d_nhwc_f32x2_presplit: null pointer");
+    return cv_presplit("conv2d_nhwc_f32x2_presplit", x_split, w_hi, w_lo, nullptr, nullptr, 0, bias, residual, y, B, H, W, Cin, Cout, ksize, gn_sums, gn_groups, tile_hint,
+                       splits_hint, splitk_ws, splitk_ws_bytes, stream);
+}
+
+extern "C" int ssdnerf_conv2d_nhwc_f32x2_presplit_sc(const void* x_split, const void* w_hi, const void* w_lo, const void* xs, const void* w_sc, uint32_t Csc, const float* bias,
+                                                     void* y, uint32_t B, uint32_t H, uint32_t W, uint32_t Cin, uint32_t Cout, uint32_t ksize, void* gn_sums, uint32_t gn_groups,
+                                                     int tile_hint, int splits_hint, void* splitk_ws, size_t splitk_ws_bytes, void* stream) {
+    if (B == 0 || H == 0 || W == 0) return SSDNERF_OK;
+    SSD_REQUIRE(x_split && w_hi && w_lo && y && xs && w_sc, "conv2d_nhwc_f32x2_presplit_sc: null pointer");
+    SSD_REQUIRE(Csc > 0 && Csc % 32 == 0, "conv2d_nhwc_f32x2_presplit_sc: the shortcut's channel count must be a positive multiple of 32");
+    SSD_REQUIRE((uint64_t)B * H * W * Csc * 4 < (1ull << 31) && (uint64_t)Cout * Csc * 4 < (1ull << 31), "conv2d_nhwc_f32x2_presplit_sc: shortcut operand too large (32-bit buffer offsets)");
+    return cv_presplit("conv2d_nhwc_f32x2_presplit_sc", x_split, w_hi, w_lo, xs, w_sc, Csc, bias, nullptr, y, B, H, W, Cin, Cout, ksize, gn_sums, gn_groups, tile_hint,
+                       splits_hint, splitk_ws, splitk_ws_bytes, stream);
+}
+
+static int cv_presplit(const char* fn, const void* x_split, const void* w_hi, const void* w_lo, const void* xs, const void* w_sc, uint32_t Csc, const float* bias,
+                       const void* residual, void* y, uint32_t B, uint32_t H, uint32_t W, uint32_t Cin, uint32_t Cout, uint32_t ksize, void* gn_sums, uint32_t gn_groups,
+                       int tile_hint, int splits_hint, void* splitk_ws, size_t splitk_ws_bytes, void* stream) {
     int kind = ssdnerf_conv2d_nhwc_f32x2_presplit_supported(B, H, W, Cin, Cout, ksize, gn_sums != nullptr);
     if (tile_hint >= 1 && tile_hint <= 3 && ssdnerf_conv2d_nhwc_f32x2_presplit_supported(B, H, W, Cin, tile_hint == 3 ? 64 : 128, ksize, 0) && Cout % (tile_hint == 3 ? 64 : 128) == 0)
         kind = 2;
-    SSD_REQUIRE(kind != 0, "conv2d_nhwc_f32x2_presplit: layer not taken by a pre-split kernel (ask ssdnerf_conv2d_nhwc_f32x2_presplit_supported first)");
-    SSD_REQUIRE((const unsigned char*)w_lo == (const unsigned char*)w_hi + (size_t)Cout * ksize * ksize * Cin * 2, "conv2d_nhwc_f32x2_presplit: w_lo must lie directly behind w_hi");
-    if (const int e = cv_check_gn("conv2d_nhwc_f32x2_presplit", gn_sums, gn_groups, Cout)) return e;
+    SSD_REQUIRE(kind != 0, "%s: layer not taken by a pre-split kernel (ask ssdnerf_conv2d_nhwc_f32x2_presplit_supported first)", fn);
+    SSD_REQUIRE(!Csc || kind == 2, "%s: only the generic kernel's pre-split form folds a shortcut (the two-group row kernel's layers keep theirs as a launch of its own)", fn);
+    SSD_REQUIRE((const unsigned char*)w_lo == (const unsigned char*)w_hi + (size_t)Cout * ksize * ksize * Cin * 2, "%s: w_lo must lie directly behind w_hi", fn);
+    if (const int e = cv_check_gn(fn, gn_sums, gn_groups, Cout)) return e;
     hipStream_t st = (hipStream_t)stream;
     ConvArgs a = cv_args(x_split, nullptr, Cin, w_hi, bias, residual, y, B, H, W, Cin, Cout, ksize, 1, 0, gn_sums, gn_groups, splitk_ws, splitk_ws_bytes);
     if (kind == 1) {
         cv_launch_pp<true, true, true>(a, st);
-        SSD_CHECK_LAUNCH("conv2d_nhwc_f32x2_presplit");
+        SSD_CHECK_LAUNCH(fn);
         return SSDNERF_OK;
     }
-    const int plan = cv_ps_plan(a.M, Cin, Cout, ksize, tile_hint, splits_hint);
+    a.xs = (const unsigned char*)xs; a.w_sc = (const unsigned char*)w_sc; a.Csc = Csc;
+    const int plan = cv_ps_plan(a.M, Cin, Cout, ksize, tile_hint, splits_hint, Csc);
     const int choice = plan & 0xff;
     const uint32_t bm = choice == 1 ? 128 : 64, bn = choice == 3 ? 64 : 128;
     a.splits = (uint32_t)plan >> 8;
-    SSD_REQUIRE(!gn_sums || a.splits > 1 || (H * W) % bm == 0, "conv2d_nhwc_f32x2_presplit: fused GroupNorm statistics need H*W to be a multiple of the M tile");
+    SSD_REQUIRE(!gn_sums || a.splits > 1 || (H * W) % bm == 0, "%s: fused GroupNorm statistics need H*W to be a multiple of the M tile", fn);
+    SSD_REQUIRE(!Csc || a.splits == 1 || a.splitk_ws, "%s: the plan cuts K %u ways and needs a zeroed split-K workspace of %zu bytes", fn, a.splits, (size_t)a.M * Cout * 4);
     a.m_tiles = (a.M + bm - 1) / bm; a.n_tiles = Cout / bn;
     float* const ws = a.splitk_ws;
     if (a.splits > 1 && !ws) {
-        if (hipMemsetAsync(y, 0, (size_t)a.M * Cout * 4, st) != hipSuccess) return ssdnerf_fail(SSDNERF_E_LAUNCH, "conv2d_nhwc_f32x2_presplit: memset failed");
+        if (hipMemsetAsync(y, 0, (size_t)a.M * Cout * 4, st) != hipSuccess) return ssdnerf_fail(SSDNERF_E_LAUNCH, "%s: memset failed", fn);
         a.splitk_ws = (float*)y;
     }
     const dim3 grid(a.m_tiles * a.n_tiles * a.splits);
@@ -1637,7 +1690,7 @@
     else if (choice == 2) hipLaunchKernelGGL((k_conv_igemm_bf16<1, 2, 2, 2, 3, false, true>), grid, dim3(256), 0, st, a);
     else hipLaunchKernelGGL((k_conv_igemm_bf16<1, 1, 2, 2, CV_NS_SMALL, false, true>), grid, dim3(256), 0, st, a);
     if (a.splits > 1) cv_launch_finish(a, true, ws, st);
-    SSD_CHECK_LAUNCH("conv2d_nhwc_f32x2_presplit");
+    SSD_CHECK_LAUNCH(fn);
     return SSDNERF_OK;
 }
 
diff --git a/ssdnerf_amd/csrc/groupnorm.hip b/ssdnerf_amd/csrc/groupnorm.hip
--- a/ssdnerf_amd/csrc/groupnorm.hip
+++ b/ssdnerf_amd/csrc/groupnorm.hip
@@ -148,7 +148,7 @@
 __global__ __launch_bounds__(GN_TPB) void k_gn_apply(const void* __restrict__ x, const void* __restrict__ x2, uint32_t C1, const float* __restrict__ pre_bias,
                                                       uint32_t HW, uint32_t C, uint32_t G, uint32_t rows_per_block, const double* __restrict__ sums, const float* __restrict__ gamma,
                                                       const float* __restrict__ beta, const float* __restrict__ scale_shift, uint32_t ss_stride, float eps,
-                                                      int act, void* __restrict__ y, const double* __restrict__ sums2 = nullptr) {
+                                                      int act, void* __restrict__ y, const double* __restrict__ sums2 = nullptr, void* __restrict__ xs = nullptr) {
     constexpr int V = GnVec<DT>::V;
     __shared__ float fa[GN_MAX_C], fb[GN_MAX_C];
     const uint32_t tpr = C / V, rif = GN_TPB / tpr;
@@ -216,6 +216,9 @@
 #pragma unroll
         for (int k = 0; k < UR; ++k) {
             if (r0 + k * rif >= rows_per_block) break;
+            if constexpr (DT == GN_F32) {
+                if (xs) GnVec<DT>::store_split(xs, base + (size_t)(r0 + k * rif) * tpr, f[k]);
+            }
 #pragma unroll
             for (int i = 0; i < V; i += 2) {
                 f2 v = __builtin_elementwise_fma(f2{f[k][i], f[k][i + 1]}, f2{a[i], a[i + 1]}, f2{o[i], o[i + 1]});
@@ -557,29 +560,44 @@
     return SSDNERF_OK;
 }
 
-extern "C" int ssdnerf_group_norm_nhwc_runs(const void* x, const void* x2, uint32_t C1, int dtype, uint32_t B, uint32_t HW, uint32_t C, uint32_t G, const float* gamma,
-                                            const float* beta, const float* scale_shift, uint32_t scale_shift_stride, float eps, int act, const void* runs1,
-                                            const void* runs2, void* y, void* stream) {
+static int gn_runs_launch(const char* fn, const void* x, const void* x2, uint32_t C1, int dtype, uint32_t B, uint32_t HW, uint32_t C, uint32_t G, const float* gamma,
+                          const float* beta, const float* scale_shift, uint32_t scale_shift_stride, float eps, int act, const void* runs1, const void* runs2, void* y,
+                          void* xs, void* stream) {
     if (B == 0 || HW == 0 || C == 0) return SSDNERF_OK;
-    SSD_REQUIRE(x && y && gamma && beta && runs1 && (!x2 || runs2), "group_norm_nhwc_runs: null pointer");
-    SSD_REQUIRE(dtype == GN_F32 || dtype == GN_F16 || dtype == GN_BF16, "group_norm_nhwc_runs: dtype must be 0 (f32), 1 (f16) or 2 (bf16)");
+    SSD_REQUIRE(x && y && gamma && beta && runs1 && (!x2 || runs2), "%s: null pointer", fn);
+    SSD_REQUIRE(dtype == GN_F32 || dtype == GN_F16 || dtype == GN_BF16, "%s: dtype must be 0 (f32), 1 (f16) or 2 (bf16)", fn);
     const uint32_t V = dtype == GN_F32 ? 4 : 8;
-    SSD_REQUIRE(G > 0 && G <= GN_TPB && C % G == 0 && (C / G) % 4 == 0, "group_norm_nhwc_runs: groups must be multiples of 4 channels (and at most 256 groups)");
-    SSD_REQUIRE(!scale_shift || scale_shift_stride >= 2 * C, "group_norm_nhwc_runs: scale_shift_stride must be >= 2*C");
-    SSD_REQUIRE(C % V == 0 && C / V <= GN_TPB && C <= GN_MAX_C, "group_norm_nhwc_runs: channel count must be a multiple of the 16-byte vector and <= 1024 (f32) / 2048 (16-bit)");
+    SSD_REQUIRE(G > 0 && G <= GN_TPB && C % G == 0 && (C / G) % 4 == 0, "%s: groups must be multiples of 4 channels (and at most 256 groups)", fn);
+    SSD_REQUIRE(!scale_shift || scale_shift_stride >= 2 * C, "%s: scale_shift_stride must be >= 2*C", fn);
+    SSD_REQUIRE(C % V == 0 && C / V <= GN_TPB && C <= GN_MAX_C, "%s: channel count must be a multiple of the 16-byte vector and <= 1024 (f32) / 2048 (16-bit)", fn);
     if (!x2) C1 = C;
-    SSD_REQUIRE(C1 <= C && C1 % V == 0 && (x2 || C1 == C), "group_norm_nhwc_runs: the first tensor's channel count must be a multiple of the 16-byte vector and <= C");
-    SSD_REQUIRE(!(act & 2) || (dtype == GN_F32 && C % 32 == 0), "group_norm_nhwc_runs: the pre-split output (act & 2) needs fp32 and C % 32 == 0");
+    SSD_REQUIRE(C1 <= C && C1 % V == 0 && (x2 || C1 == C), "%s: the first tensor's channel count must be a multiple of the 16-byte vector and <= C", fn);
+    SSD_REQUIRE(!(act & 2) || (dtype == GN_F32 && C % 32 == 0), "%s: the pre-split output (act & 2) needs fp32 and C %% 32 == 0", fn);
+    SSD_REQUIRE(!xs || (dtype == GN_F32 && C % 32 == 0), "%s: the raw pre-split output needs fp32 and C %% 32 == 0", fn);
     hipStream_t st = (hipStream_t)stream;
     const uint32_t rows_a = gn_rows_per_block(B, HW, GN_FWD_APPLY_BLOCKS, GN_FWD_APPLY_ROWS);
     const dim3 grid_a(HW / rows_a, B), block(GN_TPB);
 #define SSD_GN_LAUNCH(DT)                                                                                                                    \
     hipLaunchKernelGGL((k_gn_apply<DT, true>), grid_a, block, 0, st, x, x2, C1, (const float*)nullptr, HW, C, G, rows_a, (const double*)runs1, gamma, beta, scale_shift,    \
-                       scale_shift_stride, eps, act, y, (const double*)runs2);
+                       scale_shift_stride, eps, act, y, (const double*)runs2, xs);
     if (dtype == GN_F32) { SSD_GN_LAUNCH(GN_F32) } else if (dtype == GN_F16) { SSD_GN_LAUNCH(GN_F16) } else { SSD_GN_LAUNCH(GN_BF16) }
 #undef SSD_GN_LAUNCH
-    SSD_CHECK_LAUNCH("group_norm_nhwc_runs");
+    SSD_CHECK_LAUNCH(fn);
     return SSDNERF_OK;
+}
+
+extern "C" int ssdnerf_group_norm_nhwc_runs(const void* x, const void* x2, uint32_t C1, int dtype, uint32_t B, uint32_t HW, uint32_t C, uint32_t G, const float* gamma,
+                                            const float* beta, const float* scale_shift, uint32_t scale_shift_stride, float eps, int act, const void* runs1,
+                                            const void* runs2, void* y, void* stream) {
+    return gn_runs_launch("group_norm_nhwc_runs", x, x2, C1, dtype, B, HW, C, G, gamma, beta, scale_shift, scale_shift_stride, eps, act, runs1, runs2, y, nullptr, stream);
+}
+
+extern "C" int ssdnerf_group_norm_nhwc_runs_raw_split(const void* x, const void* x2, uint32_t C1, uint32_t B, uint32_t HW, uint32_t C, uint32_t G, const float* gamma,
+                                                      const float* beta, const float* scale_shift, uint32_t scale_shift_stride, float eps, int act, const void* runs1,
+                                                      const void* runs2, void* y, void* xs, void* stream) {
+    if (B == 0 || HW == 0 || C == 0) return SSDNERF_OK;
+    SSD_REQUIRE(xs, "group_norm_nhwc_runs_raw_split: null pointer");
+    return gn_runs_launch("group_norm_nhwc_runs_raw_split", x, x2, C1, GN_F32, B, HW, C, G, gamma, beta, scale_shift, scale_shift_stride, eps, act, runs1, runs2, y, xs, stream);
 }
 
 extern "C" int ssdnerf_group_norm_nhwc_backward_cat(const void* x, const void* x2, uint32_t C1, const void* dy, int dtype, uint32_t B, uint32_t HW, uint32_t C, uint32_t G,
diff --git a/ssdnerf_amd/unet_fast.py b/ssdnerf_amd/unet_fast.py
--- a/ssdnerf_amd/unet_fast.py
+++ b/ssdnerf_amd/unet_fast.py
@@ -23,7 +23,7 @@
 def group_norm_nhwc(x: torch.Tensor, groups: int, gamma: torch.Tensor, beta: torch.Tensor, scale_shift: Optional[torch.Tensor], eps: float,
                     act: bool, workspace: torch.Tensor, out: Optional[torch.Tensor] = None, pre_bias: Optional[torch.Tensor] = None,
                     workspace_is_zero: bool = False, stats_ready: bool = False, x2: Optional[torch.Tensor] = None,
-                    runs: Optional[Tuple[torch.Tensor, Optional[torch.Tensor]]] = None, split_out: bool = False) -> torch.Tensor:
+                    runs: Optional[Tuple[torch.Tensor, Optional[torch.Tensor]]] = None, split_out: bool = False, raw_split: bool = False):
     act_bits = int(bool(act)) | (2 if split_out else 0)
     if x.dim() == 4:
         B, C1, H, W = x.shape
@@ -50,6 +50,15 @@
     if scale_shift is not None:
         assert scale_shift.dtype == torch.float32 and scale_shift.shape == (B, 2 * Cc) and scale_shift.stride(1) == 1
         ss_stride = scale_shift.stride(0)
+    if raw_split:
+        if runs is None or x.dtype != torch.float32 or Cc % 32 != 0:
+            raise RuntimeError("group_norm_nhwc: raw_split needs fp32, C % 32 == 0 and run-level statistics")
+        assert pre_bias is None and (x2 is None) == (runs[1] is None)
+        xs = torch.empty_like(y)
+        C.check(C.lib().ssdnerf_group_norm_nhwc_runs_raw_split(C.ptr(x), C.ptr(x2), C.u32(C1), C.u32(B), C.u32(HW), C.u32(Cc), C.u32(groups), C.ptr(gamma), C.ptr(beta),
+                                                                C.ptr(scale_shift), C.u32(ss_stride), C.f32(eps), act_bits, C.ptr(runs[0]), C.ptr(runs[1]), C.ptr(y), C.ptr(xs),
+                                                                C.stream()), "group_norm_nhwc_runs_raw_split")
+        return y, xs
     if runs is not None:
         assert pre_bias is None and (x2 is None) == (runs[1] is None)
         C.check(C.lib().ssdnerf_group_norm_nhwc_runs(C.ptr(x), C.ptr(x2), C.u32(C1), _GN_DTYPE[x.dtype], C.u32(B), C.u32(HW), C.u32(Cc), C.u32(groups), C.ptr(gamma),
@@ -215,6 +224,23 @@
                                                         C.u32(Cin), C.u32(Cout), C.u32(k), C.ptr(gn_sums), C.u32(gn_groups), int(tile_hint), int(splits_hint), C.ptr(splitk_ws),
                                                         ctypes.c_size_t(0 if splitk_ws is None else splitk_ws.numel() * splitk_ws.element_size()), C.stream()),
             "conv2d_nhwc_f32x2_presplit")
+    return y
+
+
+def conv2d_nhwc_f32x2_presplit_sc(x_split: torch.Tensor, w_hi: torch.Tensor, w_lo: torch.Tensor, xs: torch.Tensor, sc_hi: torch.Tensor, sc_lo: torch.Tensor,
+                                  bias: Optional[torch.Tensor] = None, gn_sums: Optional[torch.Tensor] = None, gn_groups: int = 0, splitk_ws: Optional[torch.Tensor] = None,
+                                  tile_hint: int = 0, splits_hint: int = 0) -> torch.Tensor:
+    B, Cin, H, W = x_split.shape
+    Cout, k, Csc = w_hi.shape[0], w_hi.shape[2], xs.shape[1]
+    ok = lambda t: t.is_contiguous(memory_format=torch.channels_last) and t.dtype == torch.float32
+    if not ok(x_split) or not ok(xs) or tuple(w_hi.shape[1:]) != (Cin, k, k) or k not in (1, 3) or xs.shape != (B, Csc, H, W) or tuple(sc_hi.shape) != (Cout, Csc, 1, 1) \
+            or sc_lo.shape != sc_hi.shape or sc_lo.data_ptr() != sc_hi.data_ptr() + Cout * Csc * 2:
+        raise RuntimeError("conv2d_nhwc_f32x2_presplit_sc: channels_last carrier tensors x_split (B, Cin, H, W) and xs (B, Csc, H, W), adjacent weight pairs (Cout, Cin, k, k) and (Cout, Csc, 1, 1)")
+    y = torch.empty((B, Cout, H, W), dtype=torch.float32, device=x_split.device, memory_format=torch.channels_last)
+    C.check(C.lib().ssdnerf_conv2d_nhwc_f32x2_presplit_sc(C.ptr(x_split), C.ptr(w_hi), C.ptr(w_lo), C.ptr(xs), C.ptr(sc_hi), C.u32(Csc), C.ptr(bias), C.ptr(y), C.u32(B), C.u32(H),
+                                                           C.u32(W), C.u32(Cin), C.u32(Cout), C.u32(k), C.ptr(gn_sums), C.u32(gn_groups), int(tile_hint), int(splits_hint),
+                                                           C.ptr(splitk_ws), ctypes.c_size_t(0 if splitk_ws is None else splitk_ws.numel() * splitk_ws.element_size()), C.stream()),
+            "conv2d_nhwc_f32x2_presplit_sc")
     return y
 
 
@@ -350,8 +376,22 @@
                     and presplit_supported(x, int(self.w.shape[0]), int(self.w.shape[2]), with_stats))
 
     PRESPLIT = os.environ.get("SSDNERF_UNET_PRESPLIT", "1") != "0"
-
-    def igemm(self, x, bias=None, residual=None, upsample=False, gn_sums=None, gn_groups=0, x2=None, presplit=False):
+    FOLD_SHORTCUT = os.environ.get("SSDNERF_UNET_FOLD_SHORTCUT", "1") != "0"
+
+    def folds_shortcut(self, h, sc, csc: int) -> bool:
+        if not (_Conv.FOLD_SHORTCUT and sc is not None and sc.own and sc.w_lo is not None and csc % 32 == 0 and int(sc.w.shape[1]) == csc and int(sc.w.shape[2]) == 1
+                and sc.stride[0] == 1 and self.takes_presplit(h, with_stats=True)):
+            return False
+        if presplit_supported(h, int(self.w.shape[0]), int(self.w.shape[2]), True) != 2:
+            return False
+        M, cout = h.size(0) * h.size(2) * h.size(3), int(self.w.shape[0])
+        plan = C.lib().ssdnerf_conv2d_nhwc_f32x2_presplit_plan(C.u32(M), C.u32(h.size(1)), C.u32(cout), C.u32(self.w.shape[2]), C.u32(csc), 0, 0)
+        return M * csc * 4 < 2 ** 31 and (plan >> 8 == 1 or _Conv.SPLITK_BYTES >= M * cout * 4)
+
+    def igemm(self, x, bias=None, residual=None, upsample=False, gn_sums=None, gn_groups=0, x2=None, presplit=False, xs=None, sc=None):
+        if xs is not None:
+            assert presplit and residual is None
+            return conv2d_nhwc_f32x2_presplit_sc(x, self.w_lo[0], self.w_lo[1], xs, sc.w_lo[0], sc.w_lo[1], bias, gn_sums, gn_groups, splitk_ws=shared_splitk_ws(x.device))
         if presplit:
             return conv2d_nhwc_f32x2_presplit(x, self.w_lo[0], self.w_lo[1], bias, residual, gn_sums, gn_groups, splitk_ws=shared_splitk_ws(x.device))
         if self.w_lo is not None:
@@ -506,14 +546,15 @@
         assert ws.numel() == n, "GroupNorm statistics arena exhausted"
         return ws
 
-    def _gn(self, x, gn: _GN, ss, act, pre_bias=None, stats=None, x2=None, stats2=None, split=False):
+    def _gn(self, x, gn: _GN, ss, act, pre_bias=None, stats=None, x2=None, stats2=None, split=False, raw_split=False):
         Cc = (x.size(1) if x.dim() == 4 else x.size(2)) + (x2.size(1) if x2 is not None else 0)
         if stats is not None and (x2 is None or stats2 is not None) and (Cc // gn.groups) % 4 == 0:
-            return group_norm_nhwc(x, gn.groups, gn.gamma, gn.beta, ss, gn.eps, act, stats, x2=x2, runs=(stats, stats2), split_out=split)
+            return group_norm_nhwc(x, gn.groups, gn.gamma, gn.beta, ss, gn.eps, act, stats, x2=x2, runs=(stats, stats2), split_out=split, raw_split=raw_split)
+        assert not raw_split
         return group_norm_nhwc(x, gn.groups, gn.gamma, gn.beta, ss, gn.eps, act, self._stats_slice(x.size(0)), pre_bias=pre_bias, workspace_is_zero=True,
                                x2=x2, split_out=split)
 
-    def _can_fuse_stats(self, conv: _Conv, x, upsample=False):
+    def _can_fuse_stats(self, conv: _Conv, x, upsample=False, csc=0):
         if not conv.own:
             return False
         hw = x.size(2) * x.size(3) * (4 if upsample else 1) // (conv.stride[0] * conv.stride[1])
@@ -522,6 +563,9 @@
             return False
         if hw > 128 * 256:
             return False
+        if csc:
+            plan = C.lib().ssdnerf_conv2d_nhwc_f32x2_presplit_plan(C.u32(x.size(0) * hw), C.u32(cin), C.u32(cout), C.u32(k), C.u32(csc), 0, 0)
+            return plan >> 8 != 1 or hw % (128 if (plan & 0xff) == 1 else 64) == 0
         if conv.w_lo is not None:
             plan = C.lib().ssdnerf_conv2d_nhwc_f32x2_plan(C.u32(x.size(0) * hw), C.u32(cin), C.u32(cout), C.u32(k), 0, 0)
             if plan >> 8 != 1:
@@ -532,9 +576,10 @@
             return True
         return hw % (256 if (plan & 0xff) == 4 else 128 if (plan & 0xff) == 1 else 64) == 0
 
-    def _conv_stats(self, conv: _Conv, x, bias=None, residual=None, upsample=False, x2=None, presplit=False):
-        st = self._stats_slice(x.size(0), conv.w.size(0)) if self._can_fuse_stats(conv, x, upsample) else None
-        return conv.igemm(x, bias, residual, upsample=upsample, gn_sums=st, gn_groups=conv.w.size(0) // 4 if st is not None else 0, x2=x2, presplit=presplit), st
+    def _conv_stats(self, conv: _Conv, x, bias=None, residual=None, upsample=False, x2=None, presplit=False, xs=None, sc=None):
+        st = self._stats_slice(x.size(0), conv.w.size(0)) if self._can_fuse_stats(conv, x, upsample, csc=xs.size(1) if xs is not None else 0) else None
+        return conv.igemm(x, bias, residual, upsample=upsample, gn_sums=st, gn_groups=conv.w.size(0) // 4 if st is not None else 0, x2=x2, presplit=presplit,
+                          xs=xs, sc=sc), st
 
     def _res(self, x, stats, op, ss_all, x2=None, stats2=None):
         _, gn1, conv1, gn2, (off, n), conv2, shortcut, out_bias = op
@@ -545,10 +590,17 @@
         if own:
             cin1 = x.size(1) + (x2.size(1) if x2 is not None else 0)
             ps1 = conv1.w_lo is not None and conv1.takes_presplit(_like(x, cin1), with_stats=True)
-            g1 = self._gn(x, gn1, None, True, stats=stats, x2=x2, stats2=stats2, split=ps1)
+            fold = conv2.w_lo is not None and stats is not None and (x2 is None or stats2 is not None) and (cin1 // gn1.groups) % 4 == 0 \
+                and conv2.folds_shortcut(_like(x, int(conv1.w.shape[0])), shortcut, cin1)
+            if fold:
+                g1, xs = self._gn(x, gn1, None, True, stats=stats, x2=x2, stats2=stats2, split=ps1, raw_split=True)
+            else:
+                g1 = self._gn(x, gn1, None, True, stats=stats, x2=x2, stats2=stats2, split=ps1)
             h, st1 = self._conv_stats(conv1, g1, conv1.bias, presplit=ps1)
             ps2 = conv2.w_lo is not None and conv2.takes_presplit(h, with_stats=True)
             g2 = self._gn(h, gn2, ss, True, stats=st1, split=ps2)
+            if fold:
+                return self._conv_stats(conv2, g2, out_bias, None, presplit=True, xs=xs, sc=shortcut)
             skip = shortcut.igemm(x, x2=x2) if shortcut is not None else x
             return self._conv_stats(conv2, g2, out_bias, skip, presplit=ps2)
         g1 = self._gn(x, gn1, None, True, stats=stats, x2=x2, stats2=stats2)
```

New measurement: 6.667 billion, median of 2. No clear change (-0.2%).
